# hkchengrex/Cutie

Measured on AMD Instinct MI355X. Metric: frames/sec (480p, 3 objects), higher is better.
Workload: dtype bf16

## Files before the change

### cutie_amd/_lib.py

```python
import ctypes
import os

_HERE = os.path.dirname(os.path.abspath(__file__))
LIB_PATH = os.environ.get('CUTIE_AMD_LIB') or os.path.join(_HERE, 'libcutie_hip.so')
ABI_VERSION = 11
OP_STRUCT_SIZE = 256

_lib = None


class HipLibraryError(RuntimeError):
    pass


def load():
    global _lib
    if _lib is not None:
        return _lib
    if not os.path.exists(LIB_PATH):
        raise HipLibraryError(
            f'{LIB_PATH} not found: build it with `python -c "import __graft_entry__ as g; g.build()"` '
            f'(or `make -C cutie_amd/csrc`).  cutie_amd has no CPU fallback.')
    lib = ctypes.CDLL(LIB_PATH)
    lib.cutie_exec.argtypes = [ctypes.c_void_p, ctypes.c_int, ctypes.c_void_p]
    lib.cutie_exec.restype = ctypes.c_int
    lib.cutie_exec_one.argtypes = [ctypes.c_void_p, ctypes.c_void_p]
    lib.cutie_exec_one.restype = ctypes.c_int
    lib.cutie_graph_capture.argtypes = [ctypes.c_void_p, ctypes.c_int, ctypes.c_void_p]
    lib.cutie_graph_capture.restype = ctypes.c_void_p
    lib.cutie_graph_launch.argtypes = [ctypes.c_void_p, ctypes.c_void_p]
    lib.cutie_graph_launch.restype = ctypes.c_int
    lib.cutie_graph_destroy.argtypes = [ctypes.c_void_p]
    lib.cutie_graph_destroy.restype = None
    lib.cutie_time_ops.argtypes = [ctypes.c_void_p, ctypes.c_int, ctypes.c_int, ctypes.c_void_p]
    lib.cutie_time_ops.restype = ctypes.c_float
    lib.cutie_hip_last_error.argtypes = []
    lib.cutie_hip_last_error.restype = ctypes.c_char_p
    lib.cutie_hip_abi_version.restype = ctypes.c_int
    lib.cutie_op_struct_size.restype = ctypes.c_int
    lib.cutie_hip_build_flags.restype = ctypes.c_int
    if lib.cutie_hip_abi_version() != ABI_VERSION or lib.cutie_op_struct_size() != OP_STRUCT_SIZE:
        raise HipLibraryError(f'{LIB_PATH} is stale (ABI {lib.cutie_hip_abi_version()}, '
                              f'op size {lib.cutie_op_struct_size()}); rebuild it.')
    _lib = lib
    return lib


EXPORTED_SYMBOLS = ['cutie_exec', 'cutie_exec_one', 'cutie_graph_capture', 'cutie_graph_launch',
                    'cutie_graph_destroy', 'cutie_time_ops', 'cutie_hip_last_error',
                    'cutie_hip_abi_version', 'cutie_op_struct_size', 'cutie_hip_build_flags']


def has_diag_kernels():
    return bool(load().cutie_hip_build_flags() & 1)


def has_png_decode():
    return bool(load().cutie_hip_build_flags() & 2)


class HipExecutor:
    is_mock = False

    def __init__(self):
        import torch
        self.lib = load()
        if not torch.cuda.is_available():
            raise HipLibraryError('no HIP device visible: cutie_amd runs on MI355X only (no CPU fallback).')
        self._torch = torch
        self._raw_stream = getattr(torch._C, '_cuda_getCurrentRawStream', None)
        self.graph_stats = [0, 0]
        self._warned = False

    def stream(self):
        raw = self._raw_stream
        if raw is not None:
            return raw(self._torch.cuda.current_device())
        return self._torch.cuda.current_stream().cuda_stream

    def run(self, arr):
        rc = self.lib.cutie_exec(arr.ctypes.data, len(arr), self.stream())
        if rc != 0:
            raise RuntimeError('cutie_exec failed: ' + self.lib.cutie_hip_last_error().decode())

    def run_on(self, arr, stream):
        rc = self.lib.cutie_exec(arr.ctypes.data, len(arr), stream.cuda_stream)
        if rc != 0:
            raise RuntimeError('cutie_exec failed: ' + self.lib.cutie_hip_last_error().decode())

    GRAPH_CACHE_ENTRIES = 24

    def run_cached(self, arr, cache, head=0):
        if head:
            self.run(arr[:head])
            arr = arr[head:]
        key = arr['p'].tobytes()
        ent = cache.get(key)
        if ent is None:
            if len(cache) >= self.GRAPH_CACHE_ENTRIES:
                old = cache.pop(next(iter(cache)))
                if old not in (0, -1):
                    self.lib.cutie_graph_destroy(old)
            cache[key] = 0
            self.graph_stats[0] += 1
            return self.run(arr)
        if ent == 0:
            ent = self.lib.cutie_graph_capture(arr.ctypes.data, len(arr), self.stream()) or -1
            cache[key] = ent
            if ent == -1 and not self._warned:
                self._warned = True
                import warnings
                warnings.warn('HIP graph capture of a launch plan failed (%s); such plans keep running launch by launch'
                              % self.lib.cutie_hip_last_error().decode())
        if ent == -1:
            self.graph_stats[0] += 1
            return self.run(arr)
        self.graph_stats[1] += 1
        if self.lib.cutie_graph_launch(ent, self.stream()) != 0:
            raise RuntimeError('cutie_graph_launch failed: ' + self.lib.cutie_hip_last_error().decode())

    def time_ops(self, arr, iters):
        ms = self.lib.cutie_time_ops(arr.ctypes.data, len(arr), iters, self.stream())
        if ms < 0:
            raise RuntimeError('cutie_time_ops failed: ' + self.lib.cutie_hip_last_error().decode())
        return ms


_executor = None


def get_executor():
    global _executor
    if _executor is None:
        _executor = HipExecutor()
    return _executor


def set_executor_for_testing(ex):
    global _executor
    _executor = ex
```

### cutie_amd/csrc/api.hip

```cpp
#include "common.h"
#include <stdarg.h>
#include <stdio.h>
#include <string.h>

static thread_local char g_err[512] = "";

void cutie_set_error(const char* fmt, ...) {
    va_list ap;
    va_start(ap, fmt);
    vsnprintf(g_err, sizeof(g_err), fmt, ap);
    va_end(ap);
}

static int dispatch(const cutie_op* op, hipStream_t s) {
    switch (op->kind) {
        case CUTIE_OP_CONV: return launch_conv(op, s);
        case CUTIE_OP_QUERY_INIT: return (op->flags & 1) ? launch_attention(op, s) : launch_elementwise(op, s);
        case CUTIE_OP_QFFN: return launch_qchain(op, s);
        case CUTIE_OP_STEM: return launch_stem(op, s);
        case CUTIE_OP_ATTN_Q2P: case CUTIE_OP_ATTN_SELF: case CUTIE_OP_ATTN_P2Q:
            return (op->flags & 12) ? launch_qchain(op, s) : launch_attention(op, s);
        case CUTIE_OP_AUX_MASK:
            return launch_attention(op, s);
        case CUTIE_OP_KEY_PREP: case CUTIE_OP_AFF_SCORE: case CUTIE_OP_AFF_SELECT: case CUTIE_OP_AFF_READOUT:
            return launch_affinity(op, s);
        case CUTIE_OP_RANK_SELECT: case CUTIE_OP_GATHER_ROWS: case CUTIE_OP_CONSOL_AFF: case CUTIE_OP_CONSOL_READ:
            return launch_bank(op, s);
        default:
            if (op->kind > 0 && op->kind < CUTIE_OP__COUNT) return launch_elementwise(op, s);
            cutie_set_error("cutie_exec: unknown op kind %d", op->kind);
            return -3;
    }
}

extern "C" {

int cutie_exec(const cutie_op* ops, int n, void* stream) {
    hipStream_t s = (hipStream_t)stream;
    for (int k = 0; k < n; ++k) {
        int rc = dispatch(&ops[k], s);
        if (rc != 0) {
            if (rc > 0) cutie_set_error("op %d (kind %d): HIP error %d (%s)", k, ops[k].kind, rc, hipGetErrorString((hipError_t)rc));
            else {
                char tmp[400];
                snprintf(tmp, sizeof(tmp), "%s", g_err);
                cutie_set_error("op %d (kind %d): %s", k, ops[k].kind, tmp);
            }
            return rc > 0 ? -1 : rc;
        }
    }
    return 0;
}

int cutie_exec_one(const cutie_op* op, void* stream) { return cutie_exec(op, 1, stream); }

struct GraphHandle { hipGraph_t graph; hipGraphExec_t exec; };

void* cutie_graph_capture(const cutie_op* ops, int n, void* stream) {
    (void)stream;
    static thread_local hipStream_t cap = nullptr;
    if (!cap && hipStreamCreateWithFlags(&cap, hipStreamNonBlocking) != hipSuccess) {
        cap = nullptr;
        (void)hipGetLastError();
        cutie_set_error("graph: cannot create the capture stream");
        return nullptr;
    }
    hipGraph_t graph = nullptr;
    if (hipStreamBeginCapture(cap, hipStreamCaptureModeThreadLocal) != hipSuccess) {
        (void)hipGetLastError();
        cutie_set_error("graph: begin capture failed");
        return nullptr;
    }
    int rc = cutie_exec(ops, n, (void*)cap);
    hipError_t e = hipStreamEndCapture(cap, &graph);
    if (rc != 0 || e != hipSuccess || !graph) {
        if (graph) hipGraphDestroy(graph);
        if (rc == 0) cutie_set_error("graph: end capture failed (%d)", (int)e);
        (void)hipGetLastError();
        return nullptr;
    }
    hipGraphExec_t exec = nullptr;
    if (hipGraphInstantiate(&exec, graph, nullptr, nullptr, 0) != hipSuccess) {
        hipGraphDestroy(graph);
        (void)hipGetLastError();
        cutie_set_error("graph: instantiate failed");
        return nullptr;
    }
    GraphHandle* h = new GraphHandle{graph, exec};
    return h;
}

int cutie_graph_launch(void* graph, void* stream) {
    GraphHandle* h = (GraphHandle*)graph;
    if (!h) { cutie_set_error("graph: null handle"); return -4; }
    hipError_t e = hipGraphLaunch(h->exec, (hipStream_t)stream);
    if (e != hipSuccess) { cutie_set_error("graph launch: %s", hipGetErrorString(e)); return -1; }
    return 0;
}

void cutie_graph_destroy(void* graph) {
    GraphHandle* h = (GraphHandle*)graph;
    if (!h) return;
    hipGraphExecDestroy(h->exec);
    hipGraphDestroy(h->graph);
    delete h;
}

float cutie_time_ops(const cutie_op* ops, int n, int iters, void* stream) {
    hipStream_t s = (hipStream_t)stream;
    hipEvent_t a, b;
    if (hipEventCreate(&a) != hipSuccess || hipEventCreate(&b) != hipSuccess) { cutie_set_error("time: event create failed"); return -1.f; }
    if (cutie_exec(ops, n, stream) != 0) return -1.f;
    hipEventRecord(a, s);
    for (int it = 0; it < iters; ++it)
        if (cutie_exec(ops, n, stream) != 0) return -1.f;
    hipEventRecord(b, s);
    hipEventSynchronize(b);
    float ms = 0.f;
    hipEventElapsedTime(&ms, a, b);
    hipEventDestroy(a);
    hipEventDestroy(b);
    return ms / (float)iters;
}

const char* cutie_hip_last_error(void) { return g_err; }
int cutie_hip_abi_version(void) { return 11; }
int cutie_op_struct_size(void) { return (int)sizeof(cutie_op); }
int cutie_hip_build_flags(void) {
    const int forms = 2;
#ifdef CUTIE_DIAG
    return forms | 1;
#else
    return forms;
#endif
}

}
```

### cutie_amd/csrc/conv_common.h

```cpp
#pragma once
#include "common.h"

struct ConvParams {
    const bf16_t* x1; const bf16_t* x2; const bf16_t* w; const float* bias; const bf16_t* res; void* y;
    int B, H, W, C1, C2, ldx1, ldx2, OH, OW, Cout, ldy, KH, KW, stride, pad, ldr, Kpad;
    int flags, M, Cin, OHW;
    float* part; int splitk, ldp, Kslice;
    long long* gap; unsigned long long* zero; int nzero;
    const unsigned char* pf; int pf_bytes;
    const unsigned char* pf2; int pf2_bytes;
    int res_grp_rows, res_grp_stride;
};
#define GAP_FIXED_SCALE 16777216.f
#define GAP_ELEM_SHIFT 4
__device__ __forceinline__ long long conv_gapfx(float v) {
    if (__builtin_expect(fabsf(v) < 2048.f, 1)) return (long long)__float2int_rn(v * 1048576.f);
    if (v != v) return 0;
    const float c = fminf(fmaxf(v, -1048576.f), 1048576.f);
    const float hi = truncf(c);
    return (long long)(int)hi * 1048576LL + (long long)__float2int_rn((c - hi) * 1048576.f);
}

typedef __attribute__((ext_vector_type(4))) unsigned int u32x4;
typedef const __attribute__((address_space(1))) u32x4* gptr16;
#define GLOAD16(ptr) (*(gptr16)(ptr))

template <int CPR>
__device__ __forceinline__ int swz(int row) {
    return CPR == 4 ? ((row >> 3) & 1) * 3 : (row & (CPR - 1));
}

__device__ __forceinline__ int conv_res_row(const ConvParams& p, int m) {
    if (!(p.flags & CUTIE_F_RES_BCAST)) return m;
    int r = m % p.OHW;
    if (p.res_grp_rows > 0) r += (m / p.res_grp_rows) * p.res_grp_stride;
    return r;
}

__device__ __forceinline__ void conv_finish(const ConvParams& p, float* v, int m, int ch0) {
    const int act = (p.flags >> CUTIE_ACT_SHIFT) & 7;
    const bool out_f32 = p.flags & CUTIE_F_OUT_F32;
    const bool vec_y = out_f32 ? ((p.ldy & 3) == 0) : ((p.ldy & 7) == 0);
    const bool vec_r = (p.ldr & 7) == 0;
    const bool full = ch0 + 7 < p.Cout;
    if (p.bias) {
        if (full && (reinterpret_cast<uintptr_t>(p.bias) & 15) == 0) {
            const float4 b0 = *reinterpret_cast<const float4*>(p.bias + ch0), b1 = *reinterpret_cast<const float4*>(p.bias + ch0 + 4);
            v[0] += b0.x; v[1] += b0.y; v[2] += b0.z; v[3] += b0.w; v[4] += b1.x; v[5] += b1.y; v[6] += b1.z; v[7] += b1.w;
        } else {
#pragma unroll
            for (int r = 0; r < 8; ++r) if (ch0 + r < p.Cout) v[r] += p.bias[ch0 + r];
        }
    }
    if (p.res) {
        const int mres = conv_res_row(p, m);
        const bf16_t* rp = p.res + (long)mres * p.ldr + ch0;
        if (full && vec_r) {
            const uint4 rr = *reinterpret_cast<const uint4*>(rp);
            v[0] += __uint_as_float(rr.x << 16); v[1] += __uint_as_float(rr.x & 0xffff0000u);
            v[2] += __uint_as_float(rr.y << 16); v[3] += __uint_as_float(rr.y & 0xffff0000u);
            v[4] += __uint_as_float(rr.z << 16); v[5] += __uint_as_float(rr.z & 0xffff0000u);
            v[6] += __uint_as_float(rr.w << 16); v[7] += __uint_as_float(rr.w & 0xffff0000u);
        } else {
#pragma unroll
            for (int r = 0; r < 8; ++r) if (ch0 + r < p.Cout) v[r] += bf2f(rp[r]);
        }
    }
#pragma unroll
    for (int r = 0; r < 8; ++r) {
        if (act == CUTIE_ACT_RELU) v[r] = fmaxf(v[r], 0.f);
        else if (act == CUTIE_ACT_SIGMOID) v[r] = sigmoidf_(v[r]);
        else if (act == CUTIE_ACT_SQ1) v[r] = v[r] * v[r] + 1.f;
    }
    if (out_f32) {
        float* yp = reinterpret_cast<float*>(p.y) + (long)m * p.ldy + ch0;
        if (full && vec_y) {
            *reinterpret_cast<float4*>(yp) = make_float4(v[0], v[1], v[2], v[3]);
            *reinterpret_cast<float4*>(yp + 4) = make_float4(v[4], v[5], v[6], v[7]);
        } else {
#pragma unroll
            for (int r = 0; r < 8; ++r) if (ch0 + r < p.Cout) yp[r] = v[r];
        }
    } else {
        bf16_t* yp = reinterpret_cast<bf16_t*>(p.y) + (long)m * p.ldy + ch0;
        if (full && vec_y) {
            *reinterpret_cast<uint4*>(yp) = make_uint4(pack_bf2(v[0], v[1]), pack_bf2(v[2], v[3]), pack_bf2(v[4], v[5]), pack_bf2(v[6], v[7]));
        } else {
#pragma unroll
            for (int r = 0; r < 8; ++r) if (ch0 + r < p.Cout) yp[r] = f2bf(v[r]);
        }
    }
}

template <int BM, int BN, int BK, int WK>
constexpr int conv_lds_bytes() {
    constexpr int pipe = WK * 2 * (BM + BN) * (BK / 8) * 16, epi = BM * (BN + 4) * 4;
    return pipe > epi ? pipe : epi;
}

__device__ __forceinline__ void conv_preload_args(const ConvParams& p) {
#ifndef CONV_NO_PRELOAD
    asm volatile("" :: "s"(p.x1), "s"(p.w), "s"(p.bias), "s"(p.res), "s"(p.y), "s"(p.zero),
                 "s"(p.B), "s"(p.H), "s"(p.W), "s"(p.C1), "s"(p.C2), "s"(p.ldx1), "s"(p.ldx2), "s"(p.OH), "s"(p.OW), "s"(p.Cout), "s"(p.ldy),
                 "s"(p.KH), "s"(p.KW), "s"(p.stride), "s"(p.pad), "s"(p.ldr), "s"(p.Kpad), "s"(p.flags), "s"(p.M), "s"(p.Cin), "s"(p.OHW),
                 "s"(p.nzero), "s"(gridDim.x), "s"(gridDim.y));
#endif
}

#ifdef CONV_TIMELINE
#define TL_MAX 96
#define TL_BYTES (16 * TL_MAX * 8)
#define TL_DECL(...) unsigned long long* const tlp_ = reinterpret_cast<unsigned long long*>(__VA_ARGS__) + wave * TL_MAX; int tln_ = 0;
#define TL_PUT_(ID, CAP) { if (tln_ < (CAP)) { const unsigned long long t_ = (__builtin_readcyclecounter() << 8) | (unsigned)(ID); if ((threadIdx.x & 63) == 0) tlp_[tln_] = t_; ++tln_; } }
#define TL(ID) TL_PUT_(ID, TL_MAX - 6)
#define TLE(ID) TL_PUT_(ID, TL_MAX)
#define TL_DUMP(LOGICAL, NB, NWAVES)                                                                                        \
    {                                                                                                                       \
        const int slot_ = (LOGICAL) == 0 ? 0 : (LOGICAL) == 1 ? 1 : (LOGICAL) == (NB) / 2 ? 2 : (LOGICAL) == (NB) - 1 ? 3 : -1; \
        if (slot_ >= 0 && p.part) {                                                                                         \
            __builtin_amdgcn_s_waitcnt(0);                                                                                  \
            unsigned long long* o_ = reinterpret_cast<unsigned long long*>(p.part) + ((long)slot_ * 16 + wave) * (TL_MAX + 2); \
            if ((threadIdx.x & 63) == 0) { o_[0] = 0x544c0000ull | (unsigned)tln_; o_[1] = ((unsigned long long)(LOGICAL) << 32) | (unsigned)(NWAVES); } \
            for (int q_ = threadIdx.x & 63; q_ < tln_; q_ += 64) o_[2 + q_] = tlp_[q_];                                     \
        }                                                                                                                   \
    }
#else
#define TL_BYTES 0
#define TL_DECL(...)
#define TL(ID)
#define TLE(ID)
#define TL_DUMP(LOGICAL, NB, NWAVES)
#endif

int launch_conv_dma(const ConvParams& p, int tile, hipStream_t s);
int launch_conv_pc(const ConvParams& p, int tile, hipStream_t s);
```

### cutie_amd/csrc/conv_igemm.hip

```cpp
#include "conv_common.h"

template <int BM, int BN, int WM, int WN, int BK, int S, int OCC, int WK>
__global__ __launch_bounds__(WM * WN * WK * 64) void conv_igemm_kernel(ConvParams p) {
    if (p.flags & CUTIE_F_PRIO) __builtin_amdgcn_s_setprio(1);
    constexpr int NTB = WM * WN * WK * 64;
    constexpr int NT = WM * WN * 64;
    constexpr int CPR = BK / 8;
    constexpr int RPT = NT / CPR;
    constexpr int NX = (BM * CPR) / NT;
    constexpr int NWC = (BN * CPR + NT - 1) / NT;
    constexpr int TM = BM / WM / 16;
    constexpr int TN = BN / WN / 16;
    constexpr int KSUB = BK / 32;
    constexpr int NWRAP = BK == 32 ? 4 : BK / 32;
    static_assert((NT == 256 || NT == 512) && NTB <= 1024 && NX >= 1 && TM >= 1 && TN >= 1 && S >= 2 && (BM * CPR) % NT == 0, "bad tile");
    constexpr int LDC = BN + 4;
    constexpr int GRP_CHUNKS = 2 * (BM + BN) * CPR;
    extern __shared__ __attribute__((aligned(16))) u32x4 smem_raw[];
    const int grp = threadIdx.x / NT;
    u32x4 (*smem)[(BM + BN) * CPR] = reinterpret_cast<u32x4 (*)[(BM + BN) * CPR]>(smem_raw + grp * GRP_CHUNKS);

    const int tid = threadIdx.x % NT, lane = tid & 63, wave = tid >> 6;
    int m0, n0;
    {
// ... 136 lines not shown
            const int ks = ks0 + u;
            if (ks < nk) K_ITER(ks, u, ks + S - 1 < nk, ks + 1 < nk)
        }
    }

    float* ctile = reinterpret_cast<float*>(smem_raw);
#pragma unroll
    for (int g = WK - 1; g >= 0; --g) {
        if (grp == g) {
#pragma unroll
            for (int b = 0; b < TM; ++b)
#pragma unroll
                for (int a = 0; a < TN; ++a) {
                    const int px = pm0 + b * 16 + l15, ch = cn0 + a * 16 + l4 * 4;
                    f32x4* dst = reinterpret_cast<f32x4*>(ctile + px * LDC + ch);
                    if (g == WK - 1) *dst = acc[a][b];
                    else { f32x4 t = *dst; t[0] += acc[a][b][0]; t[1] += acc[a][b][1]; t[2] += acc[a][b][2]; t[3] += acc[a][b][3]; *dst = t; }
                }
        }
        __syncthreads();
    }
    constexpr int CH8 = BN / 8;
    if (p.splitk == 1) {
        for (int q = threadIdx.x; q < BM * CH8; q += NTB) {
            const int px = q / CH8, c8 = q - px * CH8;
            const int m = m0 + px, ch0 = n0 + c8 * 8;
            if (m >= p.M || ch0 >= p.Cout) continue;
            const f32x4 lo = *reinterpret_cast<const f32x4*>(ctile + px * LDC + c8 * 8);
            const f32x4 hi = *reinterpret_cast<const f32x4*>(ctile + px * LDC + c8 * 8 + 4);
            float v[8] = {lo[0], lo[1], lo[2], lo[3], hi[0], hi[1], hi[2], hi[3]};
            conv_finish(p, v, m, ch0);
        }
        return;
    }
    float* part = p.part + (long)blockIdx.z * p.M * p.ldp;
    for (int q = threadIdx.x; q < BM * CH8; q += NTB) {
        const int px = q / CH8, c8 = q - px * CH8;
        const int m = m0 + px, ch0 = n0 + c8 * 8;
        if (m >= p.M || ch0 >= p.Cout) continue;
        float* dst = part + (long)m * p.ldp + ch0;
        *reinterpret_cast<f32x4*>(dst) = *reinterpret_cast<const f32x4*>(ctile + px * LDC + c8 * 8);
        *reinterpret_cast<f32x4*>(dst + 4) = *reinterpret_cast<const f32x4*>(ctile + px * LDC + c8 * 8 + 4);
    }
}

__global__ __launch_bounds__(256) void conv_splitk_reduce_kernel(ConvParams p) {
    const int c8n = p.ldp >> 3;
    const long q = (long)blockIdx.x * 256 + threadIdx.x;
    if (q >= (long)p.M * c8n) return;
    const int m = (int)(q / c8n), ch0 = (int)(q - (long)m * c8n) * 8;
    float v[8] = {0.f, 0.f, 0.f, 0.f, 0.f, 0.f, 0.f, 0.f};
    for (int z = 0; z < p.splitk; ++z) {
        const float* src = p.part + ((long)z * p.M + m) * p.ldp + ch0;
        const f32x4 lo = *reinterpret_cast<const f32x4*>(src);
        const f32x4 hi = *reinterpret_cast<const f32x4*>(src + 4);
        v[0] += lo[0]; v[1] += lo[1]; v[2] += lo[2]; v[3] += lo[3];
        v[4] += hi[0]; v[5] += hi[1]; v[6] += hi[2]; v[7] += hi[3];
    }
    conv_finish(p, v, m, ch0);
}

__global__ __launch_bounds__(256) void conv_cout1_kernel(ConvParams p) {
    if (p.flags & CUTIE_F_PRIO) __builtin_amdgcn_s_setprio(1);
    extern __shared__ __attribute__((aligned(16))) unsigned char wlds_raw[];
    u32x4* wlds = reinterpret_cast<u32x4*>(wlds_raw);
    const int LP = p.Cin >> 3;
    const int ntap = p.KH * p.KW;
    const int ppb = 256 / LP;
    const int sub = threadIdx.x / LP, cl = threadIdx.x % LP;
    const int m = blockIdx.x * ppb + sub;
    const bool is33 = p.KH == 3 && p.KW == 3;
    const bool relu_in = p.flags & CUTIE_F_RELU_IN;
    const float bias0 = p.bias ? p.bias[0] : 0.f;
    u32x4 xv[9];
    float ok[9];
    if (is33) {
        const int mc = min(m, p.M - 1);
        const int b = mc / p.OHW, rem = mc - b * p.OHW, oh = rem / p.OW, ow = rem - oh * p.OW;
#pragma unroll
        for (int t = 0; t < 9; ++t) {
            const int ih = oh * p.stride - p.pad + t / 3, iw = ow * p.stride - p.pad + t % 3;
            const bool v = (unsigned)ih < (unsigned)p.H && (unsigned)iw < (unsigned)p.W;
            const int ihc = min(max(ih, 0), p.H - 1), iwc = min(max(iw, 0), p.W - 1);
            xv[t] = *reinterpret_cast<const u32x4*>(p.x1 + (((long)b * p.H + ihc) * p.W + iwc) * p.ldx1 + cl * 8);
            ok[t] = v ? 1.f : 0.f;
        }
    }
    for (int t = threadIdx.x; t < ntap * LP; t += 256) wlds[t] = *reinterpret_cast<const u32x4*>(p.w + (long)t * 8);
    __syncthreads();
    float acc = 0.f;
    if (m < p.M) {
        const int b = m / p.OHW, rem = m - b * p.OHW, oh = rem / p.OW, ow = rem - oh * p.OW;
        if (is33) {
#pragma unroll
            for (int t = 0; t < 9; ++t) {
                u32x4 x = xv[t];
                if (relu_in) { x.x = relu_bf2(x.x); x.y = relu_bf2(x.y); x.z = relu_bf2(x.z); x.w = relu_bf2(x.w); }
                const u32x4 wv = wlds[t * LP + cl];
                float a = 0.f;
#pragma unroll
                for (int i = 0; i < 4; ++i) {
                    a += __uint_as_float(x[i] << 16) * __uint_as_float(wv[i] << 16);
                    a += __uint_as_float(x[i] & 0xffff0000u) * __uint_as_float(wv[i] & 0xffff0000u);
                }
                acc += a * ok[t];
            }
        } else
        for (int kh = 0; kh < p.KH; ++kh) {
            const int ih = oh * p.stride - p.pad + kh;
            if ((unsigned)ih >= (unsigned)p.H) continue;
            for (int kw = 0; kw < p.KW; ++kw) {
                const int iw = ow * p.stride - p.pad + kw;
                if ((unsigned)iw >= (unsigned)p.W) continue;
                u32x4 xv = *reinterpret_cast<const u32x4*>(p.x1 + (((long)b * p.H + ih) * p.W + iw) * p.ldx1 + cl * 8);
                if (relu_in) { xv.x = relu_bf2(xv.x); xv.y = relu_bf2(xv.y); xv.z = relu_bf2(xv.z); xv.w = relu_bf2(xv.w); }
                const u32x4 wv = wlds[(kh * p.KW + kw) * LP + cl];
#pragma unroll
                for (int i = 0; i < 4; ++i) {
                    acc += __uint_as_float(xv[i] << 16) * __uint_as_float(wv[i] << 16);
                    acc += __uint_as_float(xv[i] & 0xffff0000u) * __uint_as_float(wv[i] & 0xffff0000u);
                }
            }
        }
    }
    for (int o = LP >> 1; o > 0; o >>= 1) acc += __shfl_xor(acc, o, 64);
    if (cl == 0 && m < p.M) {
        float v = acc + bias0;
        const int act = (p.flags >> CUTIE_ACT_SHIFT) & 7;
        if (act == CUTIE_ACT_RELU) v = fmaxf(v, 0.f);
        else if (act == CUTIE_ACT_SIGMOID) v = sigmoidf_(v);
        else if (act == CUTIE_ACT_SQ1) v = v * v + 1.f;
        if (p.flags & CUTIE_F_OUT_F32) reinterpret_cast<float*>(p.y)[(long)m * p.ldy] = v;
        else reinterpret_cast<bf16_t*>(p.y)[(long)m * p.ldy] = f2bf(v);
    }
}

template <int TR>
__global__ __launch_bounds__(256) void conv_cout1_tile_kernel(ConvParams p) {
    if (p.flags & CUTIE_F_PRIO) __builtin_amdgcn_s_setprio(1);
    static_assert(TR % 4 == 0, "rows per wave");
    constexpr int TC = 16, PW = TC + 2, NPIX = (TR + 2) * PW, RW = TR / 4;
    __shared__ u32x4 tile[NPIX * 16];
    const int tid = threadIdx.x, lane = tid & 63, wave = tid >> 6, n = lane & 15, g = lane >> 4;
    const int tiles_x = (p.W + TC - 1) / TC, tiles_y = (p.H + TR - 1) / TR;
    const int b = blockIdx.x / (tiles_x * tiles_y), rem = blockIdx.x - b * tiles_x * tiles_y;
    const int ty = rem / tiles_x, tx = rem - ty * tiles_x;
    const int x0 = tx * TC, y0 = ty * TR;
    const bool relu_in = p.flags & CUTIE_F_RELU_IN;
    const float bias0 = p.bias ? p.bias[0] : 0.f;
    __shared__ u32x4 wl[36 * 4];
    const u32x4 wmine = tid < 144 ? *reinterpret_cast<const u32x4*>(p.w + (long)((tid >> 4) * 16 + (tid & 15)) * 8) : (u32x4){0u, 0u, 0u, 0u};
    constexpr int NCH = (NPIX * 16 + 255) / 256;
    u32x4 st[NCH];
#pragma unroll
    for (int i = 0; i < NCH; ++i) {
        const int q = tid + 256 * i, px = q >> 4, c = q & 15;
        const int iy = y0 + px / PW - 1, ix = x0 + px % PW - 1;
        const bool in = q < NPIX * 16 && (unsigned)iy < (unsigned)p.H && (unsigned)ix < (unsigned)p.W;
        const long o = in ? (((long)b * p.H + iy) * p.W + ix) * p.ldx1 + c * 8 : 0;
        const u32x4 v = *reinterpret_cast<const u32x4*>(p.x1 + o);
        st[i] = in ? v : (u32x4){0u, 0u, 0u, 0u};
    }
#pragma unroll
    for (int i = 0; i < NCH; ++i) {
        const int q = tid + 256 * i, px = q >> 4, c = q & 15;
        u32x4 v = st[i];
        if (relu_in) { v.x = relu_bf2(v.x); v.y = relu_bf2(v.y); v.z = relu_bf2(v.z); v.w = relu_bf2(v.w); }
        if (q < NPIX * 16) tile[px * 16 + (c ^ (px & 15))] = v;
    }
    if (tid < 144) wl[tid] = wmine;
    __syncthreads();
    f32x4 acc[RW];
#pragma unroll
    for (int r = 0; r < RW; ++r) acc[r] = (f32x4){0.f, 0.f, 0.f, 0.f};
    const u32x4 zero4 = {0u, 0u, 0u, 0u};
#pragma unroll
    for (int sidx = 0; sidx < 36; ++sidx) {
        const int tap = sidx >> 2, ky = tap / 3, kx = tap - 3 * ky, ch = (sidx & 3) * 4 + g;
        const u32x4 wv = wl[sidx * 4 + g];
        const bf16x8 wb = __builtin_bit_cast(bf16x8, n == 0 ? wv : zero4);
#pragma unroll
        for (int r = 0; r < RW; ++r) {
            const int px = (wave * RW + r + ky) * PW + n + kx;
            const bf16x8 a = __builtin_bit_cast(bf16x8, tile[px * 16 + (ch ^ (px & 15))]);
            acc[r] = __builtin_amdgcn_mfma_f32_16x16x32_bf16(a, wb, acc[r], 0, 0, 0);
        }
    }
    if (n == 0) {
        const int act = (p.flags >> CUTIE_ACT_SHIFT) & 7;
#pragma unroll
        for (int r = 0; r < RW; ++r) {
            const int oy = y0 + wave * RW + r;
#pragma unroll
            for (int q = 0; q < 4; ++q) {
                const int x = x0 + 4 * g + q;
                if (x < p.W && oy < p.H) {
                    float v = acc[r][q] + bias0;
                    if (act == CUTIE_ACT_RELU) v = fmaxf(v, 0.f);
                    else if (act == CUTIE_ACT_SIGMOID) v = sigmoidf_(v);
                    else if (act == CUTIE_ACT_SQ1) v = v * v + 1.f;
                    const long m = ((long)b * p.H + oy) * p.W + x;
                    if (p.flags & CUTIE_F_OUT_F32) reinterpret_cast<float*>(p.y)[m * p.ldy] = v;
                    else reinterpret_cast<bf16_t*>(p.y)[m * p.ldy] = f2bf(v);
                }
            }
        }
    }
}

template <int R>
__global__ __launch_bounds__(256) void conv_cout1_rows_kernel(ConvParams p) {
    if (p.flags & CUTIE_F_PRIO) __builtin_amdgcn_s_setprio(1);
    const int LP = p.Cin >> 3;
    const int ppb = 256 / LP;
    const int sub = threadIdx.x / LP, cl = threadIdx.x % LP;
    const int tiles_x = (p.W + ppb - 1) / ppb, tiles_y = (p.H + R - 1) / R;
    const int b = blockIdx.x / (tiles_x * tiles_y), rem = blockIdx.x - b * tiles_x * tiles_y;
    const int ty = rem / tiles_x, tx = rem - ty * tiles_x;
    const int x = tx * ppb + sub, y0 = ty * R;
    const bool relu_in = p.flags & CUTIE_F_RELU_IN;
    const float bias0 = p.bias ? p.bias[0] : 0.f;
    u32x4 wv[9];
#pragma unroll
    for (int t = 0; t < 9; ++t) wv[t] = *reinterpret_cast<const u32x4*>(p.w + (long)(t * LP + cl) * 8);
    u32x4 xv[R + 2][3];
    float okc[3];
#pragma unroll
    for (int kx = 0; kx < 3; ++kx) okc[kx] = ((unsigned)(x + kx - 1) < (unsigned)p.W) ? 1.f : 0.f;
#pragma unroll
    for (int r = 0; r < R + 2; ++r) {
        const int iy = min(max(y0 + r - 1, 0), p.H - 1);
#pragma unroll
        for (int kx = 0; kx < 3; ++kx) {
            const int ix = min(max(x + kx - 1, 0), p.W - 1);
            xv[r][kx] = *reinterpret_cast<const u32x4*>(p.x1 + (((long)b * p.H + iy) * p.W + ix) * p.ldx1 + cl * 8);
        }
    }
    if (relu_in) {
#pragma unroll
        for (int r = 0; r < R + 2; ++r)
#pragma unroll
            for (int kx = 0; kx < 3; ++kx) { u32x4& v = xv[r][kx]; v.x = relu_bf2(v.x); v.y = relu_bf2(v.y); v.z = relu_bf2(v.z); v.w = relu_bf2(v.w); }
    }
    const int act = (p.flags >> CUTIE_ACT_SHIFT) & 7;
#pragma unroll
    for (int j = 0; j < R; ++j) {
        const int oy = y0 + j;
        float acc = 0.f;
#pragma unroll
        for (int ky = 0; ky < 3; ++ky) {
            const float okr = ((unsigned)(oy + ky - 1) < (unsigned)p.H) ? 1.f : 0.f;
#pragma unroll
            for (int kx = 0; kx < 3; ++kx) {
                const u32x4 xx = xv[j + ky][kx], ww = wv[ky * 3 + kx];
                float a = 0.f;
#pragma unroll
                for (int i = 0; i < 4; ++i) {
                    a += __uint_as_float(xx[i] << 16) * __uint_as_float(ww[i] << 16);
                    a += __uint_as_float(xx[i] & 0xffff0000u) * __uint_as_float(ww[i] & 0xffff0000u);
                }
                acc += a * (okr * okc[kx]);
            }
        }
        for (int o = LP >> 1; o > 0; o >>= 1) acc += __shfl_xor(acc, o, 64);
        if (cl == 0 && x < p.W && oy < p.H) {
            float v = acc + bias0;
            if (act == CUTIE_ACT_RELU) v = fmaxf(v, 0.f);
            else if (act == CUTIE_ACT_SIGMOID) v = sigmoidf_(v);
            else if (act == CUTIE_ACT_SQ1) v = v * v + 1.f;
            const long m = ((long)b * p.H + oy) * p.W + x;
            if (p.flags & CUTIE_F_OUT_F32) reinterpret_cast<float*>(p.y)[m * p.ldy] = v;
            else reinterpret_cast<bf16_t*>(p.y)[m * p.ldy] = f2bf(v);
        }
    }
}

template <int BM, int BN, int WM, int WN, int BK, int S, int OCC, int WK = 1>
static int launch_cfg(ConvParams p, hipStream_t s) {
    if (p.Kpad % BK) { cutie_set_error("conv: Kpad %d not a multiple of BK %d", p.Kpad, BK); return -2; }
    if (BK > 32 && p.Cin < 32) { cutie_set_error("conv: BK %d needs Cin >= 32 (Cin=%d)", BK, p.Cin); return -2; }
    const int nk_all = p.Kpad / BK;
    if (p.splitk > nk_all) { cutie_set_error("conv: splitk %d > K tiles %d", p.splitk, nk_all); return -2; }
    if (nk_all % (p.splitk * WK)) { cutie_set_error("conv: splitk %d x %d K groups must divide the %d K tiles", p.splitk, WK, nk_all); return -2; }
    p.Kslice = p.Kpad / p.splitk;
    constexpr int lds = conv_lds_bytes<BM, BN, BK, WK>();
    static bool attr_set = false;
    if (!attr_set) {
        if (lds > 65536 && hipFuncSetAttribute(reinterpret_cast<const void*>(conv_igemm_kernel<BM, BN, WM, WN, BK, S, OCC, WK>),
                                               hipFuncAttributeMaxDynamicSharedMemorySize, lds) != hipSuccess) {
            cutie_set_error("conv: cannot raise the dynamic LDS limit to %d bytes", lds);
            return -2;
        }
        attr_set = true;
    }
    dim3 grid((p.M + BM - 1) / BM, (p.Cout + BN - 1) / BN, p.splitk);
    hipLaunchKernelGGL((conv_igemm_kernel<BM, BN, WM, WN, BK, S, OCC, WK>), grid, dim3(WM * WN * WK * 64), lds, s, p);
    if (p.splitk > 1) {
        const long nq = (long)p.M * (p.ldp >> 3);
        hipLaunchKernelGGL(conv_splitk_reduce_kernel, dim3((unsigned)((nq + 255) / 256)), dim3(256), 0, s, p);
    }
    return (int)hipGetLastError();
}

int launch_conv(const cutie_op* op, hipStream_t s) {
    ConvParams p;
    p.x1 = (const bf16_t*)op->p[0]; p.x2 = (const bf16_t*)op->p[1]; p.w = (const bf16_t*)op->p[2];
    p.bias = (const float*)op->p[3]; p.res = (const bf16_t*)op->p[4]; p.y = (void*)op->p[5];
    const int32_t* i = op->i;
    p.B = i[0]; p.H = i[1]; p.W = i[2]; p.C1 = i[3]; p.C2 = i[4]; p.ldx1 = i[5]; p.ldx2 = i[6];
    p.OH = i[7]; p.OW = i[8]; p.Cout = i[9]; p.ldy = i[10]; p.KH = i[11]; p.KW = i[12];
    p.stride = i[13]; p.pad = i[14]; p.ldr = i[15]; p.Kpad = i[16];
    p.flags = op->flags; p.OHW = p.OH * p.OW; p.M = p.B * p.OHW; p.Cin = p.C1 + p.C2;
    p.splitk = i[19] > 1 ? i[19] : 1; p.part = (float*)op->p[6];
    p.ldp = (p.Cout + 7) & ~7;
    p.gap = (long long*)op->p[7]; p.zero = (unsigned long long*)op->p[8]; p.nzero = i[21];
    p.pf = (const unsigned char*)op->p[9]; p.pf_bytes = op->p[9] ? i[22] : 0;
    p.pf2 = (const unsigned char*)op->p[10]; p.pf2_bytes = op->p[10] ? i[23] : 0;
    p.res_grp_rows = p.res_grp_stride = 0;
    if ((p.flags & CUTIE_F_RES_BCAST) && op->f[0] > 0.f) {
        const int kg = (int)op->f[0];
        if (kg <= 0 || p.B % kg || op->f[1] < (float)p.OHW || op->f[1] != (float)(int)op->f[1]) { cutie_set_error("conv: residual groups of %d objects do not divide B = %d (or stride %g < OH*OW)", kg, p.B, (double)op->f[1]); return -2; }
        p.res_grp_rows = kg * p.OHW; p.res_grp_stride = (int)op->f[1];
    }
    if ((p.gap || p.zero) && (i[17] < 60 || i[17] >= 200 || ((p.flags & CUTIE_F_OUT_F32) && p.gap) || (p.Cout & 7) || (p.ldy & 7) || (p.res && (p.ldr & 7)))) {
        cutie_set_error("conv: GAP accumulation / zero job need an LDS-DMA tile (60..199), bf16 output, Cout %% 8 == 0 (tile %d)", i[17]);
        return -2;
    }
    if (p.splitk > 1 && (!p.part || (long)p.splitk * p.M * p.ldp > (long)i[20] * 1024)) {
        cutie_set_error("conv: split-K %d needs the fp32 partial scratch (p6, capacity i20 KiB-floats)", p.splitk);
        return -2;
    }
    if ((p.C1 & 7) || (p.C2 & 7) || (p.ldx1 & 7) || (p.C2 && (p.ldx2 & 7)) || (p.Kpad & 31) ||
        p.Kpad < p.KH * p.KW * p.Cin || p.M <= 0 || p.Cout <= 0) {
        cutie_set_error("conv: bad geometry C1=%d C2=%d ldx1=%d ldx2=%d Kpad=%d M=%d Cout=%d",
                        p.C1, p.C2, p.ldx1, p.ldx2, p.Kpad, p.M, p.Cout);
        return -2;
    }
    if (i[17] == 19) {
        const int LP = p.Cin >> 3;
        if (p.Cout != 1 || p.C2 != 0 || p.res || LP > 64 || (LP & (LP - 1)) || LP < 1) {
            cutie_set_error("conv cout1: needs Cout=1, single source, no residual, Cin/8 a power of two <= 64 (Cin=%d)", p.Cin);
            return -2;
        }
        const int ppb = 256 / LP;
        if (!(p.flags & CUTIE_F_PLAIN) && p.KH == 3 && p.KW == 3 && p.stride == 1 && p.pad == 1 && p.OH == p.H && p.OW == p.W && LP >= 8 && LP <= 32 && p.H * p.W >= 4096) {
            if (LP == 16 && !(p.flags & CUTIE_F_TILE_OFF)) {
                constexpr int TR = 8;
                const int blocks = p.B * ((p.H + TR - 1) / TR) * ((p.W + 15) / 16);
                hipLaunchKernelGGL(conv_cout1_tile_kernel<TR>, dim3(blocks), dim3(256), 0, s, p);
                return (int)hipGetLastError();
            }
            constexpr int R = 4;
            const int blocks = p.B * ((p.H + R - 1) / R) * ((p.W + ppb - 1) / ppb);
            hipLaunchKernelGGL(conv_cout1_rows_kernel<R>, dim3(blocks), dim3(256), 0, s, p);
            return (int)hipGetLastError();
        }
        hipLaunchKernelGGL(conv_cout1_kernel, dim3((p.M + ppb - 1) / ppb), dim3(256), (size_t)p.KH * p.KW * LP * 16, s, p);
        return (int)hipGetLastError();
    }
    if (i[17] >= 60 && i[17] < 90) return launch_conv_dma(p, i[17], s);
    if (i[17] >= 100 && i[17] < 200) return launch_conv_pc(p, i[17], s);
    switch (i[17]) {
        case 0: return launch_cfg<128, 128, 2, 2, 32, 4, 2>(p, s);
        case 1: return launch_cfg<128, 64, 2, 2, 32, 4, 3>(p, s);
        case 2: return launch_cfg<64, 64, 2, 2, 32, 4, 4>(p, s);
        case 3: return launch_cfg<256, 16, 4, 1, 32, 4, 3>(p, s);
        case 4: return launch_cfg<64, 128, 2, 2, 32, 4, 3>(p, s);
        case 5: return launch_cfg<64, 64, 2, 2, 64, 4, 3>(p, s);
        case 6: return launch_cfg<64, 128, 2, 2, 64, 3, 2>(p, s);
        case 7: return launch_cfg<128, 128, 2, 2, 64, 2, 2>(p, s);
        case 8: return launch_cfg<64, 64, 2, 2, 128, 3, 2>(p, s);
        case 9: return launch_cfg<32, 64, 2, 2, 64, 4, 4>(p, s);
        case 10: return launch_cfg<128, 64, 2, 2, 64, 3, 2>(p, s);
        case 11: return launch_cfg<32, 64, 2, 2, 128, 3, 3>(p, s);
        case 12: return launch_cfg<32, 128, 2, 2, 64, 3, 2>(p, s);
        case 13: return launch_cfg<64, 64, 2, 4, 64, 4, 5>(p, s);
        case 14: return launch_cfg<128, 64, 4, 2, 64, 4, 4>(p, s);
        case 15: return launch_cfg<64, 128, 2, 4, 64, 4, 4>(p, s);
        case 16: return launch_cfg<128, 128, 2, 4, 64, 3, 3>(p, s);
        case 17: return launch_cfg<64, 64, 2, 4, 128, 3, 4>(p, s);
        case 18: return launch_cfg<128, 128, 2, 4, 32, 4, 4>(p, s);
        case 20: return launch_cfg<64, 64, 2, 2, 64, 4, 3, 2>(p, s);
        case 21: return launch_cfg<64, 64, 2, 2, 128, 3, 2, 2>(p, s);
        case 22: return launch_cfg<32, 64, 2, 2, 128, 3, 3, 2>(p, s);
        case 23: return launch_cfg<128, 64, 2, 2, 64, 3, 2, 2>(p, s);
        case 24: return launch_cfg<64, 128, 2, 2, 64, 3, 2, 2>(p, s);
        case 25: return launch_cfg<128, 128, 2, 2, 64, 2, 2, 2>(p, s);
        case 26: return launch_cfg<32, 64, 2, 2, 64, 4, 4, 2>(p, s);
        case 27: return launch_cfg<64, 64, 2, 2, 64, 3, 3, 4>(p, s);
        case 28: return launch_cfg<32, 64, 2, 2, 64, 4, 4, 4>(p, s);
        case 29: return launch_cfg<64, 128, 2, 2, 32, 4, 3, 2>(p, s);
        case 30: return launch_cfg<64, 64, 2, 2, 32, 4, 4, 2>(p, s);
        default: cutie_set_error("conv: bad tile id %d", i[17]); return -2;
    }
}
```

### cutie_amd/csrc/conv_pc.hip

```cpp
#include "conv_common.h"

typedef __amdgpu_buffer_rsrc_t rsrc_t;
#define PC_WORD3 0x00020000
#define PC_RECORDS 0x7fffffff
#define PC_OOB 0x80000000u
#define LDS_PTR(p) ((__attribute__((address_space(3))) void*)(p))
#define PC_WAIT_VM(N) __builtin_amdgcn_s_waitcnt(((N) & 15) | (((N) >> 4) << 14) | (7 << 4) | (15 << 8))
#define PC_WAIT_LGKM0() __builtin_amdgcn_s_waitcnt(15 | (3 << 14) | (7 << 4) | (0 << 8))
#define PC_BARRIER() { asm volatile("" ::: "memory"); __builtin_amdgcn_s_barrier(); asm volatile("" ::: "memory"); }
#ifdef PC_ABL_NO_LOOPBAR
#define PC_LOOP_BARRIER() { asm volatile("" ::: "memory"); }
#else
#define PC_LOOP_BARRIER() PC_BARRIER()
#endif
#ifdef PC_ABL_NO_WAIT
#define PC_LOOP_WAIT_VM(N) ((void)0)
#else
#define PC_LOOP_WAIT_VM(N) PC_WAIT_VM(N)
#endif
#ifdef PC_ABL_SAME_TILE
#define PC_SAME_TILE_GUARD(...)
#else
#define PC_SAME_TILE_GUARD(...) __VA_ARGS__
#endif
#ifdef PC_ABL_NO_DMA
#define PC_DMA(...) ((void)0)
#else
#define PC_DMA(...) __builtin_amdgcn_raw_ptr_buffer_load_lds(__VA_ARGS__)
#endif

__device__ __forceinline__ rsrc_t pc_rsrc(const void* base) {
    return __builtin_amdgcn_make_buffer_rsrc(const_cast<void*>(base), 0, PC_RECORDS, PC_WORD3);
}

typedef short pc_s16x2 __attribute__((ext_vector_type(2)));
__device__ __forceinline__ unsigned pc_relu2(unsigned w) {
    return __builtin_bit_cast(unsigned, __builtin_elementwise_max(__builtin_bit_cast(pc_s16x2, w), (pc_s16x2){0, 0}));
}

__device__ __forceinline__ int pc_wrow(int R, bool pair) {
    if (!pair) return R;
    const int ii = R & 15, alo = (R >> 4) & 1;
    return (R & ~31) | ((ii >> 2) << 3) | (alo << 2) | (ii & 3);
}

#define PC_HT(TH, TW) ((TH) * 256 + (TW))
template <int BM, int BN, int NS, int HT>
constexpr int pc_lds_bytes(int NPW) {
    if (HT == 0) return NS * (BM + BN) * 128;
    const int TH = HT >> 8, TW = HT & 255, npiece = ((TH + 2) * (TW + 2) + 7) / 8, nxp = (npiece + NPW - 1) / NPW;
    return 2 * nxp * NPW * 1024 + NS * BN * 128;
}

template <int NCH>
__device__ __forceinline__ void pc_finish(const ConvParams& p, float (&v)[NCH], int m, int ch0, bool vec_ok, bool have_res,
                                          const unsigned (&rpre)[NCH / 2], float (&stored)[NCH]) {
#ifdef PC_ABL_FIXED_EPI
    {
#pragma unroll
        for (int r = 0; r < NCH; ++r) v[r] = fmaxf(v[r], 0.f);
        bf16_t* yp = reinterpret_cast<bf16_t*>(p.y) + (long)m * p.ldy + ch0;
        unsigned o[NCH / 2];
#pragma unroll
        for (int r = 0; r < NCH / 2; ++r) o[r] = pack_bf2(v[2 * r], v[2 * r + 1]);
        if constexpr (NCH == 8) *reinterpret_cast<uint4*>(yp) = make_uint4(o[0], o[1], o[NCH / 2 - 2], o[NCH / 2 - 1]);
        else *reinterpret_cast<uint2*>(yp) = make_uint2(o[0], o[1]);
        return;
    }
#endif
    const int act = (p.flags >> CUTIE_ACT_SHIFT) & 7;
    const bool out_f32 = p.flags & CUTIE_F_OUT_F32;
    const bool full = ch0 + NCH <= p.Cout;
    if (p.res) {
        if (have_res) {
#pragma unroll
            for (int r = 0; r < NCH / 2; ++r) { v[2 * r] += __uint_as_float(rpre[r] << 16); v[2 * r + 1] += __uint_as_float(rpre[r] & 0xffff0000u); }
        } else {
            const int mres = conv_res_row(p, m);
            const bf16_t* rp = p.res + (long)mres * p.ldr + ch0;
            if (full && vec_ok) {
                unsigned rr[NCH / 2];
                if constexpr (NCH == 8) { const uint4 t = *reinterpret_cast<const uint4*>(rp); rr[0] = t.x; rr[1] = t.y; rr[NCH / 2 - 2] = t.z; rr[NCH / 2 - 1] = t.w; }
                else { const uint2 t = *reinterpret_cast<const uint2*>(rp); rr[0] = t.x; rr[1] = t.y; }
#pragma unroll
                for (int r = 0; r < NCH / 2; ++r) { v[2 * r] += __uint_as_float(rr[r] << 16); v[2 * r + 1] += __uint_as_float(rr[r] & 0xffff0000u); }
            } else {
#pragma unroll
                for (int r = 0; r < NCH; ++r) if (ch0 + r < p.Cout) v[r] += bf2f(rp[r]);
            }
        }
    }
#pragma unroll
    for (int r = 0; r < NCH; ++r) {
        if (act == CUTIE_ACT_RELU) v[r] = fmaxf(v[r], 0.f);
        else if (act == CUTIE_ACT_SIGMOID) v[r] = sigmoidf_(v[r]);
        else if (act == CUTIE_ACT_SQ1) v[r] = v[r] * v[r] + 1.f;
    }
    if (out_f32) {
        float* yp = reinterpret_cast<float*>(p.y) + (long)m * p.ldy + ch0;
        if (full && vec_ok) {
#pragma unroll
            for (int r = 0; r < NCH; r += 4) *reinterpret_cast<float4*>(yp + r) = make_float4(v[r], v[r + 1], v[r + 2], v[r + 3]);
        } else {
#pragma unroll
            for (int r = 0; r < NCH; ++r) if (ch0 + r < p.Cout) yp[r] = v[r];
        }
    } else {
        bf16_t* yp = reinterpret_cast<bf16_t*>(p.y) + (long)m * p.ldy + ch0;
        unsigned o[NCH / 2];
#pragma unroll
        for (int r = 0; r < NCH / 2; ++r) o[r] = pack_bf2(v[2 * r], v[2 * r + 1]);
        if (full && vec_ok) {
            if constexpr (NCH == 8) *reinterpret_cast<uint4*>(yp) = make_uint4(o[0], o[1], o[NCH / 2 - 2], o[NCH / 2 - 1]);
            else *reinterpret_cast<uint2*>(yp) = make_uint2(o[0], o[1]);
        } else {
#pragma unroll
            for (int r = 0; r < NCH; ++r) if (ch0 + r < p.Cout) yp[r] = (bf16_t)(r & 1 ? o[r >> 1] >> 16 : o[r >> 1] & 0xffffu);
        }
        {
#pragma unroll
            for (int r = 0; r < NCH / 2; ++r) { stored[2 * r] = __uint_as_float(o[r] << 16); stored[2 * r + 1] = __uint_as_float(o[r] & 0xffff0000u); }
        }
    }
}

__device__ __forceinline__ int pc_div(int m, int d, float rd) {
    int q = (int)((float)m * rd);
    int r = m - q * d;
    q += (r >= d) ? 1 : 0;
    q -= (r < 0) ? 1 : 0;
    return q;
}

__device__ __forceinline__ int pc_res_row(const ConvParams& p, int m) {
    if (!(p.flags & CUTIE_F_RES_BCAST)) return m;
    int r = m - pc_div(m, p.OHW, __builtin_amdgcn_rcpf((float)p.OHW)) * p.OHW;
    if (p.res_grp_rows > 0) r += pc_div(m, p.res_grp_rows, __builtin_amdgcn_rcpf((float)p.res_grp_rows)) * p.res_grp_stride;
    return r;
}

template <int NCH>
__device__ __forceinline__ long long pc_colsum16(const long long (&s)[NCH], int l15, int& c, bool& writer) {
    const bool h8 = l15 & 8, h4 = l15 & 4, h2 = l15 & 2;
    long long w;
    if constexpr (NCH == 8) {
        long long t[4], u[2];
#pragma unroll
        for (int r = 0; r < 4; ++r) t[r] = (h8 ? s[4 + r] : s[r]) + __shfl_xor(h8 ? s[r] : s[4 + r], 8, 64);
#pragma unroll
        for (int r = 0; r < 2; ++r) u[r] = (h4 ? t[2 + r] : t[r]) + __shfl_xor(h4 ? t[r] : t[2 + r], 4, 64);
        w = (h2 ? u[1] : u[0]) + __shfl_xor(h2 ? u[0] : u[1], 2, 64);
        w += __shfl_xor(w, 1, 64);
        c = (h8 ? 4 : 0) + (h4 ? 2 : 0) + (h2 ? 1 : 0);
        writer = (l15 & 1) == 0;
    } else {
        long long t[2];
#pragma unroll
        for (int r = 0; r < 2; ++r) t[r] = (h8 ? s[2 + r] : s[r]) + __shfl_xor(h8 ? s[r] : s[2 + r], 8, 64);
        w = (h4 ? t[1] : t[0]) + __shfl_xor(h4 ? t[0] : t[1], 4, 64);
        w += __shfl_xor(w, 2, 64);
        w += __shfl_xor(w, 1, 64);
        c = (h8 ? 2 : 0) + (h4 ? 1 : 0);
        writer = (l15 & 3) == 0;
    }
    return w;
}
__device__ __forceinline__ long long pc_gapfx(float v) { return conv_gapfx(v); }
__device__ __forceinline__ void pc_gap_add(const ConvParams& p, int obj, int ch, long long v) {
    if (ch < p.Cout) atomicAdd(reinterpret_cast<unsigned long long*>(p.gap + (long)obj * p.Cout + ch), (unsigned long long)(v << GAP_ELEM_SHIFT));
}

template <int NCH, int TM, int TNP, bool PAIR, bool RELU_OUT, bool F32, bool RES, bool PRE, bool GAPJ = false>
__device__ __forceinline__ void pc_epilogue_fast(const ConvParams& p, const f32x4 (&acc)[PAIR ? 2 * TNP : TNP][TM], const float (&bias)[TNP][NCH],
                                                 const int (&mrow)[TM], const bool (&mval)[TM], int chbase,
                                                 const unsigned (&rpre)[PRE ? TM : 1][PRE ? TNP : 1][NCH / 2], int gap_obj = 0, int l15 = 0) {
    unsigned rr[TM][TNP][NCH / 2];
    if (RES && !PRE) {
#pragma unroll
        for (int b = 0; b < TM; ++b) {
            const int mres = pc_res_row(p, mrow[b]);
#pragma unroll
            for (int a = 0; a < TNP; ++a) {
                const bf16_t* rp = p.res + (long)mres * p.ldr + chbase + a * (PAIR ? 32 : 16);
#pragma unroll
                for (int r = 0; r < NCH / 2; ++r) rr[b][a][r] = 0u;
                if (mval[b]) {
                    if constexpr (NCH == 8) { const uint4 t = *reinterpret_cast<const uint4*>(rp); rr[b][a][0] = t.x; rr[b][a][1] = t.y; rr[b][a][NCH / 2 - 2] = t.z; rr[b][a][NCH / 2 - 1] = t.w; }
                    else { const uint2 t = *reinterpret_cast<const uint2*>(rp); rr[b][a][0] = t.x; rr[b][a][1] = t.y; }
                }
            }
        }
    }
#pragma unroll
    for (int a = 0; a < TNP; ++a) {
        long long gs[NCH];
#pragma unroll
        for (int r = 0; r < NCH; ++r) gs[r] = 0;
#pragma unroll
        for (int b = 0; b < TM; ++b) {
            float v[NCH];
#pragma unroll
            for (int r = 0; r < 4; ++r) {
                v[r] = acc[PAIR ? 2 * a : a][b][r] + bias[a][r];
                if (PAIR) v[(NCH - 4) + r] = acc[PAIR ? 2 * a + 1 : a][b][r] + bias[a][(NCH - 4) + r];
            }
            if (RES) {
#pragma unroll
                for (int r = 0; r < NCH / 2; ++r) {
                    const unsigned w = PRE ? rpre[PRE ? b : 0][PRE ? a : 0][r] : rr[b][a][r];
                    v[2 * r] += __uint_as_float(w << 16); v[2 * r + 1] += __uint_as_float(w & 0xffff0000u);
                }
            }
            if (RELU_OUT) {
#pragma unroll
                for (int r = 0; r < NCH; ++r) v[r] = fmaxf(v[r], 0.f);
            }
            if (mval[b]) {
                const long off = (long)mrow[b] * p.ldy + chbase + a * (PAIR ? 32 : 16);
                if (F32) {
                    float* yp = reinterpret_cast<float*>(p.y) + off;
#pragma unroll
                    for (int r = 0; r < NCH; r += 4) *reinterpret_cast<float4*>(yp + r) = make_float4(v[r], v[r + 1], v[r + 2], v[r + 3]);
                } else {
                    bf16_t* yp = reinterpret_cast<bf16_t*>(p.y) + off;
                    unsigned o[NCH / 2];
#pragma unroll
                    for (int r = 0; r < NCH / 2; ++r) o[r] = pack_bf2(v[2 * r], v[2 * r + 1]);
                    if constexpr (NCH == 8) *reinterpret_cast<uint4*>(yp) = make_uint4(o[0], o[1], o[NCH / 2 - 2], o[NCH / 2 - 1]);
                    else *reinterpret_cast<uint2*>(yp) = make_uint2(o[0], o[1]);
                    if (GAPJ) {
#pragma unroll
                        for (int r = 0; r < NCH / 2; ++r) { gs[2 * r] += pc_gapfx(__uint_as_float(o[r] << 16)); gs[2 * r + 1] += pc_gapfx(__uint_as_float(o[r] & 0xffff0000u)); }
                    }
                }
            }
        }
        if (GAPJ) {
            int c; bool writer;
            const long long tot = pc_colsum16<NCH>(gs, l15, c, writer);
            if (writer) pc_gap_add(p, gap_obj, chbase + a * (PAIR ? 32 : 16) + c, tot);
        }
    }
}

template <int BM, int BN, int WM, int WN, int NPW, int NS, int HT, bool TAPS, bool RELU, bool TWO, int KP = 1>
__global__ __launch_bounds__((WM * WN + NPW) * 64) void conv_pc_kernel(ConvParams p) {
#if __HIP_DEVICE_COMPILE__
    if (p.flags & CUTIE_F_PRIO) __builtin_amdgcn_s_setprio(1);
    constexpr bool HALO = HT > 0;
    constexpr int TH = HALO ? (HT >> 8) : 1, TW = HALO ? (HT & 255) : 1;
    constexpr int NC = WM * WN, NTC = NC * 64;
    constexpr int TM = BM / WM / 16, TN = BN / WN / 16;
    constexpr bool PAIR = (TN % 2) == 0;
    constexpr int NCH = PAIR ? 8 : 4, TNP = PAIR ? TN / 2 : TN;
    constexpr int NXI = HALO ? 1 : BM / 8 / NPW;
    constexpr int NWI = BN / 8 / NPW;
    constexpr int LPT = HALO ? NWI : NXI + NWI;
    constexpr int PH = TH + 2, PW = TW + 2;
    constexpr int NPIECE = (PH * PW + 7) / 8, NXP = (NPIECE + NPW - 1) / NPW, XBUF = NXP * NPW * 1024;
    constexpr int WSTAGE = BN * 128, STAGE = HALO ? WSTAGE : (BM + BN) * 128;
    constexpr int WBASE = HALO ? 2 * XBUF : 0;
    constexpr bool PRE_RES = TM * TNP <= 4;
    static_assert(TM >= 1 && TN >= 1 && BM % (WM * 16) == 0 && BN % (WN * 16) == 0 && NWI >= 1 && NWI * 8 * NPW == BN && NS >= 2 && NS <= 8, "bad tile");
    static_assert(HALO || (NXI >= 1 && NXI * 8 * NPW == BM), "bad stream tile");
    static_assert(!HALO || (TH * TW <= BM && TH * TW > BM - 16 * WM && (NS == 3 || NS == 4) && NXP <= 11 - NS && NXP <= 8), "bad halo tile");
    static_assert(KP == 1 || (KP == 2 && (NS == 4 || NS == 6)), "pair steps: a ring of 2 or 3 pairs");
    constexpr int NP = NS / 2;
    extern __shared__ __attribute__((aligned(16))) u32x4 pc_smem[];
    char* const lds = reinterpret_cast<char*>(pc_smem);
    const int tid = threadIdx.x, lane = tid & 63, l15 = lane & 15, l4 = lane >> 4;
    const int wave = __builtin_amdgcn_readfirstlane(tid >> 6);
    TL_DECL(lds + pc_lds_bytes<BM, BN, NS, HT>(NPW))
    TL(0)
    conv_preload_args(p);
    TL(10)
    const int nb = gridDim.x * gridDim.y;
    int logical;
    {
        const int id = blockIdx.y * gridDim.x + blockIdx.x;
        const int xcd = id & 7, kq = id >> 3, q = nb >> 3, r = nb & 7;
        logical = (xcd < r ? xcd * (q + 1) : r * (q + 1) + (xcd - r) * q) + kq;
    }
    const int mt = logical / (int)gridDim.y;
    const int n0 = (logical - mt * (int)gridDim.y) * BN;
    int m0 = 0, bimg = 0, ty0 = 0, tx0 = 0;
    if (HALO) {
        const int tiles_x = (p.W + TW - 1) / TW, tiles_y = (p.H + TH - 1) / TH, per = tiles_x * tiles_y;
        bimg = mt / per;
        const int r = mt - bimg * per, ty = r / tiles_x;
        ty0 = ty * TH;
        tx0 = (r - ty * tiles_x) * TW;
    } else {
        m0 = mt * BM;
    }
    if (p.zero) {
        const int nthr = (NC + NPW) * 64;
        for (int z = (blockIdx.y * gridDim.x + blockIdx.x) * nthr + tid; z < p.nzero; z += gridDim.x * gridDim.y * nthr) p.zero[z] = 0ull;
    }
    const int nslice = p.Cin / 64;
#ifdef PC_ABL_NO_LOOP
    const int nk = 0;
#else
    const int nk = HALO ? nslice * 9 : p.KH * p.KW * nslice;
#endif

    if (wave >= NC) {
        const int pw = wave - NC;
        const int lr = lane >> 3;
        const unsigned kcb = (unsigned)(((lane & 7) ^ lr) * 16);
        constexpr unsigned PRE = 4096;
        unsigned woff[NWI];
#pragma unroll
        for (int i = 0; i < NWI; ++i)
            woff[i] = (unsigned)((n0 + pc_wrow((pw * NWI + i) * 8 + lr, PAIR)) * p.Kpad * 2) + kcb + (HALO ? 0u : PRE - (unsigned)i * 1024u);
        const rsrc_t rw = pc_rsrc(reinterpret_cast<const char*>(p.w) - (HALO ? 0 : PRE));
        const int wdst = WBASE + (HALO ? 0 : BM * 128) + pw * NWI * 1024;
        TL(11)
        if constexpr (!HALO) {
            const int cin2 = p.Cin * 2, c12 = p.C1 * 2;
            unsigned wsoff = 0;
            int ldw = 0;
#define PCS_WPIECE(I, LD)                                                                                      \
    if constexpr ((I) < NWI) PC_DMA(rw, LDS_PTR(lds + (LD) + wdst), 16, woff[(I) < NWI ? (I) : 0], wsoff, (I) * 1024, 0);
#define PCS_LOAD_W(LD) { PCS_WPIECE(0, LD) PCS_WPIECE(1, LD) PCS_WPIECE(2, LD) PCS_WPIECE(3, LD) PC_SAME_TILE_GUARD(wsoff += 128;) }
            TL(1)
#pragma unroll
            for (int s = 0; s < NS - 1; ++s)
                if (s < nk) { PCS_LOAD_W(ldw) ldw += STAGE; }
            unsigned xoff1[NXI], xoff2[NXI], vmask[NXI];
            {
                int m = m0 + pw * NXI * 8 + lr;
                const int mm = m < p.M ? m : p.M - 1;
                const bool linear = !TAPS && p.stride == 1;
                int b = 0, oh = 0, ow = mm;
                if (!linear) {
                    b = pc_div(mm, p.OHW, __builtin_amdgcn_rcpf((float)p.OHW));
                    const int rem = mm - b * p.OHW;
                    oh = pc_div(rem, p.OW, __builtin_amdgcn_rcpf((float)p.OW));
                    ow = rem - oh * p.OW;
                }
#pragma unroll
                for (int i = 0; i < NXI; ++i) {
                    const int ih0 = oh * p.stride, iw0 = ow * p.stride;
                    const unsigned pix = linear ? (unsigned)min(mm + 8 * i, p.M - 1) : (unsigned)((b * p.H + ih0) * p.W + iw0);
                    xoff1[i] = pix * (unsigned)(p.ldx1 * 2) + kcb + PRE - (unsigned)i * 1024u;
                    xoff2[i] = TWO ? pix * (unsigned)(p.ldx2 * 2) + kcb + PRE - (unsigned)i * 1024u : 0u;
                    unsigned mk = 0;
                    if (TAPS) {
                        unsigned cols = 0;
                        for (int k = 0; k < p.KW; ++k) cols |= ((unsigned)(iw0 - p.pad + k) < (unsigned)p.W) ? (1u << k) : 0u;
                        for (int k = 0; k < p.KH; ++k) mk |= ((unsigned)(ih0 - p.pad + k) < (unsigned)p.H) ? (cols << (k * p.KW)) : 0u;
                    }
                    vmask[i] = mk;
                    if (i + 1 < NXI && !linear) {
                        m += 8;
                        if (m < p.M) {
                            ow += 8;
                            while (ow >= p.OW) { ow -= p.OW; ++oh; }
                            while (oh >= p.OH) { oh -= p.OH; ++b; }
                        }
                    }
                }
            }
            const long shift = (long)p.pad * p.W + p.pad;
            const char* xb1 = reinterpret_cast<const char*>(p.x1 - shift * p.ldx1) - PRE;
            const char* xb2 = TWO ? reinterpret_cast<const char*>(p.x2 - shift * p.ldx2) - PRE : xb1;
            const rsrc_t rx1 = pc_rsrc(xb1), rx2 = pc_rsrc(xb2);
            const int xdst = pw * NXI * 1024;
            int tap = 0, kw = 0, cc = 0, pixA = 0, pixB = 0;
            const int stepA1 = p.ldx1 * 2, stepA2 = (p.W - p.KW + 1) * p.ldx1 * 2;
            const int stepB1 = p.ldx2 * 2, stepB2 = (p.W - p.KW + 1) * p.ldx2 * 2;
#define PCS_XPIECE(I, LD)                                                                                      \
    if constexpr ((I) < NXI) {                                                                                 \
        const unsigned v_ = in1_ ? xoff1[(I) < NXI ? (I) : 0] : xoff2[(I) < NXI ? (I) : 0];                   \
        PC_DMA(rx_, LDS_PTR(lds + (LD) + xdst), 16, (!TAPS || (vmask[(I) < NXI ? (I) : 0] & tapbit_)) ? v_ : PC_OOB, soff_, (I) * 1024, 0); \
    }
#define PCS_LOAD_X(LD)                                                                                         \
    {                                                                                                          \
        const unsigned tapbit_ = 1u << tap;                                                                    \
        const bool in1_ = !TWO || cc < c12;                                                                    \
        const unsigned soff_ = (unsigned)(in1_ ? pixA + cc : pixB + cc - c12);                                 \
        const rsrc_t rx_ = in1_ ? rx1 : rx2;                                                                   \
        PCS_XPIECE(0, LD) PCS_XPIECE(1, LD) PCS_XPIECE(2, LD) PCS_XPIECE(3, LD)                                \
        PC_SAME_TILE_GUARD(cc += 128;)                                                                         \
        if (TAPS || TWO) {                                                                                     \
            const bool wrap_ = cc >= cin2;                                                                     \
            cc = wrap_ ? 0 : cc;                                                                               \
            if (TAPS) {                                                                                        \
                tap += wrap_ ? 1 : 0;                                                                          \
                kw += wrap_ ? 1 : 0;                                                                           \
                const bool wrap2_ = kw == p.KW;                                                                \
                kw = wrap2_ ? 0 : kw;                                                                          \
                pixA += wrap_ ? (wrap2_ ? stepA2 : stepA1) : 0;                                                \
                if (TWO) pixB += wrap_ ? (wrap2_ ? stepB2 : stepB1) : 0;                                       \
            }                                                                                                  \
        }                                                                                                      \
    }
#define PCS_LOAD_TILE(LD) { PCS_LOAD_X(LD) PCS_LOAD_W(LD) }
            static_assert(NXI <= 4 && NWI <= 4, "pieces per producer wave");
            int ld = 0;
#pragma unroll
            for (int s = 0; s < NS - 1; ++s)
                if (s < nk) { PCS_LOAD_X(ld) ld += STAGE; }
            if constexpr (KP == 1) {
            if (NS == 3 && nk >= NS - 1) { PC_WAIT_VM((NS - 2) * NXI); } else { PC_WAIT_VM(0); }
            TL(2)
            PC_BARRIER()
            int kt = 0;
            for (; kt < nk - (NS - 1); ++kt) {
                TL(3)
                PCS_LOAD_TILE(ld)
                TL(4)
                PC_LOOP_WAIT_VM((NS - 2) * LPT);
                TL(5)
                PC_LOOP_BARRIER()
                ld = ld == (NS - 1) * STAGE ? 0 : ld + STAGE;
            }
            for (; kt < nk; ++kt) {
                PC_WAIT_VM(0);
                PC_LOOP_BARRIER()
            }
            } else {
            PC_WAIT_VM(0);
            TL(2)
            PC_BARRIER()
            int t = nk < NS - 1 ? nk : NS - 1;
            const int P = (nk + 1) >> 1;
            int u = 0;
            for (; 2 * (u + NP - 1) + 1 < nk; ++u) {
                TL(3)
                for (; t <= 2 * (u + NP - 1) + 1; ++t) { PCS_LOAD_TILE(ld) ld = ld == (NS - 1) * STAGE ? 0 : ld + STAGE; }
                TL(4)
                PC_LOOP_WAIT_VM((NP - 2) * 2 * LPT);
                TL(5)
                PC_LOOP_BARRIER()
            }
            for (; u < P; ++u) {
                for (; t < nk && t <= 2 * (u + NP - 1) + 1; ++t) { PCS_LOAD_TILE(ld) ld = ld == (NS - 1) * STAGE ? 0 : ld + STAGE; }
                PC_WAIT_VM(0);
                PC_LOOP_BARRIER()
            }
            }
#undef PCS_LOAD_TILE
#undef PCS_LOAD_X
#undef PCS_LOAD_W
#undef PCS_WPIECE
#undef PCS_XPIECE
        } else {
            unsigned xo1[NXP], xo2[NXP];
#pragma unroll
            for (int i = 0; i < NXP; ++i) {
                const int pp = (pw + NPW * i) * 8 + lr;
                const int py = pp / PW, px = pp - py * PW;
                const int gy = ty0 - 1 + py, gx = tx0 - 1 + px;
                const bool ok = pp < PH * PW && (unsigned)gy < (unsigned)p.H && (unsigned)gx < (unsigned)p.W;
                const unsigned pix = (unsigned)((bimg * p.H + gy) * p.W + gx);
                const unsigned kc = (unsigned)(((lane & 7) ^ (pp & 7)) * 16);
                xo1[i] = ok ? pix * (unsigned)(p.ldx1 * 2) + kc : PC_OOB;
                xo2[i] = TWO ? (ok ? pix * (unsigned)(p.ldx2 * 2) + kc : PC_OOB) : 0u;
            }
            const rsrc_t rx1 = pc_rsrc(p.x1), rx2 = TWO ? pc_rsrc(p.x2) : rx1;
            const int cin2 = p.Cin * 2;
#define PCH_XPIECE(I, SL)                                                                                      \
    {                                                                                                          \
        const bool f_ = !TWO || (SL) * 64 < p.C1;                                                              \
        const int so_ = (f_ ? (SL) * 64 : (SL) * 64 - p.C1) * 2;                                               \
        PC_DMA(f_ ? rx1 : rx2, LDS_PTR(lds + ((SL) & 1) * XBUF + (pw + NPW * (I)) * 1024), 16, f_ ? xo1[I] : xo2[I], so_, 0, 0); \
    }
            int wsl = 0, wtap = 0, wld = 0;
            unsigned wso = 0;
#define PCH_WTILE()                                                                                            \
    {                                                                                                          \
        _Pragma("unroll") for (int i = 0; i < NWI; ++i) PC_DMA(rw, LDS_PTR(lds + wld + wdst + i * 1024), 16, woff[i], wso, 0, 0); \
        wld = wld == (NS - 1) * WSTAGE ? 0 : wld + WSTAGE;                                                     \
        ++wtap; PC_SAME_TILE_GUARD(wso += (unsigned)cin2;)                                                     \
        if (wtap == 9) { wtap = 0; ++wsl; PC_SAME_TILE_GUARD(wso = (unsigned)(wsl * 128);) }                                       \
    }
            TL(1)
#pragma unroll
            for (int s = 0; s < NS - 1; ++s)
                if (s < nk) PCH_WTILE()
#pragma unroll
            for (int i = 0; i < NXP; ++i) PCH_XPIECE(i, 0)
            PC_WAIT_VM(0);
            TL(2)
            PC_BARRIER()
            if constexpr (KP == 1) {
            int sl = 0, tap = 0;
            int xprev = 0;
            int kt = 0;
            for (; kt < nk - (NS - 1); ++kt) {
                TL(3)
                const int xp = (sl + 1 < nslice && tap < NXP) ? 1 : 0;
                if (xp) {
                    switch (tap) {
                        case 0: if constexpr (NXP > 0) PCH_XPIECE(0, sl + 1) break;
                        case 1: if constexpr (NXP > 1) PCH_XPIECE(NXP > 1 ? 1 : 0, sl + 1) break;
                        case 2: if constexpr (NXP > 2) PCH_XPIECE(NXP > 2 ? 2 : 0, sl + 1) break;
                        case 3: if constexpr (NXP > 3) PCH_XPIECE(NXP > 3 ? 3 : 0, sl + 1) break;
                        case 4: if constexpr (NXP > 4) PCH_XPIECE(NXP > 4 ? 4 : 0, sl + 1) break;
                        case 5: if constexpr (NXP > 5) PCH_XPIECE(NXP > 5 ? 5 : 0, sl + 1) break;
                        case 6: if constexpr (NXP > 6) PCH_XPIECE(NXP > 6 ? 6 : 0, sl + 1) break;
                        default: if constexpr (NXP > 7) PCH_XPIECE(NXP > 7 ? 7 : 0, sl + 1) break;
                    }
                }
                PCH_WTILE()
                TL(4)
                const int xin = NS == 3 ? xp : xp + xprev;
                if (xin == 0) { PC_LOOP_WAIT_VM((NS - 2) * NWI); } else if (xin == 1) { PC_LOOP_WAIT_VM((NS - 2) * NWI + 1); } else { PC_LOOP_WAIT_VM((NS - 2) * NWI + 2); }
                TL(5)
                PC_LOOP_BARRIER()
                xprev = xp;
                ++tap;
                if (tap == 9) { tap = 0; ++sl; }
            }
            for (; kt < nk; ++kt) {
                PC_WAIT_VM(0);
                PC_LOOP_BARRIER()
            }
            } else {
            static_assert(NXP <= 8 && NP <= 3, "pair steps: two patch pieces per iteration over four iterations");
            int t = nk < NS - 1 ? nk : NS - 1;
            const int P = (nk + 1) >> 1;
            int ps = 0, pk = 0, pnext = 5;
            int u = 0;
            for (; 2 * (u + NP - 1) + 1 < nk; ++u) {
                TL(3)
                if (u == pnext) { ++ps; pk = 0; pnext += (ps & 1) ? 4 : 5; }
                if (ps + 1 < nslice && pk < 4) {
                    switch (pk) {
                        case 0: if constexpr (NXP > 0) PCH_XPIECE(0, ps + 1) if constexpr (NXP > 1) PCH_XPIECE(NXP > 1 ? 1 : 0, ps + 1) break;
                        case 1: if constexpr (NXP > 2) PCH_XPIECE(NXP > 2 ? 2 : 0, ps + 1) if constexpr (NXP > 3) PCH_XPIECE(NXP > 3 ? 3 : 0, ps + 1) break;
                        case 2: if constexpr (NXP > 4) PCH_XPIECE(NXP > 4 ? 4 : 0, ps + 1) if constexpr (NXP > 5) PCH_XPIECE(NXP > 5 ? 5 : 0, ps + 1) break;
                        default: if constexpr (NXP > 6) PCH_XPIECE(NXP > 6 ? 6 : 0, ps + 1) if constexpr (NXP > 7) PCH_XPIECE(NXP > 7 ? 7 : 0, ps + 1) break;
                    }
                    ++pk;
                }
                for (; t <= 2 * (u + NP - 1) + 1; ++t) PCH_WTILE()
                TL(4)
                PC_LOOP_WAIT_VM((NP - 2) * 2 * NWI);
                TL(5)
                PC_LOOP_BARRIER()
            }
            for (; u < P; ++u) {
                for (; t < nk && t <= 2 * (u + NP - 1) + 1; ++t) PCH_WTILE()
                PC_WAIT_VM(0);
// ... 365 lines not shown
```

### cutie_amd/model/plans.py

```python
import math
import os

import numpy as np
import torch

from .. import _lib
from .. import ops as O
from ..ops import Dyn
from .param_spec import resnet_layers

BF16, F32 = torch.bfloat16, torch.float32


class Act:
    __slots__ = ('t', 'B', 'H', 'W', 'C', 'ld')

    def __init__(self, t, B, H, W, C, ld=None):
        self.t, self.B, self.H, self.W, self.C, self.ld = t, B, H, W, C, (C if ld is None else ld)


def positional_encoding(h, w, dim_total, scale, temperature):
    dim = int(math.ceil(dim_total / 4) * 2)
    inv_freq = 1.0 / (temperature ** (torch.arange(0, dim, 2).float() / dim))
    py = torch.arange(h, dtype=torch.float32)
    px = torch.arange(w, dtype=torch.float32)
    py = py / (py[-1] + 1e-6) * scale
    px = px / (px[-1] + 1e-6) * scale
    sy, sx = py[:, None] * inv_freq[None], px[:, None] * inv_freq[None]
    ey = torch.stack((sy.sin(), sy.cos()), -1).flatten(-2)
    ex = torch.stack((sx.sin(), sx.cos()), -1).flatten(-2)
    emb = torch.zeros(h, w, dim * 2)
    emb[:, :, :dim] = ex[None]
    emb[:, :, dim:] = ey[:, None]
    return emb


TILE_CACHE_ENV = 'CUTIE_AMD_TILE_CACHE'
TUNE_REPS, TUNE_ITERS = (int(v) for v in os.environ.get('CUTIE_AMD_TUNE', '3x8').lower().split('x'))


GRAPHS = os.environ.get('CUTIE_AMD_GRAPHS', '0') not in ('', '0')
GRAPH_MIN_OPS = 8
QINIT_SKIP = os.environ.get('CUTIE_AMD_QINIT_SKIP', '1') not in ('', '0')
AUTOTUNE = os.environ.get('CUTIE_AMD_AUTOTUNE', '0') not in ('', '0')
PACKAGED_TILES = os.path.join(os.path.dirname(os.path.abspath(__file__)), '..', 'tiles_gfx950.json')


def load_tile_cache():
    import json
    path = os.environ.get(TILE_CACHE_ENV)
    if path == 'none':
        return {}
    cache = {}
    for f in (PACKAGED_TILES, path):
        if f and os.path.exists(f):
            try:
                cache.update({tuple(k): tuple(v) for k, v in json.load(open(f))['tiles']})
            except Exception:
                pass
    return cache


def save_tile_cache(cache):
    import json
    path = os.environ.get(TILE_CACHE_ENV)
    if not path or path == 'none':
        return
    tmp = path + '.tmp%d' % os.getpid()
    with open(tmp, 'w') as f:
        json.dump({'tiles': [[list(k), list(v)] for k, v in cache.items()]}, f)
    os.replace(tmp, path)


ARENA_POISON = os.environ.get('CUTIE_AMD_ARENA_POISON', '0') not in ('', '0')
ARENA_ALIGN = 256


class Arena:

    def __init__(self, device):
        self.device = device
        self.tensor = None
        self.size = 0
        self.plans = []

    def require(self, nbytes):
        if nbytes <= self.size:
            return
        self.size = -(-int(nbytes * 1.1) // (1 << 20)) * (1 << 20)
        if self.tensor is not None:
            self._old = [self.tensor]
        self.tensor = torch.zeros(self.size, dtype=torch.uint8, device=self.device)
        for p in self.plans:
            p.rebind_arena()

    def base(self):
        return self.tensor.data_ptr()


_USE_COUNT = getattr(torch._C, '_storage_Use_Count', None)


def _storage_users(t):
    return _USE_COUNT(t.untyped_storage()._cdata) - 2


class SlotPool:
    SLOTS = int(os.environ.get('CUTIE_AMD_POOL_SLOTS', '6'))

    IDLE_FRAMES = int(os.environ.get('CUTIE_AMD_POOL_IDLE', '512'))

    def __init__(self):
        self.groups = {}
        self.last_used = {}
        self.frame = 0
        self.offset = 0

    def tick(self):
        self.frame += 1
        if self.frame % 64 == 0 and self.IDLE_FRAMES > 0:
            for k in [k for k, f in self.last_used.items() if self.frame - f > self.IDLE_FRAMES]:
                self.groups.pop(k, None)
                del self.last_used[k]

    @staticmethod
    def _make_slot(specs, dev):
        names = tuple(specs)
        tensors = [torch.zeros(sh, dtype=dt, device=dev) for (sh, dt, z) in specs.values()]
        stores = [t.untyped_storage() for t in tensors]
        return names, tensors, stores, [st._cdata for st in stores]

    @staticmethod
    def _free(slot):
        for c in slot[3]:
            if _USE_COUNT(c) != 2:
                return False
        return True

    @staticmethod
    def _hand_out(slot):
        return {nm: t.detach() for nm, t in zip(slot[0], slot[1])}

    def get(self, key, specs, dev):
        if self.SLOTS <= 0 or _USE_COUNT is None:
            return {n: (torch.zeros if z else torch.empty)(sh, dtype=dt, device=dev) for n, (sh, dt, z) in specs.items()}
        slots = self.groups.get(key)
        if slots is None:
            slots = self.groups[key] = {}
        self.last_used[key] = self.frame
        i = (self.frame + self.offset) % self.SLOTS
        slot = slots.get(i)
        if slot is None:
            slot = slots[i] = self._make_slot(specs, dev)
        if self._free(slot):
            return self._hand_out(slot)
        return {n: (torch.zeros if z else torch.empty)(sh, dtype=dt, device=dev) for n, (sh, dt, z) in specs.items()}

    def get_ring(self, key, specs, dev, ring=3):
        if self.SLOTS <= 0 or _USE_COUNT is None:
            return {n: (torch.zeros if z else torch.empty)(sh, dtype=dt, device=dev) for n, (sh, dt, z) in specs.items()}
        slots = self.groups.setdefault(key, {'next': 0})
        self.last_used[key] = self.frame
        i = slots['next'] % ring
        slots['next'] = i + 1
        slot = slots.get(i)
        if slot is None:
            slot = slots[i] = self._make_slot(specs, dev)
        if self._free(slot):
            return self._hand_out(slot)
        return {n: (torch.zeros if z else torch.empty)(sh, dtype=dt, device=dev) for n, (sh, dt, z) in specs.items()}


def weights_go_cold(px16, K=None):
    return 1400 <= px16 < 4500 if K is None else 4800 <= px16 * (1 + K) < 18000


class Plan:
    def __init__(self, eng, touch=True, prio=True):
        self.eng = eng
        self.prio = prio
        self.dev = eng.device
        self.ol = O.OpList(scratch_owner=eng, touch_next_weights=touch, prio=prio)
        self.bufs = {}
        self.meta = {}
        self.tuned = False
        self.persistent = set()
        self.arena = None
        self._arena_slots = []
        self._arena_views = {}
        self._graphs = {}
        self.korder_ref = 0

    def buf(self, name, shape, dtype=BF16, persistent=False):
        assert name not in self.bufs, name
        t = torch.zeros(tuple(int(s) for s in shape), dtype=dtype, device=self.dev)
        self.bufs[name] = t
        if persistent:
            self.persistent.add(name)
        return t

    def pack_into(self, arena):
        arr = self.ol.finalize()
        ptrs = arr['p'].astype(np.int64)
        items = []
        for name, t in self.bufs.items():
            if name in self.persistent or t.numel() == 0:
                continue
            base, nbytes = t.data_ptr(), t.numel() * t.element_size()
            hit = (ptrs >= base) & (ptrs < base + nbytes)
            if not hit.any():
                continue
            rows = np.nonzero(hit.any(axis=1))[0]
            items.append(dict(name=name, base=base, nbytes=nbytes, first=int(rows[0]), last=int(rows[-1]), hit=hit, t=t))
        items.sort(key=lambda b: (b['first'], -b['nbytes']))
        placed = []
        total = 0
        for b in items:
            size = -(-b['nbytes'] // ARENA_ALIGN) * ARENA_ALIGN
            live = sorted((o, e) for (o, e, last) in placed if last >= b['first'])
            off = 0
            for o, e in live:
                if off + size <= o:
                    break
                off = max(off, e)
            b['off'] = off
            placed.append((off, off + size, b['last']))
            total = max(total, off + size)
        self.arena = arena
        self._arena_slots = []
        for b in items:
            idx, slot = np.nonzero(b['hit'])
            for i, sl in zip(idx, slot):
                self._arena_slots.append((int(i), int(sl), b['off'] + int(ptrs[i, sl] - b['base'])))
            self._arena_views[b['name']] = (b['off'], tuple(b['t'].shape), b['t'].dtype)
        self.ol.keep = [k for k in self.ol.keep if not any(k is b['t'] for b in items)]
        arena.plans.append(self)
        arena.require(total)
        self.rebind_arena()
        self.meta['arena_bytes'] = total
        self.meta['unpacked_bytes'] = sum(b['nbytes'] for b in items)

    def rebind_arena(self):
        if self.arena is None or self.arena.tensor is None:
            return
        base = self.arena.base()
        p = self.ol.arr['p']
        for (i, sl, off) in self._arena_slots:
            p[i, sl] = base + off
            self.ol.recs[i][4][sl] = base + off
        for name, (off, shape, dtype) in self._arena_views.items():
            n = int(np.prod(shape)) * torch.empty((), dtype=dtype).element_size()
            self.bufs[name] = self.arena.tensor[off:off + n].view(dtype).view(shape)

    graph_head = 0

    def run(self, **dyn):
        if not self.tuned:
            self.tuned = True
            self.autotune_convs(**dyn)
        if ARENA_POISON and self.arena is not None and self.arena.tensor is not None:
            self.arena.tensor.fill_(0xFF)
        ol = self.ol
        ex = _lib.get_executor()
        if GRAPHS and len(ol.recs) >= GRAPH_MIN_OPS and hasattr(ex, 'run_cached'):
            if ol.arr is None:
                ol.finalize()
            if dyn:
                ol.bind(**dyn)
            ex.run_cached(ol.arr, self._graphs, self.graph_head)
        else:
            ol.run(**dyn)

    def run_part(self, lo, hi, first=True, **dyn):
        if not self.tuned:
            self.tuned = True
            self.autotune_convs(**dyn)
        if first and ARENA_POISON and self.arena is not None and self.arena.tensor is not None:
            self.arena.tensor.fill_(0xFF)
        ol = self.ol
        if ol.arr is None:
            ol.finalize()
        if dyn:
            ol.bind(**dyn)
        _lib.get_executor().run(ol.arr[lo:hi])

    def autotune_convs(self, **dyn):
        from .. import _lib
        ex = _lib.get_executor()
        ex = getattr(ex, 'ex', ex)
        if ex.is_mock or not hasattr(ex, 'time_ops'):
            return
        ol = self.ol
        if ol.arr is None:
            ol.finalize()
        ol.bind(**dyn)
        arr = ol.arr
        cache = self.eng.tile_cache
        tuned_any = False
        for n in range(len(arr)):
            if arr['kind'][n] != O.CONV:
                continue
            i = arr['i'][n]
            M, cout, cin = int(i[0]) * int(i[7]) * int(i[8]), int(i[9]), int(i[3]) + int(i[4])
            key = (M, cout, cin, int(i[11]), int(i[13]), int(arr['flags'][n]) & 3, int(i[1]), int(i[2]))
            best = cache.get(key)
            twin = self.korder_ref and int(i[0]) % self.korder_ref == 0
            if twin:
                Bk = self.korder_ref
                key1 = (M // Bk,) + key[1:]
                ref = cache.get(key1) or (O.COUT1_TILE if (int(i[17]) == O.COUT1_TILE) else
                                          O.pick_tile(M // Bk, cout, cin, dict(kh=int(i[11]), c2=int(i[4]))), 1)
                want = O.korder_class(*ref)
                if isinstance(want, str) and cache.get(key + (want,)) is not None:
                    best = cache[key + (want,)]
                if best is None or O.korder_class(*best) != want:
                    best = (int(i[17]), 1) if O.korder_class(int(i[17]), int(i[19])) == want else tuple(ref)
                assert O.korder_class(*best) == want, (key, best, ref)
            if best is None and not getattr(self.eng, 'autotune', AUTOTUNE):
                continue
            if best is None:
                one = arr[n:n + 1].copy()
                best, best_t = (int(i[17]), 1), None
                cands = O.tile_candidates(M, cout, cin, int(i[16]),
                                          geom=dict(kh=int(i[11]), stride=int(i[13]), pad=int(i[14]), W=int(i[2]), c2=int(i[4])))
                if int(i[4]) or arr['p'][n, 4]:
                    cands = [t for t in cands if t != O.COUT1_TILE]
                for t in cands:
                    for sk in O.splitk_candidates(M, cout, int(i[16]), t):
                        one['i'][0, 17], one['i'][0, 19] = t, sk
                        ms = min(ex.time_ops(one, TUNE_ITERS) for _ in range(TUNE_REPS))
                        if best_t is None or ms < best_t:
                            best, best_t = (t, sk), ms
                cache[key] = best
                tuned_any = True
            apply = True
            if (best[0] in O.DMA_TILES or best[0] in O.PC_TILES) and not O.dma_tiles_enabled():
                apply = False
            if (arr['p'][n, 7] or arr['p'][n, 8]) and best[0] not in O.DMA_TILES and best[0] not in O.PC_TILES:
                apply = False
            if apply:
                arr['i'][n, 17], arr['i'][n, 19] = best
            if twin:
                assert O.korder_class(int(arr['i'][n, 17]), int(arr['i'][n, 19])) == want, (key, int(arr['i'][n, 17]), int(arr['i'][n, 19]), want)
        ol.wire_next_weights()
        self.tuned = True
        if tuned_any:
            save_tile_cache(cache)

    def conv(self, wname, x, *, name=None, out=None, stride=1, pad=None, x2=None, res=None, res_bcast=False,
             relu_in=False, act=O.ACT_NONE, out_f32=False, ldy=None, gap_acc=None, zero=None, persistent=False, res_group=None):
        w = self.eng.w[wname]
        if pad is None:
            pad = (w.kh - 1) // 2
        OH = (x.H + 2 * pad - w.kh) // stride + 1
        OW = (x.W + 2 * pad - w.kw) // stride + 1
        if out is None:
            t = self.buf(name or wname, (x.B, OH, OW, w.cout), F32 if out_f32 else BF16, persistent=persistent)
            out = Act(t, x.B, OH, OW, w.cout, w.cout if ldy is None else ldy)
        else:
            assert out.B == x.B and out.H == OH and out.W == OW and out.C == w.cout, (wname, out.B, out.H, out.W, out.C, OH, OW, w.cout)
        if res is not None:
            assert res.C == w.cout and res.H == OH and res.W == OW
        self.ol.conv(x.t, w, out.t, B=x.B, H=x.H, W=x.W, C1=x.C, ldx1=x.ld, OH=OH, OW=OW, ldy=out.ld, stride=stride,
                     pad=pad, x2=None if x2 is None else x2.t, C2=0 if x2 is None else x2.C,
                     ldx2=0 if x2 is None else x2.ld, res=None if res is None else res.t,
                     ldr=0 if res is None else res.ld, res_bcast=res_bcast, relu_in=relu_in, act=act, out_f32=out_f32,
                     gap_acc=gap_acc, zero=zero, prio=self.prio, res_group=res_group)
        return out

    def ca_block(self, prefix, x, name, out=None, head=None):
        if head is not None:
            head = (self.eng.w[head[0]], head[1])
        w = self.eng.w[prefix + '.conv2']
        gap = self.buf(name + '.gap', (x.B, x.C), F32)
        HW = x.H * x.W
        if O.conv_side_jobs_ok(cin=x.C, cout=w.cout, kh=w.kh):
            sums = self.buf(name + '.gapsum', (x.B, x.C), torch.int64)
            t1 = self.conv(prefix + '.conv1', x, name=name + '.t1', relu_in=True, act=O.ACT_RELU, zero=sums)
            t2 = self.conv(prefix + '.conv2', t1, name=name + '.t2', gap_acc=sums)
            if out is None:
                out = Act(self.buf(name + '.out', (x.B, x.H, x.W, x.C)), x.B, x.H, x.W, x.C)
            self.ol.eca_apply(t2.t, gap, self.eng.w[prefix + '.conv.weight'], x.t, out.t, B=x.B, HW=HW, C=x.C, fixed_sums=sums, head=head)
            return out
        t1 = self.conv(prefix + '.conv1', x, name=name + '.t1', relu_in=True, act=O.ACT_RELU)
        t2 = self.conv(prefix + '.conv2', t1, name=name + '.t2')
        self.ol.gap(t2.t, gap, B=x.B, HW=HW, C=x.C, partial_only=True)
        if out is None:
            out = Act(self.buf(name + '.out', (x.B, x.H, x.W, x.C)), x.B, x.H, x.W, x.C)
        self.ol.eca_apply(t2.t, gap, self.eng.w[prefix + '.conv.weight'], x.t, out.t, B=x.B, HW=HW, C=x.C, head=head)
        return out

    def fusion_block(self, prefix, x, g, name, out=None, xt=None, xt_group=None):
        if xt is None:
            xt = self.conv(prefix + '.distributor.x_transform', x, name=name + '.xt')
        g0 = self.conv(prefix + '.distributor.g_transform', g, name=name + '.g0', res=xt, res_bcast=True, res_group=xt_group)
        g1 = self.ca_block(prefix + '.block1', g0, name + '.b1')
        return self.ca_block(prefix + '.block2', g1, name + '.b2', out=out)

    def resnet(self, prefix, x, taps=None):
        bottleneck, layers = resnet_layers(self.eng.m, prefix)
        feats = {}
        for (lname, planes, nb, lstride) in layers:
            for bi in range(nb):
                p = f'{prefix}.{lname}.{bi}'
                s = lstride if bi == 0 else 1
                last = bi == nb - 1
                out = taps.get(lname) if (taps and last) else None
                if bottleneck:
                    t1 = self.conv(p + '.conv1', x, act=O.ACT_RELU)
                    t2 = self.conv(p + '.conv2', t1, stride=s, act=O.ACT_RELU)
                    r = self.conv(p + '.downsample.0', x, stride=s) if (p + '.downsample.0') in self.eng.w else x
                    x = self.conv(p + '.conv3', t2, res=r, act=O.ACT_RELU, out=out)
                else:
                    t1 = self.conv(p + '.conv1', x, stride=s, act=O.ACT_RELU)
                    r = self.conv(p + '.downsample.0', x, stride=s) if (p + '.downsample.0') in self.eng.w else x
                    x = self.conv(p + '.conv2', t1, res=r, act=O.ACT_RELU, out=out)
            feats[lname] = x
        return x, feats


def stem_ok(eng, name):
    w = eng.w.get(name)
    return w is not None and w.cout == 64 and w.kh == 7 and w.kw == 7 and w.cin_padded == 8 and w.bias is not None


def build_encode(eng, h0, w0, H, W, pad_left, pad_top, B=1, qrows=64):
    P = Plan(eng, touch=weights_go_cold(B * (H // 16) * (W // 16)), prio=False)
    m = eng.m
    img = (lambda b: Dyn('image')) if B == 1 else (lambda b: Dyn('image%d' % b))
    if stem_ok(eng, 'pixel_encoder.conv1'):
        pool = P.buf('pool', (B, H // 4, W // 4, 64))
        SM = O.OpList.STEM_MAX_IMAGES
        for b0 in range(0, B, SM):
            P.ol.stem(img(b0), None, eng.w['pixel_encoder.conv1'], pool[b0:], h0=h0, w0=w0, H=H, W=W, pad_left=pad_left, pad_top=pad_top, K=1,
                      mean=m['pixel_mean'], std=m['pixel_std'], relu=True, more_images=[img(b) for b in range(b0 + 1, min(B, b0 + SM))])
        x = Act(pool, B, H // 4, W // 4, 64)
    else:
        img8 = P.buf('img8', (B, H, W, 8))
        for b in range(B):
            P.ol.img_prep(img(b), None, img8[b], h0=h0, w0=w0, H=H, W=W, pad_left=pad_left, pad_top=pad_top, K=1,
                          mean=m['pixel_mean'], std=m['pixel_std'])
        x = P.conv('pixel_encoder.conv1', Act(img8, B, H, W, 8), stride=2, pad=3, act=O.ACT_RELU)
        pool = P.buf('pool', (B, x.H // 2, x.W // 2, 64))
        P.ol.maxpool(x.t, pool, B=B, H=x.H, W=x.W, C=64)
        x = Act(pool, B, x.H // 2, x.W // 2, 64)
    h4, w4, h8, w8, h, w = H // 4, W // 4, H // 8, W // 8, H // 16, W // 16
    ms = m['pixel_encoder']['ms_dims']
    taps = {'res2': Act(Dyn('f4'), B, h4, w4, ms[2]), 'layer2': Act(Dyn('f8'), B, h8, w8, ms[1]),
            'layer3': Act(Dyn('f16'), B, h, w, ms[0])}
    f16, _ = P.resnet('pixel_encoder', x, taps)
    pix = P.conv('pix_feat_proj', f16, out=Act(Dyn('pix_feat'), B, h, w, m['pixel_dim']))
    build_key_ops(P, f16, h, w, qrows)
    W_ = eng.w
    for wname, src, dname in (('mask_decoder.decoder_feat_proc.transforms.0', taps['layer2'], 'f8p'),
                              ('mask_decoder.decoder_feat_proc.transforms.1', taps['res2'], 'f4p'),
                              ('pixel_fuser.fuser.distributor.x_transform', pix, 'fuse_xt')):
        P.conv(wname, src, out=Act(Dyn(dname), B, src.H, src.W, W_[wname].cout))
    P.meta.update(h=h, w=w, B=B)
    if B > 1:
        P.korder_ref = B
    return P


def build_key_ops(P, f16, h, w, qrows=64):
    m = P.eng.m
    CK = m['key_dim']
    B = f16.B
    kx = P.conv('key_proj.pix_feat_proj', f16, name='keyx')
    P.conv('key_proj.key_proj', kx, out=Act(Dyn('key'), B, h, w, CK), out_f32=True)
    P.conv('key_proj.d_proj', kx, out=Act(Dyn('shr'), B, h, w, 1), out_f32=True, act=O.ACT_SQ1)
    P.conv('key_proj.e_proj', kx, out=Act(Dyn('sel'), B, h, w, CK), out_f32=True, act=O.ACT_SIGMOID)
    hw, HWp = h * w, -(-h * w // qrows) * qrows
    for b in range(B):
        P.ol.key_prep(Dyn('key', b * hw * CK * 4), Dyn('sel', b * hw * CK * 4), Dyn('Bhi', b * HWp * 128 * 2), Dyn('Blo', b * HWp * 128 * 2),
                      Dyn('cq', b * HWp * 4), n=hw, query=True)


def build_transform_key(eng, h, w):
    P = Plan(eng)
    build_key_ops(P, Act(Dyn('f16'), 1, h, w, eng.m['pixel_encoder']['ms_dims'][0]), h, w)
    return P


def build_pixel_fusion(eng, K, h, w, pre=False, pre_md=False, clips=1, wstride=1, stacked=False):
    G, Kc = clips, K
    K = G * Kc
    assert G == 1 or pre, 'clips in lock step take x_transform(pix_feat) from the encoder plan'
    P = Plan(eng, touch=weights_go_cold(h * w, K))
    m = eng.m
    if pre_md:
        pair = eng.mask_down_bufs(K, h, w, G)[0]
        P.ol.keep.append(pair)
    else:
        pair = P.buf('pair', (K, h, w, 64), persistent=True)
        m16 = P.buf('m16', (K, h, w), F32)
        for c in range(G):
            P.ol.mask_down(Dyn('last_mask' if G == 1 else 'last_mask%d' % c), pair[c * Kc:], m16[c * Kc:], K=Kc, H=16 * h, W=16 * w, pair_channels=64)
    if G > 1 and not stacked:
        px = P.buf('pixel_all', (K, h, w, m['value_dim']))
        nb = Kc * h * w * m['value_dim'] * 2
        P.ol.bank_write([(Dyn('pixel%d' % c), px[c * Kc:], nb) for c in range(G)])
        pixel = Act(px, K, h, w, m['value_dim'])
    else:
        pixel = Act(Dyn('pixel'), K, h, w, m['value_dim'])
    p16 = P.conv('pixel_fuser.sensory_compress', Act(Dyn('sensory_bf16'), K, h, w, m['sensory_dim']),
                 x2=Act(pair, K, h, w, 64), res=pixel, name='p16')
    xt = Act(Dyn('fuse_xt'), G, h, w, eng.w['pixel_fuser.fuser.distributor.x_transform'].cout) if pre else None
    P.fusion_block('pixel_fuser.fuser', Act(Dyn('pix_feat'), 1, h, w, m['pixel_dim']), p16, 'fuse',
                   out=Act(Dyn('fused'), K, h, w, m['embed_dim']), xt=xt, xt_group=(Kc, wstride * h * w) if G > 1 else None)
    if G > 1:
        P.korder_ref = G
    return P


def build_readout_query(eng, K, h, w, last_aux=True, fresh=True, clips=1):
    G, Kc = clips, K
    K = G * Kc
    P = Plan(eng, touch=weights_go_cold(h * w, K))
    if G > 1:
        P.korder_ref = G
    m, ol, W = eng.m, P.ol, eng.w
    ot = m['object_transformer']
    C, Q, heads, nb = m['embed_dim'], ot['num_queries'], ot['num_heads'], ot['num_blocks']
    HW, M = h * w, K * Q
    t = 'object_transformer'
    f = lambda name, shape: P.buf(name, shape, F32)
    query, query_emb = eng.query_bufs(K)
    use_chain = C == 256 and Q == 16 and heads == 8 and HW <= 24576 and ot['ff_dim'] % 64 == 0
    assert G == 1 or use_chain, 'clips in lock step need the chain form of the query side'
    qacc = P.buf('qacc', (3 * nb, M, C), torch.int64) if use_chain else None
    zero_on_conv = None
    if C == 256 and Q == 16:
        if fresh or not use_chain:
            ol.query_init2(Dyn('obj_mem'), query, query_emb, rows=M, w_init=W[t + '.summary_to_query_init'], res_init=eng.rep_embedding('query_init', K),
                           w_emb=W[t + '.summary_to_query_emb'], res_emb=eng.rep_embedding('query_emb', K), zero=qacc)
        elif O.conv_side_jobs_ok(cin=C, cout=C, kh=1):
            zero_on_conv = qacc
        else:
            ol.memset32(qacc, 2 * qacc.numel(), 0)
    else:
        vals = f('vals', (M, C))
        ol.query_init(Dyn('obj_mem'), vals, rows=M, C=C)
        ol.linear(vals, W[t + '.summary_to_query_init'], query, M=M, res=eng.rep_embedding('query_init', K))
        ol.linear(vals, W[t + '.summary_to_query_emb'], query_emb, M=M, res=eng.rep_embedding('query_emb', K))
    pix_in = Act(Dyn('pixel'), K, h, w, C)
    pixel = P.conv(t + '.pixel_init_proj', pix_in, name='pixel_init', zero=zero_on_conv)
    aux = P.buf('aux_logits', (nb + 1, K, HW), F32, persistent=True)
    fused_mask = HW <= 24576
    fg = None if fused_mask else P.buf('fg', (K, HW), torch.uint8)
    nfg = None if fused_mask else P.buf('nfg', (K,), torch.int32)
    P.conv(t + '.mask_pred.0.1', pixel, relu_in=True, out_f32=True, out=Act(aux[0], K, h, w, 1))
    if not fused_mask:
        ol.aux_mask(aux[0], fg, nfg, K=K, HW=HW)
    x = query
    prev_acc = q_pre = xn_next = None
    for b in range(nb):
        q = f'{t}.blocks.{b}'
        n = f'b{b}.'
        kvq = P.conv(q + '.pixel_proj_x', pixel, x2=pix_in, name=n + 'kvq', res=Act(eng.pe_rb(h, w, b), 1, h, w, 3 * C), res_bcast=True)
        ln = lambda name: (W[q + name + '.weight'], W[q + name + '.bias'])
        xn = xn_next if xn_next is not None else f(n + 'xn', (M, C))
        xn_next = None
        fuse_proj = fused_mask and C == 256
        chain = fuse_proj and use_chain
        if chain:
            Wo1, Wo2 = W[q + '.read_from_pixel.out'], W[q + '.self_attn.out']
            W1, W2 = W[q + '.ffn.linear1'], W[q + '.ffn.linear2']
            a1, a2, a3 = qacc[3 * b], qacc[3 * b + 1], qacc[3 * b + 2]
            if q_pre is not None:
                ol.attn_q2p(None, kvq.t, None, None, None, K=K, Q=Q, HW=HW, C=C, heads=heads, ldkv=3 * C, voff=C, logits=aux[b],
                            q_pre=q_pre, out_proj=(Wo1, a1), clip_objects=Kc)
            else:
                ol.attn_q2p(None, kvq.t, None, None, None, K=K, Q=Q, HW=HW, C=C, heads=heads, ldkv=3 * C, voff=C, logits=aux[b],
                            proj=dict(x=x, W=W[q + '.read_from_pixel.q'], emb=query_emb, ln=ln('.read_from_pixel.norm'), ln_out=xn),
                            acc_in=prev_acc, out_proj=(Wo1, a1), clip_objects=Kc)
            y = f(n + 'y', (M, C))
            ol.attn_self(None, None, None, K=K, Q=Q, C=C, heads=heads,
                         proj=dict(x=xn, W=W[q + '.self_attn.qkv'], emb=query_emb, ln=ln('.self_attn.norm'), ln_out=y),
                         acc_in=(a1, Wo1.bias), out_proj=(Wo2, a2))
            x2 = f(n + 'x2', (M, C))
            ol.qffn(y, x2, a3, rows=M, ln=ln('.ffn.norm'), W1=W1, W2=W2, acc_in=(a2, Wo2.bias), hid_slice=64)
            x = x2
            prev_acc = (a3, W2.bias)
            next_q = None
            if b + 1 < nb:
                qn = f'{t}.blocks.{b + 1}'
                q_pre, xn_next = f(f'b{b + 1}.q', (M, C)), f(f'b{b + 1}.xn', (M, C))
                next_q = dict(ln=(W[qn + '.read_from_pixel.norm.weight'], W[qn + '.read_from_pixel.norm.bias']), W=W[qn + '.read_from_pixel.q'],
                              q_out=q_pre, xn_out=xn_next)
            else:
                q_pre = None
            pa = P.buf(n + 'pa', (K, h, w, C))
            ol.attn_p2q(kvq.t.view(-1)[2 * C:], None, None, pa, K=K, Q=Q, HW=HW, C=C, heads=heads, ldq=3 * C,
                        proj=dict(x=x, W=W[q + '.read_from_query.kv'], emb=query_emb), acc_in=prev_acc, next_q=next_q)
        else:
            att = f(n + 'att', (M, C))
            if fuse_proj:
                ol.attn_q2p(None, kvq.t, None, None, att, K=K, Q=Q, HW=HW, C=C, heads=heads, ldkv=3 * C, voff=C, logits=aux[b],
                            proj=dict(x=x, W=W[q + '.read_from_pixel.q'], emb=query_emb, ln=ln('.read_from_pixel.norm'), ln_out=xn))
            else:
                qp = f(n + 'qp', (M, C))
                ol.linear(x, W[q + '.read_from_pixel.q'], qp, M=M, x_add=query_emb, add_rows=M, ln=ln('.read_from_pixel.norm'), ln_out=xn)
                ol.attn_q2p(qp, kvq.t, fg, nfg, att, K=K, Q=Q, HW=HW, C=C, heads=heads, ldkv=3 * C, voff=C, logits=aux[b] if fused_mask else None)
            x1 = f(n + 'x1', (M, C))
            ol.linear(att, W[q + '.read_from_pixel.out'], x1, M=M, res=xn)
            y = f(n + 'y', (M, C))
            sa = f(n + 'sa', (M, C))
            if fuse_proj:
                ol.attn_self(None, None, sa, K=K, Q=Q, C=C, heads=heads,
                             proj=dict(x=x1, W=W[q + '.self_attn.qkv'], emb=query_emb, ln=ln('.self_attn.norm'), ln_out=y))
            else:
                qkv = f(n + 'qkv', (M, 3 * C))
                ol.linear(x1, W[q + '.self_attn.qkv'], qkv, M=M, x_add=query_emb, add_rows=M, add_cols=2 * C, ln=ln('.self_attn.norm'), ln_out=y)
                ol.attn_self(qkv, qkv.view(-1)[2 * C:], sa, K=K, Q=Q, C=C, heads=heads, ldqk=3 * C, ldv=3 * C)
            x2 = f(n + 'x2', (M, C))
            ol.linear(sa, W[q + '.self_attn.out'], x2, M=M, res=y)
            hid = f(n + 'hid', (M, ot['ff_dim']))
            ol.linear(x2, W[q + '.ffn.linear1'], hid, M=M, relu=True, ln=ln('.ffn.norm'))
            x3 = f(n + 'x3', (M, C))
            ol.linear(hid, W[q + '.ffn.linear2'], x3, M=M, res=x2)
            x = x3
            pa = P.buf(n + 'pa', (K, h, w, C))
            if fuse_proj:
                ol.attn_p2q(kvq.t.view(-1)[2 * C:], None, None, pa, K=K, Q=Q, HW=HW, C=C, heads=heads, ldq=3 * C,
                            proj=dict(x=x, W=W[q + '.read_from_query.kv'], emb=query_emb))
            else:
                kv2 = f(n + 'kv2', (M, 2 * C))
                ol.linear(x, W[q + '.read_from_query.kv'], kv2, M=M, x_add=query_emb, add_rows=M, add_cols=C)
                ol.attn_p2q(kvq.t.view(-1)[2 * C:], kv2, kv2.view(-1)[C:], pa, K=K, Q=Q, HW=HW, C=C, heads=heads, ldq=3 * C, ldkv=2 * C)
        pf = P.conv(q + '.read_from_query.out', Act(pa, K, h, w, C), name=n + 'pf', res=pixel)
        last = b == nb - 1
        want_aux = not last or last_aux
        fuse_head = want_aux and C == 256
        pixel = P.ca_block(q + '.pixel_ffn.conv', pf, n + 'ffn', out=Act(Dyn('out'), K, h, w, C) if last else None,
                           head=(f'{t}.mask_pred.{b + 1}.1', aux[b + 1]) if fuse_head else None)
        if want_aux and not fuse_head:
            P.conv(f'{t}.mask_pred.{b + 1}.1', pixel, relu_in=True, out_f32=True, out=Act(aux[b + 1], K, h, w, 1))
        if not last and not fused_mask:
            ol.aux_mask(aux[b + 1], fg, nfg, K=K, HW=HW)
    return P


def build_segment(eng, K, h, w, update_sensory, pre=False, md=False, clips=1, wstride=1):
    G, Kc = clips, K
    K = G * Kc
    assert G == 1 or (pre and Kc + 1 <= 8), 'clips in lock step: image-only decoder convs from the encoder plan, <= 7 objects per clip'
    P = Plan(eng, touch=weights_go_cold(h * w, K))
    if G > 1:
        P.korder_ref = G
    m, ol = eng.m, P.ol
    up = m['mask_decoder']['up_dims']
    ms = m['pixel_encoder']['ms_dims']
    CS = m['sensory_dim']
    h8, w8, h4, w4 = 2 * h, 2 * w, 4 * h, 4 * w
    if pre:
        f8p, f4p = Act(Dyn('f8p'), G, h8, w8, up[0]), Act(Dyn('f4p'), G, h4, w4, up[1])
    else:
        f8p = P.conv('mask_decoder.decoder_feat_proc.transforms.0', Act(Dyn('f8'), 1, h8, w8, ms[1]), name='f8p')
        f4p = P.conv('mask_decoder.decoder_feat_proc.transforms.1', Act(Dyn('f4'), 1, h4, w4, ms[2]), name='f4p')
    p16 = Act(Dyn('p16'), K, h, w, up[0])
    u8 = P.buf('u8', (K, h8, w8, up[0]))
    ol.upsample2x_add(p16.t, f8p.t, u8, B=K, h=h, w=w, C=up[0], skip_group=(Kc, wstride * h8 * w8) if G > 1 else None)
    u8 = Act(u8, K, h8, w8, up[0])
    t1 = P.conv('mask_decoder.up_16_8.out_conv.conv1', u8, relu_in=True, act=O.ACT_RELU)
    ds = P.conv('mask_decoder.up_16_8.out_conv.downsample', u8)
    p8 = P.conv('mask_decoder.up_16_8.out_conv.conv2', t1, res=ds, name='p8')
    u4 = P.buf('u4', (K, h4, w4, up[1]))
    ol.upsample2x_add(p8.t, f4p.t, u4, B=K, h=h8, w=w8, C=up[1], skip_group=(Kc, wstride * h4 * w4) if G > 1 else None)
    u4 = Act(u4, K, h4, w4, up[1])
    t2 = P.conv('mask_decoder.up_8_4.out_conv.conv1', u4, relu_in=True, act=O.ACT_RELU)
    p4 = P.conv('mask_decoder.up_8_4.out_conv.conv2', t2, res=u4, name='p4')
    logits = P.buf('logits', (K, h4, w4), F32)
    P.conv('mask_decoder.pred', p4, relu_in=True, out_f32=True, out=Act(logits, K, h4, w4, 1))
    P.meta['logits_done'] = len(ol.recs)
    if update_sensory:
        CT = up[1] + up[2] + 64
        gcat = P.buf('gcat', (K, h, w, CT), persistent=True)
        ol.area_down3([dict(x=p8.t, y=gcat, B=K, H=h8, W=w8, C=up[1], ldx=up[1], ldy=CT, r=2),
                       dict(x=p4.t, y=gcat.view(-1)[up[1]:], B=K, H=h4, W=w4, C=up[2], ldx=up[2], ldy=CT, r=4),
                       dict(x=logits, y=gcat.view(-1)[up[1] + up[2]:], B=K, H=h4, W=w4, C=1, ldx=1, ldy=CT, r=4, f32_in=True, Cz=8)])
        g3 = P.conv('mask_decoder.sensory_update.g_all', p16, x2=Act(gcat, K, h, w, CT), name='g3')
        vals = P.conv('mask_decoder.sensory_update.transform', g3, x2=Act(Dyn('sensory_bf16'), K, h, w, CS),
                      out_f32=True, name='gru_vals')
        ol.gru(vals.t, Dyn('sensory_f32'), Dyn('sensory_bf16'), n=K * h * w, C=CS)
    if Kc + 1 <= 16:
        ol.up4_softmax(logits, Dyn('prob'), Dyn('logits_up'), P=Kc + 1, h=h4, w=w4, from_logits=True, clips=G,
                       mask_down=(eng.mask_down_bufs(K, h, w, G)[1], eng.mask_down_bufs(K, h, w, G)[0], 64) if md else None)
    else:
        agg = P.buf('agg', (K + 1, h4, w4), F32)
        ol.seg_agg(logits, agg, K=K, hw=h4 * w4)
        ol.up4_softmax(agg, Dyn('prob'), Dyn('logits_up'), P=K + 1, h=h4, w=w4)
    return P


def build_encode_mask(eng, K, h0, w0, H, W, pad_left, pad_top, deep_update=True, pre_md=False, clips=1, wstride=1):
    G, Kc = clips, K
    K = G * Kc
    P = Plan(eng, touch=weights_go_cold((H // 16) * (W // 16), K))
    if G > 1:
        P.korder_ref = G
    m, ol = eng.m, P.ol
    h, w = H // 16, W // 16
    CV, CS, CE, Q = m['value_dim'], m['sensory_dim'], m['embed_dim'], m['object_summarizer']['num_summaries']
    masks_of = (lambda c: Dyn('masks')) if G == 1 else (lambda c: Dyn('masks', 4 * (c * (Kc + 1) + 1) * H * W))
    assert G == 1 or stem_ok(eng, 'mask_encoder.conv1')
    if stem_ok(eng, 'mask_encoder.conv1'):
        pool = P.buf('pool', (K, H // 4, W // 4, 64))
        iname = lambda c: Dyn('image' if G == 1 else 'image%d' % c)
        SM = O.OpList.STEM_MAX_IMAGES
        for c0 in range(0, G, SM):
            ol.stem(iname(c0), masks_of(c0), eng.w['mask_encoder.conv1'], pool[c0 * Kc:], h0=h0, w0=w0, H=H, W=W, pad_left=pad_left, pad_top=pad_top,
                    K=Kc, mean=m['pixel_mean'], std=m['pixel_std'], relu=True, more_images=[iname(c) for c in range(c0 + 1, min(G, c0 + SM))],
                    mask_stride=(Kc + 1) * H * W)
    else:
# ... 43 lines not shown
```

### cutie_amd/ops.py

```python
import os

import numpy as np
import torch

from . import _lib

NI, NF, NP = 24, 6, 16
OP_DTYPE = np.dtype([('kind', '<i4'), ('flags', '<i4'), ('i', '<i4', (NI,)), ('f', '<f4', (NF,)), ('p', '<u8', (NP,))])
assert OP_DTYPE.itemsize == _lib.OP_STRUCT_SIZE

(CONV, MAXPOOL, IMG_PREP, UPSAMPLE2X_ADD, AREA_DOWN, MASK_DOWN, GAP, ECA_APPLY, GRU, SEG_AGG, UP4_SOFTMAX,
 MASK_MERGE, AGG_SOFTMAX, LINEAR, LAYERNORM, QUERY_INIT, AUX_MASK, ATTN_Q2P, ATTN_SELF, ATTN_P2Q, SUMMARIZE,
 ADD_PE, KEY_PREP, AFF_SCORE, AFF_SELECT, AFF_READOUT, MEMSET32, COPY2D, AXPY, USAGE_TICK, RANK_SELECT,
 GATHER_ROWS, CONSOL_AFF, CONSOL_READ, CAST, PROB_TO_ID, RESIZE, FLIP_W, AREA_DOWN3, QFFN, STEM, BANK_WRITE) = range(1, 43)

KIND_NAMES = {}
for _n in ('CONV MAXPOOL IMG_PREP UPSAMPLE2X_ADD AREA_DOWN MASK_DOWN GAP ECA_APPLY GRU SEG_AGG UP4_SOFTMAX MASK_MERGE '
           'AGG_SOFTMAX LINEAR LAYERNORM QUERY_INIT AUX_MASK ATTN_Q2P ATTN_SELF ATTN_P2Q SUMMARIZE ADD_PE KEY_PREP '
           'AFF_SCORE AFF_SELECT AFF_READOUT MEMSET32 COPY2D AXPY USAGE_TICK RANK_SELECT GATHER_ROWS CONSOL_AFF '
           'CONSOL_READ CAST PROB_TO_ID RESIZE FLIP_W AREA_DOWN3 QFFN STEM').split():
    KIND_NAMES[globals()[_n]] = _n

F_RELU_IN, F_OUT_F32, F_RES_BCAST = 1, 2, 4
F_PRIO, F_AFF_PRIO = 256, 64
F_TILE_OFF = 128 if os.environ.get('CUTIE_AMD_COUT1_TILE', '1') in ('', '0') else 0
ACT_NONE, ACT_RELU, ACT_SIGMOID, ACT_SQ1 = 0, 1, 2, 3
ACT_SHIFT = 4
AREA_RT = 8 if os.environ.get('CUTIE_AMD_AREA_R', '1') in ('', '0') else 0
GRU_SCALAR = 1 if os.environ.get('CUTIE_AMD_GRU4', '1') in ('', '0') else 0
KEYPREP_LOOP = 2 if os.environ.get('CUTIE_AMD_KEYPREP_LOOP', '0') not in ('', '0') else 0
UP4_LANES = 16 if os.environ.get('CUTIE_AMD_UP4_SHARED', '1') in ('', '0') else 0
SELECT_COARSE = 2 if os.environ.get('CUTIE_AMD_SELECT_FINE', '1') in ('', '0') else 0
UP4_RTK = 8 if os.environ.get('CUTIE_AMD_UP4_KC', '1') in ('', '0') else 0

TILES = {0: (128, 128, 32), 1: (128, 64, 32), 2: (64, 64, 32), 3: (256, 16, 32), 4: (64, 128, 32),
         5: (64, 64, 64), 6: (64, 128, 64), 7: (128, 128, 64), 8: (64, 64, 128), 9: (32, 64, 64),
         10: (128, 64, 64), 11: (32, 64, 128), 12: (32, 128, 64),
         13: (64, 64, 64), 14: (128, 64, 64), 15: (64, 128, 64), 16: (128, 128, 64), 17: (64, 64, 128), 18: (128, 128, 32),
         20: (64, 64, 64), 21: (64, 64, 128), 22: (32, 64, 128), 23: (128, 64, 64), 24: (64, 128, 64), 25: (128, 128, 64),
         26: (32, 64, 64), 27: (64, 64, 64), 28: (32, 64, 64), 29: (64, 128, 32), 30: (64, 64, 32)}
TILE_WK = {20: 2, 21: 2, 22: 2, 23: 2, 24: 2, 25: 2, 26: 2, 27: 4, 28: 4, 29: 2, 30: 2}

DMA_TILES = {60: (128, 128, 64), 61: (128, 128, 64), 62: (128, 128, 64), 63: (128, 64, 64), 64: (64, 128, 64), 65: (64, 64, 64),
             66: (64, 64, 64), 67: (32, 64, 64), 68: (256, 128, 64), 69: (32, 128, 64), 70: (128, 128, 64), 71: (128, 64, 64),
             72: (64, 64, 64), 73: (64, 64, 64), 74: (64, 64, 64), 75: (32, 64, 64), 76: (128, 64, 64), 77: (64, 128, 64), 78: (32, 128, 64),
             80: (64, 64, 128), 81: (64, 64, 128), 82: (32, 64, 128), 83: (32, 64, 128), 84: (64, 128, 128), 85: (128, 64, 128),
             86: (96, 64, 64), 87: (96, 64, 64), 88: (64, 64, 64), 89: (64, 64, 64)}


PC_TILES = {100: (64, 64, 64), 101: (64, 64, 64), 102: (32, 64, 64), 103: (128, 64, 64), 104: (64, 128, 64), 105: (128, 128, 64),
            106: (128, 128, 64), 107: (64, 64, 64), 108: (128, 128, 64), 109: (32, 64, 64), 110: (96, 64, 64), 111: (96, 128, 64),
            120: (64, 64, 64), 121: (64, 64, 64), 122: (128, 64, 64), 123: (128, 128, 64), 124: (64, 128, 64), 125: (32, 64, 64),
            126: (128, 128, 64), 127: (64, 128, 64), 129: (96, 64, 64), 130: (32, 64, 64), 131: (64, 128, 64),
            132: (64, 64, 64), 133: (96, 128, 64), 134: (320, 64, 64),
            140: (64, 64, 64), 141: (96, 64, 64), 142: (96, 64, 64), 143: (32, 64, 64), 144: (128, 64, 64),
            145: (96, 64, 64), 146: (128, 64, 64), 147: (32, 64, 64)}
PC_HALO = {120: (8, 8), 121: (4, 16), 122: (8, 16), 123: (8, 16), 124: (8, 8), 125: (4, 8), 126: (8, 16), 127: (4, 16),
           129: (10, 9), 130: (5, 6), 131: (6, 9), 132: (6, 9), 133: (10, 9), 134: (20, 16),
           145: (10, 9), 146: (8, 16), 147: (5, 6)}

ALL_TILES = {**TILES, **DMA_TILES, **PC_TILES}


def korder_class(tile, splitk=1):
    if tile in PC_HALO:
        return 'halo'
    if tile in TILE_WK or splitk != 1:
        return ('split', tile, splitk)
    if tile in (3, COUT1_TILE):
        return ('small', tile)
    return 'stream' if (tile in DMA_TILES or tile in PC_TILES) else 'igemm'


def pc_tile_ok(tile, *, cin, kh, stride=1, pad=None, c2=0):
    if cin % 64 or (c2 and (c2 % 64 or (cin - c2) % 64)) or kh > 5:
        return False
    if tile in PC_HALO:
        return kh == 3 and stride == 1 and (pad is None or pad == 1)
    return True


def pc_blocks(tile, B, OH, OW, cout):
    bm, bn, _ = PC_TILES[tile]
    if tile in PC_HALO:
        th, tw = PC_HALO[tile]
        return B * -(-OH // th) * -(-OW // tw) * -(-cout // bn)
    return -(-(B * OH * OW) // bm) * -(-cout // bn)


def dma_tiles_enabled():
    return os.environ.get('CUTIE_AMD_DMA_TILES', '1') not in ('', '0')


def dma_tile_ok(tile, *, cin, kh, c2=0):
    bk = DMA_TILES[tile][2]
    return cin % bk == 0 and (c2 == 0 or (c2 % bk == 0 and (cin - c2) % bk == 0)) and kh * kh <= 32


def conv_side_jobs_ok(*, cin, cout, kh, c2=0):
    return dma_tiles_enabled() and dma_tile_ok(60, cin=cin, kh=kh, c2=c2) and cout % 8 == 0 and cout > 16


NUM_CU = 256
WEIGHT_PREFETCH = int(os.environ.get('CUTIE_AMD_WPF', str(8 << 20)))
WEIGHT_PREFETCH_BLOCK = int(os.environ.get('CUTIE_AMD_WPF_BLOCK', str(48 << 10)))


COUT1_TILE = 19


def cout1_ok(cout, cin, c2=0, res=False):
    lp = cin // 8
    return cout == 1 and c2 == 0 and not res and cin % 8 == 0 and 1 <= lp <= 64 and (lp & (lp - 1)) == 0


def tile_candidates(M, cout, cin, kpad=None, geom=None):
    if cout <= 16:
        return [3] + ([COUT1_TILE] if cout1_ok(cout, cin) else [])
    out = []
    for t, (bm, bn, bk) in TILES.items():
        if t == 3 or (bk > 32 and cin < 32):
            continue
        wk = TILE_WK.get(t, 1)
        if wk > 1 and (kpad is None or (kpad // bk) % wk or kpad // bk < 2 * wk):
            continue
        if bn == 128 and cout <= 64:
            continue
        if bm * 2 > max(M, 64) * 2 and bm > 64:
            continue
        out.append(t)
    if dma_tiles_enabled() and geom is not None and dma_tile_ok(60, cin=cin, kh=geom['kh'], c2=geom.get('c2', 0)):
        for t, (bm, bn, bk) in DMA_TILES.items():
            if not (bn == 128 and cout <= 64) and not (bm > 64 and bm > max(M, 64)) and not (bm == 256 and M < 16384) \
                    and dma_tile_ok(t, cin=cin, kh=geom['kh'], c2=geom.get('c2', 0)):
                out.append(t)
    if dma_tiles_enabled() and geom is not None:
        for t, (bm, bn, bk) in PC_TILES.items():
            if pc_tile_ok(t, cin=cin, kh=geom['kh'], stride=geom.get('stride', 1), pad=geom.get('pad'), c2=geom.get('c2', 0)) \
                    and not (bn == 128 and cout <= 64) and not (bm > 64 and bm > max(M, 64)) and not (bm == 256 and M < 16384):
                out.append(t)
    return out


SPLITK_PART_FLOATS = 16 << 20
_splitk_scratch = {}


def splitk_scratch(device, owner=None):
    dev = torch.device(device)
    store = _splitk_scratch if owner is None else owner.__dict__.setdefault('_splitk_part', {})
    key = str(dev)
    if key not in store:
        n = SPLITK_PART_FLOATS if dev.type == 'cuda' else 1024
        store[key] = torch.zeros(n, dtype=torch.float32, device=device)
    return store[key]


def splitk_candidates(M, cout, kpad, tile):
    if tile == COUT1_TILE or tile == 3 or tile in DMA_TILES or tile in PC_TILES:
        return [1]
    bm, bn, bk = TILES[tile]
    blocks = -(-M // bm) * -(-cout // bn)
    nk = kpad // bk // TILE_WK.get(tile, 1)
    ldp = (cout + 7) & ~7
    out = [1]
    for sk in (2, 3, 4, 6, 8, 9, 12, 16, 18):
        if blocks >= NUM_CU or blocks * sk > 6 * NUM_CU or nk // sk < 2:
            break
        if sk * M * ldp > SPLITK_PART_FLOATS:
            break
        if nk % sk == 0:
            out.append(sk)
    return out


def pick_tile(M, cout, cin=64, geom=None):
    if cout <= 16:
        return 3
    if geom is not None and dma_tiles_enabled() and dma_tile_ok(60, cin=cin, kh=geom['kh'], c2=geom.get('c2', 0)):
        cands = [t for t in (108, 103, 110, 101, 102) if pc_tile_ok(t, cin=cin, kh=geom['kh'], c2=geom.get('c2', 0))]
    else:
        cands = [6, 5, 9] if cin >= 32 else [4, 2]
    if cout <= 64:
        cands = [c for c in cands if ALL_TILES[c][1] <= 64] or [2]
    best, best_blocks = None, -1
    for t in cands:
        bm, bn, _ = ALL_TILES[t]
        blocks = -(-M // bm) * -(-cout // bn)
        if blocks >= NUM_CU:
            return t
        if blocks > best_blocks:
            best, best_blocks = t, blocks
    return best


def aa_taps(n_in, n_out):
    f32 = np.float32
    i = np.arange(n_out)
    if n_in == n_out:
        return i, np.ones(n_out, dtype=np.int64), np.ones((n_out, 1), dtype=f32)
    scale = f32(n_in) / f32(n_out)
    support = scale if scale >= 1 else f32(1.0)
    invscale = f32(1.0 / np.float64(scale)) if scale >= 1 else f32(1.0)
    max_taps = int(np.ceil(support)) * 2 + 1
    center = (np.float64(scale) * (i + 0.5)).astype(f32)
    first = np.maximum(((center - support).astype(np.float64) + 0.5).astype(np.int64), 0)
    count = np.minimum(((center + support).astype(np.float64) + 0.5).astype(np.int64), n_in) - first
    count = np.clip(count, 0, max_taps)
    j = np.arange(max_taps)
    pos = (first[:, None] + j[None, :]).astype(f32)
    arg = (((pos - center[:, None]).astype(np.float64) + 0.5) * np.float64(invscale)).astype(f32)
    arg = np.abs(arg)
    w = np.where(arg < 1, f32(1.0) - arg, f32(0.0)).astype(f32)
    w[j[None, :] >= count[:, None]] = 0
    total = np.zeros(n_out, dtype=f32)
    for k in range(max_taps):
        total = (total + w[:, k]).astype(f32)
    nz = total != 0
    w[nz] = (w[nz] / total[nz, None]).astype(f32)
    return first, count, w


def resize_aa_table(H, W, OH, OW):
    parts = [aa_taps(W, OW), aa_taps(H, OH)]
    K = max(int(w.shape[1]) for _, _, w in parts)
    tab = np.zeros((OW + OH, K + 2), dtype=np.int32)
    r = 0
    for first, count, w in parts:
        n = len(first)
        tab[r:r + n, 0], tab[r:r + n, 1] = first, count
        tab[r:r + n, 2:2 + w.shape[1]] = w.view(np.int32)
        r += n
    return tab


class Dyn:
    __slots__ = ('name', 'offset')

    def __init__(self, name, offset=0):
        self.name, self.offset = name, offset


def _ptr(t):
    if t is None:
        return 0
    if isinstance(t, int):
        return t
    return t.data_ptr()


JPEG_SYNC_ROUNDS = 4


class OpList:
    PRIO_KINDS = frozenset((UPSAMPLE2X_ADD, AREA_DOWN3, ECA_APPLY, GRU, UP4_SOFTMAX, ATTN_Q2P, ATTN_SELF, ATTN_P2Q, QFFN))

    def __init__(self, scratch_owner=None, touch_next_weights=True, prio=True):
        self.prio = prio
        self.scratch_owner = scratch_owner
        self.touch_next_weights = touch_next_weights
        self.recs = []
        self.keep = []
        self.wbytes = {}
        self.dyn = {}
        self.arr = None
        self._words = None

    def add(self, kind, flags=0, ints=(), floats=(), ptrs=()):
        idx = len(self.recs)
        if kind in self.PRIO_KINDS and self.prio:
            flags |= F_PRIO
        pl = []
        for slot, t in enumerate(ptrs):
            if isinstance(t, Dyn):
                self.dyn.setdefault(t.name, []).append((idx, slot, t.offset))
                pl.append(0)
            else:
                if isinstance(t, torch.Tensor):
                    self.keep.append(t)
                pl.append(_ptr(t))
        self.recs.append((kind, flags, [int(v) for v in ints], [float(v) for v in floats], pl))
        self.arr = self._words = None
        return idx

    def finalize(self):
        arr = np.zeros(len(self.recs), dtype=OP_DTYPE)
        for n, (kind, flags, ints, floats, ptrs) in enumerate(self.recs):
            arr['kind'][n] = kind
            arr['flags'][n] = flags
            arr['i'][n, :len(ints)] = ints
            arr['f'][n, :len(floats)] = floats
            arr['p'][n, :len(ptrs)] = ptrs
        self.arr = arr
        self._words = None
        self.wire_next_weights()
        return arr

    def wire_next_weights(self):
        arr = self.arr
        convs = [n for n in range(len(arr)) if arr['kind'][n] == CONV]
        for n in convs:
            arr['p'][n, 9:11] = 0
            arr['i'][n, 22:24] = 0
        if not (WEIGHT_PREFETCH and self.touch_next_weights):
            return
        nxt, nxt2 = None, None
        for n in reversed(convs):
            i = arr['i'][n]
            pc = int(i[17]) in PC_TILES
            if nxt is not None and pc:
                budget = WEIGHT_PREFETCH_BLOCK * -(-pc_blocks(int(i[17]), int(i[0]), int(i[7]), int(i[8]), int(i[9])) // 8)
                n1 = min(nxt[1], WEIGHT_PREFETCH, budget)
                arr['p'][n, 9], arr['i'][n, 22] = nxt[0], n1
                n2 = min(nxt2[1], WEIGHT_PREFETCH, budget - n1) if (nxt2 is not None and not nxt[2]) else 0
                if n2 > 0:
                    arr['p'][n, 10], arr['i'][n, 23] = nxt2[0], n2
            nxt, nxt2 = (int(arr['p'][n, 2]), self.wbytes[n], pc), nxt

    def patch_ints(self, op, start, values):
        values = [int(v) for v in values]
        ints = self.recs[op][2]
        end = start + len(values)
        if len(ints) < end:
            ints.extend([0] * (end - len(ints)))
        ints[start:end] = values
        if self.arr is not None:
            self.arr['i'][op, start:end] = values

    def bind(self, **tensors):
        if self.arr is None:
            self.finalize()
        words = self._words
        if words is None:
            assert OP_DTYPE.itemsize == 256 and OP_DTYPE.fields['p'][1] == 128
            words = self._words = ({name: tuple((idx * 32 + 16 + slot, off) for (idx, slot, off) in sl) for name, sl in self.dyn.items()},
                                   memoryview(self.arr).cast('B').cast('Q'))
        table, mv = words
        for name, t in tensors.items():
            sl = table.get(name)
            if sl is None:
                continue
            base = 0 if t is None else (t if type(t) is int else t.data_ptr())
            if base:
                for w, off in sl:
                    mv[w] = base + off
            else:
                for w, off in sl:
                    mv[w] = 0

    def run(self, _stream=None, **tensors):
        if self.arr is None:
            self.finalize()
        if tensors:
            self.bind(**tensors)
        ex = _lib.get_executor()
        if _stream is None:
            ex.run(self.arr)
        elif hasattr(ex, 'run_on'):
            ex.run_on(self.arr, _stream)
        else:
            with torch.cuda.stream(_stream):
                ex.run(self.arr)

    def __len__(self):
        return len(self.recs)

    def conv(self, x1, w, y, *, B, H, W, C1, ldx1, OH, OW, ldy, stride=1, pad=0, x2=None, C2=0, ldx2=0,
             res=None, ldr=0, res_bcast=False, relu_in=False, act=ACT_NONE, out_f32=False, tile=None, splitk=1,
             gap_acc=None, zero=None, prio=False, res_group=None):
        flags = (F_RELU_IN if relu_in else 0) | (F_OUT_F32 if out_f32 else 0) | (F_RES_BCAST if res_bcast else 0) | (act << ACT_SHIFT) | F_TILE_OFF | \
            (F_PRIO if prio else 0)
        assert C1 + C2 == w.cin_padded, (C1, C2, w.cin_padded)
        M = B * OH * OW
        side = gap_acc is not None or zero is not None
        if tile is None:
            tile = COUT1_TILE if (cout1_ok(w.cout, C1 + C2, C2, res is not None) and not side) else pick_tile(M, w.cout, C1 + C2, dict(kh=w.kh, c2=C2))
        if side:
            assert (tile in DMA_TILES or tile in PC_TILES) and not out_f32 and w.cout % 8 == 0 and ldy % 8 == 0, 'GAP accumulation needs an LDS-DMA conv (see conv_side_jobs_ok)'
        part = splitk_scratch(w.weight.device, self.scratch_owner)
        self.wbytes[len(self.recs)] = w.weight.numel() * w.weight.element_size()
        return self.add(CONV, flags,
                        [B, H, W, C1, C2, ldx1, ldx2, OH, OW, w.cout, ldy, w.kh, w.kw, stride, pad, ldr, w.kpad, tile, w.cin_real,
                         splitk, part.numel() // 1024, 0 if zero is None else zero.numel()],
                        self._res_group(res_group, res_bcast, B, OH * OW), [x1, x2, w.weight, w.bias, res, y, part, gap_acc, zero])

    @staticmethod
    def _res_group(res_group, res_bcast, B, OHW):
        if res_group is None:
            return []
        kg, stride = int(res_group[0]), int(res_group[1])
        assert res_bcast and kg > 0 and B % kg == 0 and stride >= OHW and stride < (1 << 24), (res_group, B, OHW)
        return [float(kg), float(stride)]

    def maxpool(self, x, y, *, B, H, W, C, relu=False):
        OH, OW = (H + 2 - 3) // 2 + 1, (W + 2 - 3) // 2 + 1
        return self.add(MAXPOOL, 1 if relu else 0, [B, H, W, C, OH, OW], [], [x, y])

    STEM_MAX_IMAGES = 12

    def stem(self, image, masks, w, y, *, h0, w0, H, W, pad_left, pad_top, K, mean, std, relu=True, more_images=(), mask_stride=0):
        assert w.cout == 64 and w.kh == 7 and w.cin_padded == 8 and H % 16 == 0 and W % 16 == 0
        more = list(more_images)
        assert len(more) < self.STEM_MAX_IMAGES
        ints = [h0, w0, H, W, pad_left, pad_top, K, w.kpad] + ([1 + len(more), int(mask_stride)] if more else [])
        return self.add(STEM, 1 if relu else 0, ints, list(mean) + list(std), [image, masks, w.weight, w.bias, y] + more)

    def img_prep(self, image, masks, y, *, h0, w0, H, W, pad_left, pad_top, K, mean, std):
        return self.add(IMG_PREP, 0, [h0, w0, H, W, pad_left, pad_top, K], list(mean) + list(std), [image, masks, y])

    def upsample2x_add(self, g, skip, y, *, B, h, w, C, skip_group=None):
        ints = [B, h, w, C]
        if skip_group is not None:
            kg, stride = int(skip_group[0]), int(skip_group[1])
            assert kg > 0 and B % kg == 0 and stride >= 4 * h * w
            ints += [kg, stride]
        return self.add(UPSAMPLE2X_ADD, 0, ints, [], [g, skip, y])

    def area_down(self, x, y, *, B, H, W, C, ldx, ldy, r, f32_in=False, Cz=None):
        return self.add(AREA_DOWN, 1 if f32_in else 0, [B, H, W, C, ldx, ldy, r, C if Cz is None else Cz], [], [x, y])

    def area_down3(self, segs):
        assert len(segs) == 3
        ints, ptrs, flags = [], [], 0
        for q, g in enumerate(segs):
            ints += [g['B'], g['H'], g['W'], g['C'], g['ldx'], g['ldy'], g['r'], g['C'] if g.get('Cz') is None else g['Cz']]
            ptrs += [g['x'], g['y']]
            flags |= (1 << q) if g.get('f32_in') else 0
        return self.add(AREA_DOWN3, flags | AREA_RT, ints, [], ptrs)

    def mask_down(self, masks, pair, m16, *, K, H, W, r=16, pair_channels=8):
        assert pair_channels % 8 == 0
        return self.add(MASK_DOWN, 0, [K, H, W, r, pair_channels], [], [masks, pair, m16])

    def gap(self, x, y, *, B, HW, C, scratch=None, partial_only=False):
        if scratch is None:
            scratch = torch.zeros((B, -(-HW // 64), C), dtype=torch.float32, device=y.device)
        self._last_gap_scratch = scratch
        return self.add(GAP, 1 if partial_only else 0, [B, HW, C], [], [x, y, scratch])

    def eca_apply(self, x, gap, wk, r, y, *, B, HW, C, part=None, fixed_sums=None, head=None):
        tail = []
        if head is not None:
            w, out = head
            assert C == 256 and w.cout == 1 and w.kh == 1 and w.cin_padded == 256
            tail = [w.weight, w.bias, out]
        if fixed_sums is not None:
            return self.add(ECA_APPLY, 1, [B, HW, C], [], [x, gap, wk, r, y, fixed_sums] + tail)
        if part is None:
            part = self._last_gap_scratch
        return self.add(ECA_APPLY, 0, [B, HW, C], [], [x, gap, wk, r, y, part] + tail)

    def gru(self, values, h, hb, *, n, C):
        return self.add(GRU, GRU_SCALAR, [n, C], [], [values, h, hb])

    def seg_agg(self, logits, agg, *, K, hw):
        return self.add(SEG_AGG, 0, [K, hw], [], [logits, agg])

    def up4_softmax(self, agg, prob, logits_up, *, P, h, w, from_logits=False, mask_down=None, clips=1):
        if mask_down is not None:
            assert from_logits and P <= 8 and h % 4 == 0 and w % 4 == 0
            m16, pair, pitch = mask_down
            return self.add(UP4_SOFTMAX, 1 | 4 | UP4_RTK | UP4_LANES, [P, h, w, pitch, clips], [], [agg, prob, logits_up, m16, pair])
        assert clips == 1 or (from_logits and P <= 8)
        return self.add(UP4_SOFTMAX, (1 | UP4_RTK) if from_logits else 0, [P, h, w, 0, clips], [], [agg, prob, logits_up])

    def mask_merge(self, inmask, pred, src, planes, *, h0, w0, H, W, pad_left, pad_top, Knew, Kold, nfloat, float_mode):
        return self.add(MASK_MERGE, 1 if float_mode else 0, [h0, w0, H, W, pad_left, pad_top, Knew, Kold, nfloat], [],
                        [inmask, pred, src, planes])

    def agg_softmax(self, planes, prob, *, K, HW):
        return self.add(AGG_SOFTMAX, 0, [K, HW], [], [planes, prob])

    def linear(self, x, w, y, *, M, ldx=None, ldy=None, x_add=None, add_rows=0, res=None, relu=False, add_cols=0,
               ln=None, ln_out=None, eps=1e-5):
        flags = (1 if relu else 0) | (2 if ln is not None else 0)
        return self.add(LINEAR, flags,
                        [M, w.n, w.kd, w.kd if ldx is None else ldx, w.n if ldy is None else ldy, add_rows, add_cols], [eps],
                        [x, x_add, w.weight, w.bias, res, y, ln[0] if ln else None, ln[1] if ln else None, ln_out])

    def layernorm(self, x, g, b, y, *, M, C):
        return self.add(LAYERNORM, 0, [M, C], [], [x, g, b, y])

    def query_init(self, obj_mem, y, *, rows, C):
        return self.add(QUERY_INIT, 0, [rows, C], [], [obj_mem, y])

    def query_init2(self, obj_mem, query, query_emb, *, rows, w_init, res_init, w_emb, res_emb, zero=None):
        assert w_init.kd == 256 and w_init.n == 256 and w_emb.kd == 256 and w_emb.n == 256 and rows % 16 == 0
        nz = 0
        if zero is not None:
            nb = zero.numel() * zero.element_size()
            assert nb % 16 == 0 and zero.is_contiguous()
            nz = nb // 16
        return self.add(QUERY_INIT, 1, [rows, 256, nz], [], [obj_mem, query, query_emb, w_init.weight, w_init.bias, res_init,
                                                             w_emb.weight, w_emb.bias, res_emb, zero])

    def aux_mask(self, logits, fg, nfg, *, K, HW):
        self.memset32(nfg, K, 0)
        return self.add(AUX_MASK, 0, [K, HW], [], [logits, fg, nfg])

    @staticmethod
    def _proj(proj):
        ln = proj.get('ln') or (None, None)
        assert proj['W'].kd == 256
        return proj.get('ldx', 256), proj.get('ln_out'), [proj['W'].weight, proj['W'].bias, proj.get('emb'), ln[0], ln[1]]

    QACC_SCALE = 4294967296.0

    @staticmethod
    def _proj_extras(flags, ints, ptrs, acc_in, out_proj):
        ints = list(ints) + [0] * (9 - len(ints))
        ptrs = list(ptrs) + [None] * (14 - len(ptrs))
        if acc_in is not None:
            assert acc_in[0].dtype == torch.int64
            flags |= 4
            ptrs[10], ptrs[11] = acc_in[0], acc_in[1]
        if out_proj is not None:
            assert out_proj[0].kd == 256 and out_proj[0].n == 256 and out_proj[1].dtype == torch.int64
            flags |= 8
            ptrs[12], ptrs[13] = out_proj[0].weight, out_proj[1]
        return flags, ints, ptrs

    def attn_q2p(self, q, kv, fg, nfg, y, *, K, Q, HW, C, heads, ldkv, voff, logits=None, proj=None, acc_in=None, out_proj=None, q_pre=None, hstride=None,
                 clip_objects=None):
        hs = 0 if hstride in (None, C // heads) else hstride
        kg = 0 if clip_objects in (None, K) else int(clip_objects)
        assert kg == 0 or (out_proj is not None and K % kg == 0), 'clips in lock step need the chain form'
        if q_pre is not None:
            assert proj is None and acc_in is None and out_proj is not None and logits is not None
            flags, ints, ptrs = self._proj_extras(3 | 16, [K, Q, HW, C, heads, ldkv, voff, 256], [q_pre, kv, logits, None, None], None, out_proj)
            ints[8] = hs
            return self.add(ATTN_Q2P, flags, ints + [kg], [], ptrs)
        if proj is not None:
            assert logits is not None
            ldx, ln_out, tail = self._proj(proj)
            assert out_proj is not None or acc_in is None, 'the chain form of ATTN_Q2P needs out_proj'
            flags, ints, ptrs = self._proj_extras(3, [K, Q, HW, C, heads, ldkv, voff, ldx], [proj['x'], kv, logits, ln_out, y] + tail, acc_in, out_proj)
            assert hs == 0 or out_proj is not None, 'a head stride needs the chain form'
            ints[8] = hs
            return self.add(ATTN_Q2P, flags, ints + [kg], [], ptrs)
        assert acc_in is None and out_proj is None
        if logits is not None:
            return self.add(ATTN_Q2P, 1, [K, Q, HW, C, heads, ldkv, voff], [], [q, kv, logits, None, y])
        return self.add(ATTN_Q2P, 0, [K, Q, HW, C, heads, ldkv, voff], [], [q, kv, fg, nfg, y])

    def attn_self(self, qk, v, y, *, K, Q, C, heads, ldqk=0, ldv=0, proj=None, acc_in=None, out_proj=None):
        if proj is not None:
            ldx, ln_out, tail = self._proj(proj)
            assert out_proj is not None or acc_in is None, 'the chain form of ATTN_SELF needs out_proj'
            flags, ints, ptrs = self._proj_extras(2, [K, Q, C, heads, 0, 0, ldx], [proj['x'], None, y, ln_out, None] + tail, acc_in, out_proj)
            return self.add(ATTN_SELF, flags, ints, [], ptrs)
        assert acc_in is None and out_proj is None
        return self.add(ATTN_SELF, 0, [K, Q, C, heads, ldqk, ldv], [], [qk, v, y])

    def attn_p2q(self, q, kq, vq, y, *, K, Q, HW, C, heads, ldq, ldkv=0, proj=None, acc_in=None, next_q=None, out=None):
        if proj is not None:
            ldx, _, tail = self._proj(proj)
            flags, ints, ptrs = self._proj_extras(2, [K, Q, HW, C, heads, ldq, ldkv, ldx], [q, proj['x'], None, y, None] + tail[:3], acc_in, None)
            if out is not None:
                assert acc_in is not None and out['Wo'].dtype == torch.uint8 and out['Wo'].numel() == 256 * 256 * 2 + 256 * 4
                flags |= 32
                ptrs[2], ptrs[4] = out['Wo'], out['res']
            if next_q is not None:
                assert acc_in is not None and next_q['W'].kd == 256 and next_q['W'].n == 256
                flags |= 16
                ptrs = ptrs + [None] * (16 - len(ptrs))
                ptrs[8], ptrs[9] = next_q['ln']
                ptrs[12], ptrs[13], ptrs[14], ptrs[15] = next_q['W'].weight, next_q['W'].bias, next_q['q_out'], next_q['xn_out']
            return self.add(ATTN_P2Q, flags, ints, [], ptrs)
        assert acc_in is None
        return self.add(ATTN_P2Q, 0, [K, Q, HW, C, heads, ldq, ldkv], [], [q, kq, vq, y])

    def qffn(self, x, x_out, acc_out, *, rows, ln, W1, W2, acc_in=None, hid_slice=64):
        FF = W1.n
        assert W1.kd == 256 and W2.kd == FF and W2.n == 256 and FF % hid_slice == 0 and hid_slice in (64, 128) and rows % 16 == 0
        assert acc_out.dtype == torch.int64
        ints = [rows, FF, hid_slice]
        ptrs = [x, x_out, ln[0], ln[1], W1.weight, W1.bias, W2.weight, acc_out] + [None] * 6
        if acc_in is not None:
            assert acc_in[0].dtype == torch.int64
            ptrs[10], ptrs[11] = acc_in[0], acc_in[1]
        return self.add(QFFN, 0, ints, [], ptrs)

    def summarize(self, feat, wl, m16, y, *, K, HW, C, Q, scratch=None, feat_f32=False, ldf=None, ldw=None):
        if scratch is None:
            scratch = torch.zeros((K, -(-HW // 128), Q, C + 1), dtype=torch.float32, device=m16.device)
        return self.add(SUMMARIZE, 1 if feat_f32 else 0, [K, HW, C, Q, C if ldf is None else ldf, Q if ldw is None else ldw], [], [feat, wl, m16, y, scratch])

    def add_pe(self, x, pe, y, *, B, n):
        return self.add(ADD_PE, 0, [B, n], [], [x, pe, y])

    def key_prep(self, key, aux, hi, lo, sc, *, n, query):
        return self.add(KEY_PREP, (1 | KEYPREP_LOOP) if query else 0, [n], [], [key, aux, hi, lo, sc])

    AFF_CSTRIDE = 32

    def aff_score(self, Ahi, Alo, scale, Bhi, Blo, c, out, cand_val, cand_idx, count, *, HW, HWp, ranges, cap, mode, gmax_precedes_tau=False, nq=None, dma=None,
                  frames=1, extra_lds_kb=0, prio=False, banks=None):
        ranges = [(s, n) for (s, n) in ranges if n > 0]
        assert 1 <= len(ranges) <= 3
        G = sum(-(-n // 16) for _, n in ranges)
        ints = [HW, HWp, len(ranges)]
        for r in range(3):
            ints += list(ranges[r]) if r < len(ranges) else [0, 0]
        ints += [G, cap, mode, 2 if nq is None else nq, 0, int(extra_lds_kb), int(bool(dma))]
        if frames > 1:
            ints[1] = frames * HWp
            ints += [HWp]
        ptrs = [Ahi, Alo, scale, Bhi, Blo, c, out, cand_val, cand_idx, count]
        flags = (1 if (gmax_precedes_tau and mode == 1) else 0) | (F_AFF_PRIO if prio else 0)
        if banks is not None:
            assert frames > 1 and frames % banks[1] == 0 and ints[12] == 2 and HWp % 128 == 0
            ints += [banks[1]]
            ptrs += [None, banks[0]]
            flags |= 4
        return self.add(AFF_SCORE, flags, ints, [], ptrs)

    def aff_select(self, gmax, tau, *, HW, HWp, G, top_k, clear_count=None, ticks=(), zero=None, frames=1, prio=False):
        if zero is not None:
            assert not ticks
            return self.add(AFF_SELECT, 1 | SELECT_COARSE | (F_AFF_PRIO if prio else 0), [HW, HWp, G, top_k, zero[1], 0, frames], [], [gmax, tau, clear_count, zero[0], None])
        ticks = list(ticks) + [(None, 0)] * (2 - len(ticks))
        assert len(ticks) == 2
        return self.add(AFF_SELECT, SELECT_COARSE | (F_AFF_PRIO if prio else 0), [HW, HWp, G, top_k, ticks[0][1], ticks[1][1], frames], [], [gmax, tau, clear_count, ticks[0][0], ticks[1][0]])

    def aff_readout(self, cand_val, cand_idx, count, vptrs, usage, y, overflow, *, HW, cap, top_k, K, CV, frames=1, HWp=0, usage_stride=0, prio=False, banks=1, usage_fx=False):
        assert banks == 1 or frames % banks == 0
        return self.add(AFF_READOUT, (F_AFF_PRIO if prio else 0) | (1 if usage_fx else 0), [HW, cap, top_k, K, CV, frames, HWp, usage_stride, banks], [], [cand_val, cand_idx, count, vptrs, usage, y, overflow])

    def memset32(self, dst, n, value=0):
        return self.add(MEMSET32, 0, [n, value], [], [dst])

    def bank_write(self, copies=(), fills=()):
        copies, fills = list(copies), list(fills)
        idx = None
        while copies or fills:
            c, copies = copies[:6], copies[6:]
            fl, fills = fills[:2], fills[2:]
            ints, ptrs = [0] * 10, [0] * 14
            for s, (src, dst, nbytes) in enumerate(c):
                assert nbytes % 4 == 0 and nbytes > 0
                ints[s], ptrs[2 * s], ptrs[2 * s + 1] = nbytes // 4, src, dst
            for t, (dst, words, pattern) in enumerate(fl):
                ints[6 + t], ints[8 + t], ptrs[12 + t] = words, pattern, dst
            idx = self.add(BANK_WRITE, 0, ints, [], ptrs)
        return idx

    def copy2d(self, src, dst, *, rows, rowbytes, src_stride, dst_stride):
        assert rowbytes % 4 == 0 and src_stride % 4 == 0 and dst_stride % 4 == 0
        return self.add(COPY2D, 0, [rows, rowbytes, src_stride, dst_stride], [], [src, dst])

    def axpy(self, x, y, *, n, a=1.0):
        return self.add(AXPY, 0, [n], [a], [x, y])

    def usage_tick(self, life, n, life2=None, n2=0, use=None, delta=None, n_use=0, delta_fx=False, clear_delta=False):
        assert delta_fx or not clear_delta
        return self.add(USAGE_TICK, (1 if delta_fx else 0) | (2 if clear_delta else 0), [n, n2, n_use], [], [life, life2, use, delta])

    RS_SPLIT = 16

    def rank_select(self, use, life, order, *, n, k, scratch=None, gathers=(), zero=None):
        if scratch is None:
            scratch = torch.empty((self.RS_SPLIT * n,), dtype=torch.int32, device=use.device)
            self.keep.append(scratch)
        gathers = list(gathers) + [(None, None, 0)] * (2 - len(gathers))
        assert len(gathers) == 2 and all(g[2] % 16 == 0 for g in gathers)
        z = zero if zero is not None else (None, 0)
        return self.add(RANK_SELECT, 0, [n, k, gathers[0][2] // 4, gathers[1][2] // 4, z[1]], [],
                        [use, life, order, scratch, gathers[0][0], gathers[0][1], gathers[1][0], gathers[1][1], z[0]])

    def gather_rows(self, src, order, dst, *, k, rowbytes, src_stride, dst_stride):
        return self.add(GATHER_ROWS, 0, [k, rowbytes, src_stride, dst_stride], [], [src, order, dst])

    @staticmethod
    def consol_lds(n):
# ... 303 lines not shown
```

### include/cutie_hip.h

```cpp
#ifndef CUTIE_HIP_H
#define CUTIE_HIP_H

#include <stdint.h>

#ifdef __cplusplus
extern "C" {
#endif

#define CUTIE_OP_NI 24
#define CUTIE_OP_NF 6
#define CUTIE_OP_NP 16
#define CUTIE_MERGE_MAX_SOURCES 8
#define CUTIE_JF_MAX_RADIUS 40

typedef struct cutie_op {
    int32_t kind;
    int32_t flags;
    int32_t i[CUTIE_OP_NI];
    float f[CUTIE_OP_NF];
    uint64_t p[CUTIE_OP_NP];
} cutie_op;

#define CUTIE_F_RELU_IN   1
#define CUTIE_F_OUT_F32   2
#define CUTIE_F_RES_BCAST 4
#define CUTIE_F_PLAIN     8
#define CUTIE_F_TILE_OFF  128
#define CUTIE_F_PRIO      256
#define CUTIE_ACT_SHIFT   4
#define CUTIE_ACT_NONE    0
#define CUTIE_ACT_RELU    1
#define CUTIE_ACT_SIGMOID 2
#define CUTIE_ACT_SQ1     3

enum {
    CUTIE_OP_CONV = 1,
    CUTIE_OP_MAXPOOL = 2,
    CUTIE_OP_IMG_PREP = 3,
    CUTIE_OP_UPSAMPLE2X_ADD = 4,
    CUTIE_OP_AREA_DOWN = 5,
    CUTIE_OP_MASK_DOWN = 6,
    CUTIE_OP_GAP = 7,
    CUTIE_OP_ECA_APPLY = 8,
    CUTIE_OP_GRU = 9,
    CUTIE_OP_SEG_AGG = 10,
    CUTIE_OP_UP4_SOFTMAX = 11,
    CUTIE_OP_MASK_MERGE = 12,
    CUTIE_OP_AGG_SOFTMAX = 13,
    CUTIE_OP_LINEAR = 14,
    CUTIE_OP_LAYERNORM = 15,
    CUTIE_OP_QUERY_INIT = 16,
    CUTIE_OP_AUX_MASK = 17,
    CUTIE_OP_ATTN_Q2P = 18,
    CUTIE_OP_ATTN_SELF = 19,
    CUTIE_OP_ATTN_P2Q = 20,
    CUTIE_OP_SUMMARIZE = 21,
    CUTIE_OP_ADD_PE = 22,
    CUTIE_OP_KEY_PREP = 23,
    CUTIE_OP_AFF_SCORE = 24,
    CUTIE_OP_AFF_SELECT = 25,
    CUTIE_OP_AFF_READOUT = 26,
    CUTIE_OP_MEMSET32 = 27,
    CUTIE_OP_COPY2D = 28,
    CUTIE_OP_AXPY = 29,
    CUTIE_OP_USAGE_TICK = 30,
    CUTIE_OP_RANK_SELECT = 31,
    CUTIE_OP_GATHER_ROWS = 32,
    CUTIE_OP_CONSOL_AFF = 33,
    CUTIE_OP_CONSOL_READ = 34,
    CUTIE_OP_CAST = 35,
    CUTIE_OP_PROB_TO_ID = 36,
    CUTIE_OP_RESIZE = 37,
    CUTIE_OP_FLIP_W = 38,
    CUTIE_OP_AREA_DOWN3 = 39,
    CUTIE_OP_QFFN = 40,
    CUTIE_OP_STEM = 41,
    CUTIE_OP_BANK_WRITE = 42,
    CUTIE_OP__COUNT
};

int cutie_exec(const cutie_op* ops, int n, void* stream);
int cutie_exec_one(const cutie_op* op, void* stream);
void* cutie_graph_capture(const cutie_op* ops, int n, void* stream);
int cutie_graph_launch(void* graph, void* stream);
void cutie_graph_destroy(void* graph);
float cutie_time_ops(const cutie_op* ops, int n, int iters, void* stream);
const char* cutie_hip_last_error(void);
int cutie_hip_abi_version(void);
int cutie_op_struct_size(void);
int cutie_hip_build_flags(void);

#ifdef __cplusplus
}
#endif
#endif
```

Measured before the change: 1166.

## Fuse ResNet bottleneck conv2 and conv3 into one back-to-back conv kernel

Adds a back-to-back conv kernel that computes the 3x3 conv2 tile and keeps its output in LDS as the input for the 1x1 conv3 GEMM, with producer waves streaming conv2 inputs and conv3 weights through LDS DMA rings. The executor fuses a conv flagged FUSE_NEXT with the op that follows it. The planner moves the downsample conv ahead of conv2 so that conv2 and conv3 sit next to each other, and extends buffer lifetimes to match. This removes the global write and re-read of the intermediate activation and one kernel launch per bottleneck. The cost is a larger LDS footprint and lower occupancy, plus possible register pressure and a fallback path when fusion is not accepted.

```diff
diff --git a/cutie_amd/_lib.py b/cutie_amd/_lib.py
--- a/cutie_amd/_lib.py
+++ b/cutie_amd/_lib.py
@@ -57,6 +57,10 @@
 
 def has_png_decode():
     return bool(load().cutie_hip_build_flags() & 2)
+
+
+def has_conv_b2b():
+    return bool(load().cutie_hip_build_flags() & 16)
 
 
 class HipExecutor:
diff --git a/cutie_amd/csrc/api.hip b/cutie_amd/csrc/api.hip
--- a/cutie_amd/csrc/api.hip
+++ b/cutie_amd/csrc/api.hip
@@ -1,4 +1,4 @@
-#include "common.h"
+#include "conv_common.h"
 #include <stdarg.h>
 #include <stdio.h>
 #include <string.h>
@@ -38,7 +38,14 @@
 int cutie_exec(const cutie_op* ops, int n, void* stream) {
     hipStream_t s = (hipStream_t)stream;
     for (int k = 0; k < n; ++k) {
-        int rc = dispatch(&ops[k], s);
+        int rc, fused = 0;
+        if (ops[k].kind == CUTIE_OP_CONV && (ops[k].flags & CUTIE_F_FUSE_NEXT) && k + 1 < n) {
+            rc = launch_conv_b2b(&ops[k], &ops[k + 1], s, &fused);
+            if (rc == 0 && fused) { ++k; continue; }
+            if (rc == 0) rc = dispatch(&ops[k], s);
+        } else {
+            rc = dispatch(&ops[k], s);
+        }
         if (rc != 0) {
             if (rc > 0) cutie_set_error("op %d (kind %d): HIP error %d (%s)", k, ops[k].kind, rc, hipGetErrorString((hipError_t)rc));
             else {
@@ -127,7 +134,7 @@
 int cutie_hip_abi_version(void) { return 11; }
 int cutie_op_struct_size(void) { return (int)sizeof(cutie_op); }
 int cutie_hip_build_flags(void) {
-    const int forms = 2;
+    const int forms = 2 | 16;
 #ifdef CUTIE_DIAG
     return forms | 1;
 #else
diff --git a/cutie_amd/csrc/conv_b2b.hip b/cutie_amd/csrc/conv_b2b.hip
--- /dev/null
+++ b/cutie_amd/csrc/conv_b2b.hip
@@ -0,0 +1,377 @@
+#include "conv_pc_common.h"
+
+template <int BM, int CMID, int BN2, int NS, int NS2, bool W2SEP>
+constexpr int b2b_w2_base() {
+    return W2SEP ? NS * (BM + CMID) * 128 : BM * CMID * 2;
+}
+template <int BM, int CMID, int BN2, int NS, int NS2, bool W2SEP>
+constexpr int b2b_lds_bytes() {
+    constexpr int ring = NS * (BM + CMID) * 128, w2end = b2b_w2_base<BM, CMID, BN2, NS, NS2, W2SEP>() + NS2 * BN2 * 128;
+    return ring > w2end ? ring : w2end;
+}
+
+template <int BM, int CMID, int NPW, int WM1, int WN1, int WM2, int WN2, int BN2, int NS, int NS2, bool W2SEP>
+__global__ __launch_bounds__((WM1 * WN1 + NPW) * 64) void conv_b2b_kernel(ConvParams p, ConvParams q) {
+#if __HIP_DEVICE_COMPILE__
+    if (p.flags & CUTIE_F_PRIO) __builtin_amdgcn_s_setprio(1);
+    constexpr int NC = WM1 * WN1;
+    constexpr int TM1 = BM / WM1 / 16, TN1 = CMID / WN1 / 16, TM2 = BM / WM2 / 16, TN2 = BN2 / WN2 / 16;
+    constexpr int TNP1 = TN1 / 2, TNP2 = TN2 / 2;
+    constexpr int NXI = BM / 8 / NPW, NWI = CMID / 8 / NPW, LPT = NXI + NWI, NWI2 = BN2 / 8 / NPW;
+    constexpr int STAGE = (BM + CMID) * 128, RING = NS * STAGE;
+    constexpr int KS2 = CMID / 64, A2SLICE = BM * 128, W2STAGE = BN2 * 128;
+    constexpr int W2BASE = b2b_w2_base<BM, CMID, BN2, NS, NS2, W2SEP>();
+    constexpr bool W2_EARLY = W2SEP;
+    static_assert(WM2 * WN2 == NC && TM1 >= 1 && TM2 >= 1 && TN1 >= 2 && TN2 >= 2 && TN1 % 2 == 0 && TN2 % 2 == 0, "bad wave grid");
+    static_assert(BM % (WM1 * 16) == 0 && BM % (WM2 * 16) == 0 && CMID % (WN1 * 32) == 0 && BN2 % (WN2 * 32) == 0, "bad tile");
+    static_assert(NXI >= 1 && NXI <= 4 && NWI >= 1 && NWI <= 4 && NWI2 >= 1 && NXI * 8 * NPW == BM && NS >= 3 && NS2 >= 3, "pieces per producer wave");
+    static_assert(W2BASE >= BM * CMID * 2, "the stage-2 weight ring must not meet the hand-over tile");
+    extern __shared__ __attribute__((aligned(16))) u32x4 b2b_smem[];
+    char* const lds = reinterpret_cast<char*>(b2b_smem);
+    const int tid = threadIdx.x, lane = tid & 63, l15 = lane & 15, l4 = lane >> 4;
+    const int wave = __builtin_amdgcn_readfirstlane(tid >> 6);
+    conv_preload_args(p);
+    const int nb = gridDim.x;
+    int logical;
+    {
+        const int id = blockIdx.x;
+        const int xcd = id & 7, kq = id >> 3, qq = nb >> 3, r = nb & 7;
+        logical = (xcd < r ? xcd * (qq + 1) : r * (qq + 1) + (xcd - r) * qq) + kq;
+    }
+    const int m0 = logical * BM;
+    const int nk1 = p.KH * p.KW * (p.Cin / 64);
+    const int nk2 = (q.Cout / BN2) * KS2;
+
+    if (wave >= NC) {
+        const int pw = wave - NC;
+        const int lr = lane >> 3;
+        const unsigned kcb = (unsigned)(((lane & 7) ^ lr) * 16);
+        constexpr unsigned PRE = 4096;
+        unsigned woff[NWI];
+#pragma unroll
+        for (int i = 0; i < NWI; ++i)
+            woff[i] = (unsigned)(pc_wrow((pw * NWI + i) * 8 + lr, true) * p.Kpad * 2) + kcb + PRE - (unsigned)i * 1024u;
+        const rsrc_t rw = pc_rsrc(reinterpret_cast<const char*>(p.w) - PRE);
+        const int wdst = BM * 128 + pw * NWI * 1024;
+        const int cin2 = p.Cin * 2;
+        unsigned wsoff = 0;
+        int ldw = 0;
+#define B2B_WPIECE(I, LD)                                                                                      \
+    if constexpr ((I) < NWI) PC_DMA(rw, LDS_PTR(lds + (LD) + wdst), 16, woff[(I) < NWI ? (I) : 0], wsoff, (I) * 1024, 0);
+#define B2B_LOAD_W(LD) { B2B_WPIECE(0, LD) B2B_WPIECE(1, LD) B2B_WPIECE(2, LD) B2B_WPIECE(3, LD) wsoff += 128; }
+#pragma unroll
+        for (int s = 0; s < NS - 1; ++s) { B2B_LOAD_W(ldw) ldw += STAGE; }
+        unsigned xoff1[NXI], vmask[NXI];
+        {
+            int m = m0 + pw * NXI * 8 + lr;
+            const int mm = m < p.M ? m : p.M - 1;
+            int b = pc_div(mm, p.OHW, __builtin_amdgcn_rcpf((float)p.OHW));
+            const int rem = mm - b * p.OHW;
+            int oh = pc_div(rem, p.OW, __builtin_amdgcn_rcpf((float)p.OW));
+            int ow = rem - oh * p.OW;
+#pragma unroll
+            for (int i = 0; i < NXI; ++i) {
+                const int ih0 = oh * p.stride, iw0 = ow * p.stride;
+                const unsigned pix = (unsigned)((b * p.H + ih0) * p.W + iw0);
+                xoff1[i] = pix * (unsigned)(p.ldx1 * 2) + kcb + PRE - (unsigned)i * 1024u;
+                unsigned mk = 0, cols = 0;
+                for (int k = 0; k < p.KW; ++k) cols |= ((unsigned)(iw0 - p.pad + k) < (unsigned)p.W) ? (1u << k) : 0u;
+                for (int k = 0; k < p.KH; ++k) mk |= ((unsigned)(ih0 - p.pad + k) < (unsigned)p.H) ? (cols << (k * p.KW)) : 0u;
+                vmask[i] = mk;
+                if (i + 1 < NXI) {
+                    m += 8;
+                    if (m < p.M) {
+                        ow += 8;
+                        while (ow >= p.OW) { ow -= p.OW; ++oh; }
+                        while (oh >= p.OH) { oh -= p.OH; ++b; }
+                    }
+                }
+            }
+        }
+        const long shift = (long)p.pad * p.W + p.pad;
+        const rsrc_t rx1 = pc_rsrc(reinterpret_cast<const char*>(p.x1 - shift * p.ldx1) - PRE);
+        const int xdst = pw * NXI * 1024;
+        int tap = 0, kw = 0, cc = 0, pixA = 0;
+        const int stepA1 = p.ldx1 * 2, stepA2 = (p.W - p.KW + 1) * p.ldx1 * 2;
+#define B2B_XPIECE(I, LD)                                                                                      \
+    if constexpr ((I) < NXI)                                                                                   \
+        PC_DMA(rx1, LDS_PTR(lds + (LD) + xdst), 16, (vmask[(I) < NXI ? (I) : 0] & tapbit_) ? xoff1[(I) < NXI ? (I) : 0] : PC_OOB, soff_, (I) * 1024, 0);
+#define B2B_LOAD_X(LD)                                                                                         \
+    {                                                                                                          \
+        const unsigned tapbit_ = 1u << tap;                                                                    \
+        const unsigned soff_ = (unsigned)(pixA + cc);                                                          \
+        B2B_XPIECE(0, LD) B2B_XPIECE(1, LD) B2B_XPIECE(2, LD) B2B_XPIECE(3, LD)                                \
+        cc += 128;                                                                                             \
+        const bool wrap_ = cc >= cin2;                                                                         \
+        cc = wrap_ ? 0 : cc;                                                                                   \
+        tap += wrap_ ? 1 : 0;                                                                                  \
+        kw += wrap_ ? 1 : 0;                                                                                   \
+        const bool wrap2_ = kw == p.KW;                                                                        \
+        kw = wrap2_ ? 0 : kw;                                                                                  \
+        pixA += wrap_ ? (wrap2_ ? stepA2 : stepA1) : 0;                                                        \
+    }
+        int ld = 0;
+#pragma unroll
+        for (int s = 0; s < NS - 1; ++s) { B2B_LOAD_X(ld) ld += STAGE; }
+        if (NS == 3) { PC_WAIT_VM((NS - 2) * NXI); } else { PC_WAIT_VM(0); }
+        PC_BARRIER()
+        int kt = 0;
+        for (; kt < nk1 - (NS - 1); ++kt) {
+            B2B_LOAD_X(ld) B2B_LOAD_W(ld)
+            PC_WAIT_VM((NS - 2) * LPT);
+            PC_BARRIER()
+            ld = ld == (NS - 1) * STAGE ? 0 : ld + STAGE;
+        }
+#undef B2B_LOAD_X
+#undef B2B_XPIECE
+#undef B2B_LOAD_W
+#undef B2B_WPIECE
+        unsigned woff2[NWI2];
+#pragma unroll
+        for (int i = 0; i < NWI2; ++i) woff2[i] = (unsigned)(pc_wrow((pw * NWI2 + i) * 8 + lr, true) * q.Kpad * 2) + kcb;
+        const rsrc_t rw2 = pc_rsrc(q.w);
+        const unsigned chunk2 = (unsigned)(BN2 * q.Kpad * 2);
+        unsigned w2so = 0, w2chunk = 0;
+        int w2ks = 0, w2ld = 0;
+#define B2B_W2TILE()                                                                                           \
+    {                                                                                                          \
+        _Pragma("unroll") for (int i = 0; i < NWI2; ++i)                                                       \
+            PC_DMA(rw2, LDS_PTR(lds + W2BASE + w2ld + (pw * NWI2 + i) * 1024), 16, woff2[i], w2chunk + w2so, 0, 0); \
+        w2ld = w2ld == (NS2 - 1) * W2STAGE ? 0 : w2ld + W2STAGE;                                               \
+        ++w2ks; w2so += 128;                                                                                   \
+        if (w2ks == KS2) { w2ks = 0; w2so = 0; w2chunk += chunk2; }                                            \
+    }
+        if (W2_EARLY) {
+#pragma unroll
+            for (int s = 0; s < NS2 - 1; ++s) B2B_W2TILE()
+        }
+        for (; kt < nk1; ++kt) {
+            PC_WAIT_VM(0);
+            PC_BARRIER()
+        }
+        if (!W2_EARLY) {
+#pragma unroll
+            for (int s = 0; s < NS2 - 1; ++s) B2B_W2TILE()
+        }
+        PC_WAIT_VM((NS2 - 2) * NWI2);
+        PC_BARRIER()
+        for (int t = 0; t < nk2; ++t) {
+            if (t + NS2 - 1 < nk2) {
+                B2B_W2TILE()
+                PC_WAIT_VM((NS2 - 2) * NWI2);
+            } else {
+                PC_WAIT_VM(0);
+            }
+            PC_BARRIER()
+        }
+#undef B2B_W2TILE
+        if (q.pf_bytes > 0) {
+            const int id = blockIdx.x;
+            const int nbx = (nb + 7) >> 3, kq = id >> 3;
+            u32x4 t = {0u, 0u, 0u, 0u};
+#pragma unroll
+            for (int r = 0; r < 2; ++r) {
+                const unsigned char* base = r ? q.pf2 : q.pf;
+                const int bytes = r ? q.pf2_bytes : q.pf_bytes;
+                const int chunk = (((bytes + nbx - 1) / nbx) + 1023) & ~1023;
+                const int b0 = kq * chunk, b1 = min(b0 + chunk, bytes & ~15);
+                for (int o = b0 + (pw * 64 + lane) * 16; o < b1; o += NPW * 1024)
+                    asm volatile("global_load_dwordx4 %0, %1, off" : "+v"(t) : "v"(base + o) : "memory");
+            }
+            asm volatile("s_waitcnt vmcnt(0)" : "+v"(t) :: "memory");
+        }
+        return;
+    }
+
+    typedef const __attribute__((address_space(1))) float* pc_gf32;
+    const int c0 = l4 << 4, c1 = (4 + l4) << 4;
+    const int swl = (l15 & 7) << 4;
+#define B2B_MFMA(AF, BF, ACC) ACC = __builtin_amdgcn_mfma_f32_16x16x32_bf16(AF, BF, ACC, 0, 0, 0)
+    {
+        const int pm0 = (wave / WN1) * (BM / WM1), cn0 = (wave % WN1) * (CMID / WN1);
+        float bias[TNP1][8];
+        const pc_gf32 bias_g = (pc_gf32)p.bias;
+#pragma unroll
+        for (int a = 0; a < TNP1; ++a)
+#pragma unroll
+            for (int r = 0; r < 8; ++r) bias[a][r] = bias_g[cn0 + a * 32 + l4 * 8 + r];
+        const int rdw0 = BM * 128 + (cn0 + l15) * 128, rdx0 = (pm0 + l15) * 128;
+        f32x4 acc[TN1][TM1];
+#pragma unroll
+        for (int a = 0; a < TN1; ++a)
+#pragma unroll
+            for (int b = 0; b < TM1; ++b) acc[a][b] = (f32x4){0.f, 0.f, 0.f, 0.f};
+        int rd = 0;
+        PC_BARRIER()
+        for (int kt = 0; kt < nk1; ++kt) {
+            u32x4 x0[TM1], x1[TM1];
+            bf16x8 w0[TN1], w1[TN1];
+            const char* const wst = lds + rd + rdw0;
+#pragma unroll
+            for (int a = 0; a < TN1; ++a) {
+                w0[a] = __builtin_bit_cast(bf16x8, *reinterpret_cast<const u32x4*>(wst + a * 2048 + (c0 ^ swl)));
+                w1[a] = __builtin_bit_cast(bf16x8, *reinterpret_cast<const u32x4*>(wst + a * 2048 + (c1 ^ swl)));
+            }
+            const char* const xs = lds + rd + rdx0;
+#pragma unroll
+            for (int b = 0; b < TM1; ++b) {
+                x0[b] = *reinterpret_cast<const u32x4*>(xs + b * 2048 + (c0 ^ swl));
+                x1[b] = *reinterpret_cast<const u32x4*>(xs + b * 2048 + (c1 ^ swl));
+            }
+#pragma unroll
+            for (int a = 0; a < TN1; ++a)
+#pragma unroll
+                for (int b = 0; b < TM1; ++b) B2B_MFMA(w0[a], __builtin_bit_cast(bf16x8, x0[b]), acc[a][b]);
+#pragma unroll
+            for (int a = 0; a < TN1; ++a)
+#pragma unroll
+                for (int b = 0; b < TM1; ++b) B2B_MFMA(w1[a], __builtin_bit_cast(bf16x8, x1[b]), acc[a][b]);
+            PC_WAIT_LGKM0();
+            PC_BARRIER()
+            rd = rd == (NS - 1) * STAGE ? 0 : rd + STAGE;
+        }
+        const bool relu1 = ((p.flags >> CUTIE_ACT_SHIFT) & 7) == CUTIE_ACT_RELU;
+#pragma unroll
+        for (int a = 0; a < TNP1; ++a)
+#pragma unroll
+            for (int b = 0; b < TM1; ++b) {
+                float v[8];
+#pragma unroll
+                for (int r = 0; r < 4; ++r) {
+                    v[r] = acc[2 * a][b][r] + bias[a][r];
+                    v[4 + r] = acc[2 * a + 1][b][r] + bias[a][4 + r];
+                }
+                if (relu1) {
+#pragma unroll
+                    for (int r = 0; r < 8; ++r) v[r] = fmaxf(v[r], 0.f);
+                }
+                const int row = pm0 + b * 16 + l15, ch = cn0 + a * 32 + l4 * 8;
+                u32x4 o = {pack_bf2(v[0], v[1]), pack_bf2(v[2], v[3]), pack_bf2(v[4], v[5]), pack_bf2(v[6], v[7])};
+                *reinterpret_cast<u32x4*>(lds + (ch >> 6) * A2SLICE + row * 128 + ((((ch & 63) >> 3) ^ (row & 7)) << 4)) = o;
+            }
+        PC_WAIT_LGKM0();
+        PC_BARRIER()
+    }
+    {
+        const int pm0 = (wave / WN2) * (BM / WM2), cn0 = (wave % WN2) * (BN2 / WN2);
+        int mrow[TM2];
+        bool mval[TM2];
+#pragma unroll
+        for (int b = 0; b < TM2; ++b) {
+            mrow[b] = m0 + pm0 + b * 16 + l15;
+            mval[b] = mrow[b] < p.M;
+        }
+        const pc_gf32 bias_g = (pc_gf32)q.bias;
+        const int rdw0 = W2BASE + (cn0 + l15) * 128, rdx0 = (pm0 + l15) * 128;
+        const unsigned rpre[1][1][4] = {{{0u, 0u, 0u, 0u}}};
+        f32x4 acc[TN2][TM2];
+        float bias[TNP2][8];
+        int rd = 0, ks = 0, n0 = 0;
+        for (int t = 0; t < nk2; ++t) {
+            if (ks == 0) {
+#pragma unroll
+                for (int a = 0; a < TN2; ++a)
+#pragma unroll
+                    for (int b = 0; b < TM2; ++b) acc[a][b] = (f32x4){0.f, 0.f, 0.f, 0.f};
+#pragma unroll
+                for (int a = 0; a < TNP2; ++a)
+#pragma unroll
+                    for (int r = 0; r < 8; ++r) bias[a][r] = bias_g[n0 + cn0 + a * 32 + l4 * 8 + r];
+            }
+            u32x4 x0[TM2], x1[TM2];
+            bf16x8 w0[TN2], w1[TN2];
+            const char* const wst = lds + rd + rdw0;
+#pragma unroll
+            for (int a = 0; a < TN2; ++a) {
+                w0[a] = __builtin_bit_cast(bf16x8, *reinterpret_cast<const u32x4*>(wst + a * 2048 + (c0 ^ swl)));
+                w1[a] = __builtin_bit_cast(bf16x8, *reinterpret_cast<const u32x4*>(wst + a * 2048 + (c1 ^ swl)));
+            }
+            const char* const xs = lds + ks * A2SLICE + rdx0;
+#pragma unroll
+            for (int b = 0; b < TM2; ++b) {
+                x0[b] = *reinterpret_cast<const u32x4*>(xs + b * 2048 + (c0 ^ swl));
+                x1[b] = *reinterpret_cast<const u32x4*>(xs + b * 2048 + (c1 ^ swl));
+            }
+#pragma unroll
+            for (int a = 0; a < TN2; ++a)
+#pragma unroll
+                for (int b = 0; b < TM2; ++b) B2B_MFMA(w0[a], __builtin_bit_cast(bf16x8, x0[b]), acc[a][b]);
+#pragma unroll
+            for (int a = 0; a < TN2; ++a)
+#pragma unroll
+                for (int b = 0; b < TM2; ++b) B2B_MFMA(w1[a], __builtin_bit_cast(bf16x8, x1[b]), acc[a][b]);
+            PC_WAIT_LGKM0();
+            PC_BARRIER()
+            rd = rd == (NS2 - 1) * W2STAGE ? 0 : rd + W2STAGE;
+            if (++ks == KS2) {
+                pc_epilogue_fast<8, TM2, TNP2, true, true, false, true, false>(q, acc, bias, mrow, mval, n0 + cn0 + l4 * 8, rpre);
+                ks = 0;
+                n0 += BN2;
+            }
+        }
+    }
+#undef B2B_MFMA
+#endif
+}
+
+template <int BM, int CMID, int NPW, int WM1, int WN1, int WM2, int WN2, int BN2, int NS, int NS2, bool W2SEP>
+static int launch_b2b(const ConvParams& p, const ConvParams& q, hipStream_t s) {
+    constexpr int lds = b2b_lds_bytes<BM, CMID, BN2, NS, NS2, W2SEP>();
+    static_assert(lds <= 160 * 1024, "LDS");
+    static bool attr_set = false;
+    if (!attr_set) {
+        if (hipFuncSetAttribute(reinterpret_cast<const void*>(conv_b2b_kernel<BM, CMID, NPW, WM1, WN1, WM2, WN2, BN2, NS, NS2, W2SEP>),
+                                hipFuncAttributeMaxDynamicSharedMemorySize, lds) != hipSuccess) {
+            cutie_set_error("conv b2b: cannot raise the dynamic LDS limit to %d bytes", lds);
+            return -2;
+        }
+        attr_set = true;
+    }
+    hipLaunchKernelGGL((conv_b2b_kernel<BM, CMID, NPW, WM1, WN1, WM2, WN2, BN2, NS, NS2, W2SEP>), dim3((unsigned)((p.M + BM - 1) / BM)),
+                       dim3((WM1 * WN1 + NPW) * 64), lds, s, p, q);
+    return (int)hipGetLastError();
+}
+
+static int b2b_min_rows(int cmid) {
+    switch (cmid) {
+        case 64: return 25920;
+        case 128: return 77760;
+        default: return 1 << 30;
+    }
+}
+
+static bool b2b_stream_tile(int t) { return (t >= 60 && t < 90) || (t >= 100 && t < 120) || (t >= 140 && t <= 144); }
+
+int launch_conv_b2b(const cutie_op* a, const cutie_op* b, hipStream_t s, int* fused) {
+    *fused = 0;
+    if (b->kind != CUTIE_OP_CONV || !a->p[5] || b->p[0] != a->p[5]) return 0;
+    const int32_t *ia = a->i, *ib = b->i;
+    const int act_a = (a->flags >> CUTIE_ACT_SHIFT) & 7, act_b = (b->flags >> CUTIE_ACT_SHIFT) & 7;
+    const int plain = CUTIE_F_RELU_IN | CUTIE_F_OUT_F32 | CUTIE_F_RES_BCAST | CUTIE_F_PLAIN;
+    const int cmid = ia[9];
+    if ((a->flags & plain) || (b->flags & plain) || act_a > CUTIE_ACT_RELU || act_b != CUTIE_ACT_RELU) return 0;
+    if (cmid != 64 && cmid != 128 && cmid != 256) return 0;
+    if (!b2b_stream_tile(ia[17]) || !b2b_stream_tile(ib[17])) return 0;
+    if (ia[4] || a->p[1] || a->p[4] || !a->p[3] || ia[19] > 1 || a->p[7] || a->p[8] || ia[3] % 64 || ia[11] > 5 || ia[12] > 5) return 0;
+    if (ib[11] != 1 || ib[12] != 1 || ib[13] != 1 || ib[14] != 0 || ib[4] || b->p[1] || !b->p[4] || !b->p[3] || ib[19] > 1 || b->p[7] || b->p[8]) return 0;
+    if (ib[3] != cmid || ib[5] != ia[10] || ib[0] != ia[0] || ib[1] != ia[7] || ib[2] != ia[8] || (ib[10] & 7) || (ib[15] & 7) || (ib[9] & 127) || ib[9] < 256) return 0;
+    if (ia[11] * ia[12] * (ia[3] / 64) < 2) return 0;
+    const long M = (long)ia[0] * ia[7] * ia[8];
+    if (!(a->flags & CUTIE_F_FUSE_ANY) && M < b2b_min_rows(cmid)) return 0;
+    ConvParams p, q;
+    if (const int rc = conv_params_from_op(a, p)) return rc;
+    if (const int rc = conv_params_from_op(b, q)) return rc;
+    const long x_bytes = (long)p.B * p.H * p.W * p.ldx1 * 2, w1_bytes = (long)cmid * p.Kpad * 2, w2_bytes = (long)q.Cout * q.Kpad * 2;
+    if (p.Kpad < p.KH * p.KW * p.Cin || q.Kpad < cmid || x_bytes >= PC_RECORDS - 8192 || w1_bytes >= PC_RECORDS - 8192 || w2_bytes >= PC_RECORDS - 8192) return 0;
+    int rc;
+    if (cmid == 64 && M >= 65536)
+        rc = launch_b2b<128, 64, 4, 2, 2, 2, 2, 64, 3, 3, false>(p, q, s);
+    else if (cmid == 64)
+        rc = launch_b2b<128, 64, 8, 4, 2, 2, 4, 128, 3, 3, true>(p, q, s);
+    else if (cmid == 128)
+        rc = launch_b2b<128, 128, 8, 2, 4, 2, 4, 128, 3, 3, true>(p, q, s);
+    else
+        rc = launch_b2b<64, 256, 8, 2, 4, 2, 4, 128, 3, 3, false>(p, q, s);
+    if (rc == 0) *fused = 1;
+    return rc;
+}
diff --git a/cutie_amd/csrc/conv_common.h b/cutie_amd/csrc/conv_common.h
--- a/cutie_amd/csrc/conv_common.h
+++ b/cutie_amd/csrc/conv_common.h
@@ -134,3 +134,5 @@
 
 int launch_conv_dma(const ConvParams& p, int tile, hipStream_t s);
 int launch_conv_pc(const ConvParams& p, int tile, hipStream_t s);
+int conv_params_from_op(const cutie_op* op, ConvParams& p);
+int launch_conv_b2b(const cutie_op* a, const cutie_op* b, hipStream_t s, int* fused);
diff --git a/cutie_amd/csrc/conv_igemm.hip b/cutie_amd/csrc/conv_igemm.hip
--- a/cutie_amd/csrc/conv_igemm.hip
+++ b/cutie_amd/csrc/conv_igemm.hip
@@ -462,8 +462,7 @@
     return (int)hipGetLastError();
 }
 
-int launch_conv(const cutie_op* op, hipStream_t s) {
-    ConvParams p;
+int conv_params_from_op(const cutie_op* op, ConvParams& p) {
     p.x1 = (const bf16_t*)op->p[0]; p.x2 = (const bf16_t*)op->p[1]; p.w = (const bf16_t*)op->p[2];
     p.bias = (const float*)op->p[3]; p.res = (const bf16_t*)op->p[4]; p.y = (void*)op->p[5];
     const int32_t* i = op->i;
@@ -496,6 +495,13 @@
                         p.C1, p.C2, p.ldx1, p.ldx2, p.Kpad, p.M, p.Cout);
         return -2;
     }
+    return 0;
+}
+
+int launch_conv(const cutie_op* op, hipStream_t s) {
+    ConvParams p;
+    if (const int rc = conv_params_from_op(op, p)) return rc;
+    const int32_t* i = op->i;
     if (i[17] == 19) {
         const int LP = p.Cin >> 3;
         if (p.Cout != 1 || p.C2 != 0 || p.res || LP > 64 || (LP & (LP - 1)) || LP < 1) {
diff --git a/cutie_amd/csrc/conv_pc.hip b/cutie_amd/csrc/conv_pc.hip
--- a/cutie_amd/csrc/conv_pc.hip
+++ b/cutie_amd/csrc/conv_pc.hip
@@ -1,247 +1,4 @@
-#include "conv_common.h"
-
-typedef __amdgpu_buffer_rsrc_t rsrc_t;
-#define PC_WORD3 0x00020000
-#define PC_RECORDS 0x7fffffff
-#define PC_OOB 0x80000000u
-#define LDS_PTR(p) ((__attribute__((address_space(3))) void*)(p))
-#define PC_WAIT_VM(N) __builtin_amdgcn_s_waitcnt(((N) & 15) | (((N) >> 4) << 14) | (7 << 4) | (15 << 8))
-#define PC_WAIT_LGKM0() __builtin_amdgcn_s_waitcnt(15 | (3 << 14) | (7 << 4) | (0 << 8))
-#define PC_BARRIER() { asm volatile("" ::: "memory"); __builtin_amdgcn_s_barrier(); asm volatile("" ::: "memory"); }
-#ifdef PC_ABL_NO_LOOPBAR
-#define PC_LOOP_BARRIER() { asm volatile("" ::: "memory"); }
-#else
-#define PC_LOOP_BARRIER() PC_BARRIER()
-#endif
-#ifdef PC_ABL_NO_WAIT
-#define PC_LOOP_WAIT_VM(N) ((void)0)
-#else
-#define PC_LOOP_WAIT_VM(N) PC_WAIT_VM(N)
-#endif
-#ifdef PC_ABL_SAME_TILE
-#define PC_SAME_TILE_GUARD(...)
-#else
-#define PC_SAME_TILE_GUARD(...) __VA_ARGS__
-#endif
-#ifdef PC_ABL_NO_DMA
-#define PC_DMA(...) ((void)0)
-#else
-#define PC_DMA(...) __builtin_amdgcn_raw_ptr_buffer_load_lds(__VA_ARGS__)
-#endif
-
-__device__ __forceinline__ rsrc_t pc_rsrc(const void* base) {
-    return __builtin_amdgcn_make_buffer_rsrc(const_cast<void*>(base), 0, PC_RECORDS, PC_WORD3);
-}
-
-typedef short pc_s16x2 __attribute__((ext_vector_type(2)));
-__device__ __forceinline__ unsigned pc_relu2(unsigned w) {
-    return __builtin_bit_cast(unsigned, __builtin_elementwise_max(__builtin_bit_cast(pc_s16x2, w), (pc_s16x2){0, 0}));
-}
-
-__device__ __forceinline__ int pc_wrow(int R, bool pair) {
-    if (!pair) return R;
-    const int ii = R & 15, alo = (R >> 4) & 1;
-    return (R & ~31) | ((ii >> 2) << 3) | (alo << 2) | (ii & 3);
-}
-
-#define PC_HT(TH, TW) ((TH) * 256 + (TW))
-template <int BM, int BN, int NS, int HT>
-constexpr int pc_lds_bytes(int NPW) {
-    if (HT == 0) return NS * (BM + BN) * 128;
-    const int TH = HT >> 8, TW = HT & 255, npiece = ((TH + 2) * (TW + 2) + 7) / 8, nxp = (npiece + NPW - 1) / NPW;
-    return 2 * nxp * NPW * 1024 + NS * BN * 128;
-}
-
-template <int NCH>
-__device__ __forceinline__ void pc_finish(const ConvParams& p, float (&v)[NCH], int m, int ch0, bool vec_ok, bool have_res,
-                                          const unsigned (&rpre)[NCH / 2], float (&stored)[NCH]) {
-#ifdef PC_ABL_FIXED_EPI
-    {
-#pragma unroll
-        for (int r = 0; r < NCH; ++r) v[r] = fmaxf(v[r], 0.f);
-        bf16_t* yp = reinterpret_cast<bf16_t*>(p.y) + (long)m * p.ldy + ch0;
-        unsigned o[NCH / 2];
-#pragma unroll
-        for (int r = 0; r < NCH / 2; ++r) o[r] = pack_bf2(v[2 * r], v[2 * r + 1]);
-        if constexpr (NCH == 8) *reinterpret_cast<uint4*>(yp) = make_uint4(o[0], o[1], o[NCH / 2 - 2], o[NCH / 2 - 1]);
-        else *reinterpret_cast<uint2*>(yp) = make_uint2(o[0], o[1]);
-        return;
-    }
-#endif
-    const int act = (p.flags >> CUTIE_ACT_SHIFT) & 7;
-    const bool out_f32 = p.flags & CUTIE_F_OUT_F32;
-    const bool full = ch0 + NCH <= p.Cout;
-    if (p.res) {
-        if (have_res) {
-#pragma unroll
-            for (int r = 0; r < NCH / 2; ++r) { v[2 * r] += __uint_as_float(rpre[r] << 16); v[2 * r + 1] += __uint_as_float(rpre[r] & 0xffff0000u); }
-        } else {
-            const int mres = conv_res_row(p, m);
-            const bf16_t* rp = p.res + (long)mres * p.ldr + ch0;
-            if (full && vec_ok) {
-                unsigned rr[NCH / 2];
-                if constexpr (NCH == 8) { const uint4 t = *reinterpret_cast<const uint4*>(rp); rr[0] = t.x; rr[1] = t.y; rr[NCH / 2 - 2] = t.z; rr[NCH / 2 - 1] = t.w; }
-                else { const uint2 t = *reinterpret_cast<const uint2*>(rp); rr[0] = t.x; rr[1] = t.y; }
-#pragma unroll
-                for (int r = 0; r < NCH / 2; ++r) { v[2 * r] += __uint_as_float(rr[r] << 16); v[2 * r + 1] += __uint_as_float(rr[r] & 0xffff0000u); }
-            } else {
-#pragma unroll
-                for (int r = 0; r < NCH; ++r) if (ch0 + r < p.Cout) v[r] += bf2f(rp[r]);
-            }
-        }
-    }
-#pragma unroll
-    for (int r = 0; r < NCH; ++r) {
-        if (act == CUTIE_ACT_RELU) v[r] = fmaxf(v[r], 0.f);
-        else if (act == CUTIE_ACT_SIGMOID) v[r] = sigmoidf_(v[r]);
-        else if (act == CUTIE_ACT_SQ1) v[r] = v[r] * v[r] + 1.f;
-    }
-    if (out_f32) {
-        float* yp = reinterpret_cast<float*>(p.y) + (long)m * p.ldy + ch0;
-        if (full && vec_ok) {
-#pragma unroll
-            for (int r = 0; r < NCH; r += 4) *reinterpret_cast<float4*>(yp + r) = make_float4(v[r], v[r + 1], v[r + 2], v[r + 3]);
-        } else {
-#pragma unroll
-            for (int r = 0; r < NCH; ++r) if (ch0 + r < p.Cout) yp[r] = v[r];
-        }
-    } else {
-        bf16_t* yp = reinterpret_cast<bf16_t*>(p.y) + (long)m * p.ldy + ch0;
-        unsigned o[NCH / 2];
-#pragma unroll
-        for (int r = 0; r < NCH / 2; ++r) o[r] = pack_bf2(v[2 * r], v[2 * r + 1]);
-        if (full && vec_ok) {
-            if constexpr (NCH == 8) *reinterpret_cast<uint4*>(yp) = make_uint4(o[0], o[1], o[NCH / 2 - 2], o[NCH / 2 - 1]);
-            else *reinterpret_cast<uint2*>(yp) = make_uint2(o[0], o[1]);
-        } else {
-#pragma unroll
-            for (int r = 0; r < NCH; ++r) if (ch0 + r < p.Cout) yp[r] = (bf16_t)(r & 1 ? o[r >> 1] >> 16 : o[r >> 1] & 0xffffu);
-        }
-        {
-#pragma unroll
-            for (int r = 0; r < NCH / 2; ++r) { stored[2 * r] = __uint_as_float(o[r] << 16); stored[2 * r + 1] = __uint_as_float(o[r] & 0xffff0000u); }
-        }
-    }
-}
-
-__device__ __forceinline__ int pc_div(int m, int d, float rd) {
-    int q = (int)((float)m * rd);
-    int r = m - q * d;
-    q += (r >= d) ? 1 : 0;
-    q -= (r < 0) ? 1 : 0;
-    return q;
-}
-
-__device__ __forceinline__ int pc_res_row(const ConvParams& p, int m) {
-    if (!(p.flags & CUTIE_F_RES_BCAST)) return m;
-    int r = m - pc_div(m, p.OHW, __builtin_amdgcn_rcpf((float)p.OHW)) * p.OHW;
-    if (p.res_grp_rows > 0) r += pc_div(m, p.res_grp_rows, __builtin_amdgcn_rcpf((float)p.res_grp_rows)) * p.res_grp_stride;
-    return r;
-}
-
-template <int NCH>
-__device__ __forceinline__ long long pc_colsum16(const long long (&s)[NCH], int l15, int& c, bool& writer) {
-    const bool h8 = l15 & 8, h4 = l15 & 4, h2 = l15 & 2;
-    long long w;
-    if constexpr (NCH == 8) {
-        long long t[4], u[2];
-#pragma unroll
-        for (int r = 0; r < 4; ++r) t[r] = (h8 ? s[4 + r] : s[r]) + __shfl_xor(h8 ? s[r] : s[4 + r], 8, 64);
-#pragma unroll
-        for (int r = 0; r < 2; ++r) u[r] = (h4 ? t[2 + r] : t[r]) + __shfl_xor(h4 ? t[r] : t[2 + r], 4, 64);
-        w = (h2 ? u[1] : u[0]) + __shfl_xor(h2 ? u[0] : u[1], 2, 64);
-        w += __shfl_xor(w, 1, 64);
-        c = (h8 ? 4 : 0) + (h4 ? 2 : 0) + (h2 ? 1 : 0);
-        writer = (l15 & 1) == 0;
-    } else {
-        long long t[2];
-#pragma unroll
-        for (int r = 0; r < 2; ++r) t[r] = (h8 ? s[2 + r] : s[r]) + __shfl_xor(h8 ? s[r] : s[2 + r], 8, 64);
-        w = (h4 ? t[1] : t[0]) + __shfl_xor(h4 ? t[0] : t[1], 4, 64);
-        w += __shfl_xor(w, 2, 64);
-        w += __shfl_xor(w, 1, 64);
-        c = (h8 ? 2 : 0) + (h4 ? 1 : 0);
-        writer = (l15 & 3) == 0;
-    }
-    return w;
-}
-__device__ __forceinline__ long long pc_gapfx(float v) { return conv_gapfx(v); }
-__device__ __forceinline__ void pc_gap_add(const ConvParams& p, int obj, int ch, long long v) {
-    if (ch < p.Cout) atomicAdd(reinterpret_cast<unsigned long long*>(p.gap + (long)obj * p.Cout + ch), (unsigned long long)(v << GAP_ELEM_SHIFT));
-}
-
-template <int NCH, int TM, int TNP, bool PAIR, bool RELU_OUT, bool F32, bool RES, bool PRE, bool GAPJ = false>
-__device__ __forceinline__ void pc_epilogue_fast(const ConvParams& p, const f32x4 (&acc)[PAIR ? 2 * TNP : TNP][TM], const float (&bias)[TNP][NCH],
-                                                 const int (&mrow)[TM], const bool (&mval)[TM], int chbase,
-                                                 const unsigned (&rpre)[PRE ? TM : 1][PRE ? TNP : 1][NCH / 2], int gap_obj = 0, int l15 = 0) {
-    unsigned rr[TM][TNP][NCH / 2];
-    if (RES && !PRE) {
-#pragma unroll
-        for (int b = 0; b < TM; ++b) {
-            const int mres = pc_res_row(p, mrow[b]);
-#pragma unroll
-            for (int a = 0; a < TNP; ++a) {
-                const bf16_t* rp = p.res + (long)mres * p.ldr + chbase + a * (PAIR ? 32 : 16);
-#pragma unroll
-                for (int r = 0; r < NCH / 2; ++r) rr[b][a][r] = 0u;
-                if (mval[b]) {
-                    if constexpr (NCH == 8) { const uint4 t = *reinterpret_cast<const uint4*>(rp); rr[b][a][0] = t.x; rr[b][a][1] = t.y; rr[b][a][NCH / 2 - 2] = t.z; rr[b][a][NCH / 2 - 1] = t.w; }
-                    else { const uint2 t = *reinterpret_cast<const uint2*>(rp); rr[b][a][0] = t.x; rr[b][a][1] = t.y; }
-                }
-            }
-        }
-    }
-#pragma unroll
-    for (int a = 0; a < TNP; ++a) {
-        long long gs[NCH];
-#pragma unroll
-        for (int r = 0; r < NCH; ++r) gs[r] = 0;
-#pragma unroll
-        for (int b = 0; b < TM; ++b) {
-            float v[NCH];
-#pragma unroll
-            for (int r = 0; r < 4; ++r) {
-                v[r] = acc[PAIR ? 2 * a : a][b][r] + bias[a][r];
-                if (PAIR) v[(NCH - 4) + r] = acc[PAIR ? 2 * a + 1 : a][b][r] + bias[a][(NCH - 4) + r];
-            }
-            if (RES) {
-#pragma unroll
-                for (int r = 0; r < NCH / 2; ++r) {
-                    const unsigned w = PRE ? rpre[PRE ? b : 0][PRE ? a : 0][r] : rr[b][a][r];
-                    v[2 * r] += __uint_as_float(w << 16); v[2 * r + 1] += __uint_as_float(w & 0xffff0000u);
-                }
-            }
-            if (RELU_OUT) {
-#pragma unroll
-                for (int r = 0; r < NCH; ++r) v[r] = fmaxf(v[r], 0.f);
-            }
-            if (mval[b]) {
-                const long off = (long)mrow[b] * p.ldy + chbase + a * (PAIR ? 32 : 16);
-                if (F32) {
-                    float* yp = reinterpret_cast<float*>(p.y) + off;
-#pragma unroll
-                    for (int r = 0; r < NCH; r += 4) *reinterpret_cast<float4*>(yp + r) = make_float4(v[r], v[r + 1], v[r + 2], v[r + 3]);
-                } else {
-                    bf16_t* yp = reinterpret_cast<bf16_t*>(p.y) + off;
-                    unsigned o[NCH / 2];
-#pragma unroll
-                    for (int r = 0; r < NCH / 2; ++r) o[r] = pack_bf2(v[2 * r], v[2 * r + 1]);
-                    if constexpr (NCH == 8) *reinterpret_cast<uint4*>(yp) = make_uint4(o[0], o[1], o[NCH / 2 - 2], o[NCH / 2 - 1]);
-                    else *reinterpret_cast<uint2*>(yp) = make_uint2(o[0], o[1]);
-                    if (GAPJ) {
-#pragma unroll
-                        for (int r = 0; r < NCH / 2; ++r) { gs[2 * r] += pc_gapfx(__uint_as_float(o[r] << 16)); gs[2 * r + 1] += pc_gapfx(__uint_as_float(o[r] & 0xffff0000u)); }
-                    }
-                }
-            }
-        }
-        if (GAPJ) {
-            int c; bool writer;
-            const long long tot = pc_colsum16<NCH>(gs, l15, c, writer);
-            if (writer) pc_gap_add(p, gap_obj, chbase + a * (PAIR ? 32 : 16) + c, tot);
-        }
-    }
-}
+#include "conv_pc_common.h"
 
 template <int BM, int BN, int WM, int WN, int NPW, int NS, int HT, bool TAPS, bool RELU, bool TWO, int KP = 1>
 __global__ __launch_bounds__((WM * WN + NPW) * 64) void conv_pc_kernel(ConvParams p) {
diff --git a/cutie_amd/csrc/conv_pc_common.h b/cutie_amd/csrc/conv_pc_common.h
--- /dev/null
+++ b/cutie_amd/csrc/conv_pc_common.h
@@ -0,0 +1,245 @@
+#pragma once
+#include "conv_common.h"
+
+typedef __amdgpu_buffer_rsrc_t rsrc_t;
+#define PC_WORD3 0x00020000
+#define PC_RECORDS 0x7fffffff
+#define PC_OOB 0x80000000u
+#define LDS_PTR(p) ((__attribute__((address_space(3))) void*)(p))
+#define PC_WAIT_VM(N) __builtin_amdgcn_s_waitcnt(((N) & 15) | (((N) >> 4) << 14) | (7 << 4) | (15 << 8))
+#define PC_WAIT_LGKM0() __builtin_amdgcn_s_waitcnt(15 | (3 << 14) | (7 << 4) | (0 << 8))
+#define PC_BARRIER() { asm volatile("" ::: "memory"); __builtin_amdgcn_s_barrier(); asm volatile("" ::: "memory"); }
+#ifdef PC_ABL_NO_LOOPBAR
+#define PC_LOOP_BARRIER() { asm volatile("" ::: "memory"); }
+#else
+#define PC_LOOP_BARRIER() PC_BARRIER()
+#endif
+#ifdef PC_ABL_NO_WAIT
+#define PC_LOOP_WAIT_VM(N) ((void)0)
+#else
+#define PC_LOOP_WAIT_VM(N) PC_WAIT_VM(N)
+#endif
+#ifdef PC_ABL_SAME_TILE
+#define PC_SAME_TILE_GUARD(...)
+#else
+#define PC_SAME_TILE_GUARD(...) __VA_ARGS__
+#endif
+#ifdef PC_ABL_NO_DMA
+#define PC_DMA(...) ((void)0)
+#else
+#define PC_DMA(...) __builtin_amdgcn_raw_ptr_buffer_load_lds(__VA_ARGS__)
+#endif
+
+__device__ __forceinline__ rsrc_t pc_rsrc(const void* base) {
+    return __builtin_amdgcn_make_buffer_rsrc(const_cast<void*>(base), 0, PC_RECORDS, PC_WORD3);
+}
+
+typedef short pc_s16x2 __attribute__((ext_vector_type(2)));
+__device__ __forceinline__ unsigned pc_relu2(unsigned w) {
+    return __builtin_bit_cast(unsigned, __builtin_elementwise_max(__builtin_bit_cast(pc_s16x2, w), (pc_s16x2){0, 0}));
+}
+
+__device__ __forceinline__ int pc_wrow(int R, bool pair) {
+    if (!pair) return R;
+    const int ii = R & 15, alo = (R >> 4) & 1;
+    return (R & ~31) | ((ii >> 2) << 3) | (alo << 2) | (ii & 3);
+}
+
+#define PC_HT(TH, TW) ((TH) * 256 + (TW))
+template <int BM, int BN, int NS, int HT>
+constexpr int pc_lds_bytes(int NPW) {
+    if (HT == 0) return NS * (BM + BN) * 128;
+    const int TH = HT >> 8, TW = HT & 255, npiece = ((TH + 2) * (TW + 2) + 7) / 8, nxp = (npiece + NPW - 1) / NPW;
+    return 2 * nxp * NPW * 1024 + NS * BN * 128;
+}
+
+template <int NCH>
+__device__ __forceinline__ void pc_finish(const ConvParams& p, float (&v)[NCH], int m, int ch0, bool vec_ok, bool have_res,
+                                          const unsigned (&rpre)[NCH / 2], float (&stored)[NCH]) {
+#ifdef PC_ABL_FIXED_EPI
+    {
+#pragma unroll
+        for (int r = 0; r < NCH; ++r) v[r] = fmaxf(v[r], 0.f);
+        bf16_t* yp = reinterpret_cast<bf16_t*>(p.y) + (long)m * p.ldy + ch0;
+        unsigned o[NCH / 2];
+#pragma unroll
+        for (int r = 0; r < NCH / 2; ++r) o[r] = pack_bf2(v[2 * r], v[2 * r + 1]);
+        if constexpr (NCH == 8) *reinterpret_cast<uint4*>(yp) = make_uint4(o[0], o[1], o[NCH / 2 - 2], o[NCH / 2 - 1]);
+        else *reinterpret_cast<uint2*>(yp) = make_uint2(o[0], o[1]);
+        return;
+    }
+#endif
+    const int act = (p.flags >> CUTIE_ACT_SHIFT) & 7;
+    const bool out_f32 = p.flags & CUTIE_F_OUT_F32;
+    const bool full = ch0 + NCH <= p.Cout;
+    if (p.res) {
+        if (have_res) {
+#pragma unroll
+            for (int r = 0; r < NCH / 2; ++r) { v[2 * r] += __uint_as_float(rpre[r] << 16); v[2 * r + 1] += __uint_as_float(rpre[r] & 0xffff0000u); }
+        } else {
+            const int mres = conv_res_row(p, m);
+            const bf16_t* rp = p.res + (long)mres * p.ldr + ch0;
+            if (full && vec_ok) {
+                unsigned rr[NCH / 2];
+                if constexpr (NCH == 8) { const uint4 t = *reinterpret_cast<const uint4*>(rp); rr[0] = t.x; rr[1] = t.y; rr[NCH / 2 - 2] = t.z; rr[NCH / 2 - 1] = t.w; }
+                else { const uint2 t = *reinterpret_cast<const uint2*>(rp); rr[0] = t.x; rr[1] = t.y; }
+#pragma unroll
+                for (int r = 0; r < NCH / 2; ++r) { v[2 * r] += __uint_as_float(rr[r] << 16); v[2 * r + 1] += __uint_as_float(rr[r] & 0xffff0000u); }
+            } else {
+#pragma unroll
+                for (int r = 0; r < NCH; ++r) if (ch0 + r < p.Cout) v[r] += bf2f(rp[r]);
+            }
+        }
+    }
+#pragma unroll
+    for (int r = 0; r < NCH; ++r) {
+        if (act == CUTIE_ACT_RELU) v[r] = fmaxf(v[r], 0.f);
+        else if (act == CUTIE_ACT_SIGMOID) v[r] = sigmoidf_(v[r]);
+        else if (act == CUTIE_ACT_SQ1) v[r] = v[r] * v[r] + 1.f;
+    }
+    if (out_f32) {
+        float* yp = reinterpret_cast<float*>(p.y) + (long)m * p.ldy + ch0;
+        if (full && vec_ok) {
+#pragma unroll
+            for (int r = 0; r < NCH; r += 4) *reinterpret_cast<float4*>(yp + r) = make_float4(v[r], v[r + 1], v[r + 2], v[r + 3]);
+        } else {
+#pragma unroll
+            for (int r = 0; r < NCH; ++r) if (ch0 + r < p.Cout) yp[r] = v[r];
+        }
+    } else {
+        bf16_t* yp = reinterpret_cast<bf16_t*>(p.y) + (long)m * p.ldy + ch0;
+        unsigned o[NCH / 2];
+#pragma unroll
+        for (int r = 0; r < NCH / 2; ++r) o[r] = pack_bf2(v[2 * r], v[2 * r + 1]);
+        if (full && vec_ok) {
+            if constexpr (NCH == 8) *reinterpret_cast<uint4*>(yp) = make_uint4(o[0], o[1], o[NCH / 2 - 2], o[NCH / 2 - 1]);
+            else *reinterpret_cast<uint2*>(yp) = make_uint2(o[0], o[1]);
+        } else {
+#pragma unroll
+            for (int r = 0; r < NCH; ++r) if (ch0 + r < p.Cout) yp[r] = (bf16_t)(r & 1 ? o[r >> 1] >> 16 : o[r >> 1] & 0xffffu);
+        }
+        {
+#pragma unroll
+            for (int r = 0; r < NCH / 2; ++r) { stored[2 * r] = __uint_as_float(o[r] << 16); stored[2 * r + 1] = __uint_as_float(o[r] & 0xffff0000u); }
+        }
+    }
+}
+
+__device__ __forceinline__ int pc_div(int m, int d, float rd) {
+    int q = (int)((float)m * rd);
+    int r = m - q * d;
+    q += (r >= d) ? 1 : 0;
+    q -= (r < 0) ? 1 : 0;
+    return q;
+}
+
+__device__ __forceinline__ int pc_res_row(const ConvParams& p, int m) {
+    if (!(p.flags & CUTIE_F_RES_BCAST)) return m;
+    int r = m - pc_div(m, p.OHW, __builtin_amdgcn_rcpf((float)p.OHW)) * p.OHW;
+    if (p.res_grp_rows > 0) r += pc_div(m, p.res_grp_rows, __builtin_amdgcn_rcpf((float)p.res_grp_rows)) * p.res_grp_stride;
+    return r;
+}
+
+template <int NCH>
+__device__ __forceinline__ long long pc_colsum16(const long long (&s)[NCH], int l15, int& c, bool& writer) {
+    const bool h8 = l15 & 8, h4 = l15 & 4, h2 = l15 & 2;
+    long long w;
+    if constexpr (NCH == 8) {
+        long long t[4], u[2];
+#pragma unroll
+        for (int r = 0; r < 4; ++r) t[r] = (h8 ? s[4 + r] : s[r]) + __shfl_xor(h8 ? s[r] : s[4 + r], 8, 64);
+#pragma unroll
+        for (int r = 0; r < 2; ++r) u[r] = (h4 ? t[2 + r] : t[r]) + __shfl_xor(h4 ? t[r] : t[2 + r], 4, 64);
+        w = (h2 ? u[1] : u[0]) + __shfl_xor(h2 ? u[0] : u[1], 2, 64);
+        w += __shfl_xor(w, 1, 64);
+        c = (h8 ? 4 : 0) + (h4 ? 2 : 0) + (h2 ? 1 : 0);
+        writer = (l15 & 1) == 0;
+    } else {
+        long long t[2];
+#pragma unroll
+        for (int r = 0; r < 2; ++r) t[r] = (h8 ? s[2 + r] : s[r]) + __shfl_xor(h8 ? s[r] : s[2 + r], 8, 64);
+        w = (h4 ? t[1] : t[0]) + __shfl_xor(h4 ? t[0] : t[1], 4, 64);
+        w += __shfl_xor(w, 2, 64);
+        w += __shfl_xor(w, 1, 64);
+        c = (h8 ? 2 : 0) + (h4 ? 1 : 0);
+        writer = (l15 & 3) == 0;
+    }
+    return w;
+}
+__device__ __forceinline__ long long pc_gapfx(float v) { return conv_gapfx(v); }
+__device__ __forceinline__ void pc_gap_add(const ConvParams& p, int obj, int ch, long long v) {
+    if (ch < p.Cout) atomicAdd(reinterpret_cast<unsigned long long*>(p.gap + (long)obj * p.Cout + ch), (unsigned long long)(v << GAP_ELEM_SHIFT));
+}
+
+template <int NCH, int TM, int TNP, bool PAIR, bool RELU_OUT, bool F32, bool RES, bool PRE, bool GAPJ = false>
+__device__ __forceinline__ void pc_epilogue_fast(const ConvParams& p, const f32x4 (&acc)[PAIR ? 2 * TNP : TNP][TM], const float (&bias)[TNP][NCH],
+                                                 const int (&mrow)[TM], const bool (&mval)[TM], int chbase,
+                                                 const unsigned (&rpre)[PRE ? TM : 1][PRE ? TNP : 1][NCH / 2], int gap_obj = 0, int l15 = 0) {
+    unsigned rr[TM][TNP][NCH / 2];
+    if (RES && !PRE) {
+#pragma unroll
+        for (int b = 0; b < TM; ++b) {
+            const int mres = pc_res_row(p, mrow[b]);
+#pragma unroll
+            for (int a = 0; a < TNP; ++a) {
+                const bf16_t* rp = p.res + (long)mres * p.ldr + chbase + a * (PAIR ? 32 : 16);
+#pragma unroll
+                for (int r = 0; r < NCH / 2; ++r) rr[b][a][r] = 0u;
+                if (mval[b]) {
+                    if constexpr (NCH == 8) { const uint4 t = *reinterpret_cast<const uint4*>(rp); rr[b][a][0] = t.x; rr[b][a][1] = t.y; rr[b][a][NCH / 2 - 2] = t.z; rr[b][a][NCH / 2 - 1] = t.w; }
+                    else { const uint2 t = *reinterpret_cast<const uint2*>(rp); rr[b][a][0] = t.x; rr[b][a][1] = t.y; }
+                }
+            }
+        }
+    }
+#pragma unroll
+    for (int a = 0; a < TNP; ++a) {
+        long long gs[NCH];
+#pragma unroll
+        for (int r = 0; r < NCH; ++r) gs[r] = 0;
+#pragma unroll
+        for (int b = 0; b < TM; ++b) {
+            float v[NCH];
+#pragma unroll
+            for (int r = 0; r < 4; ++r) {
+                v[r] = acc[PAIR ? 2 * a : a][b][r] + bias[a][r];
+                if (PAIR) v[(NCH - 4) + r] = acc[PAIR ? 2 * a + 1 : a][b][r] + bias[a][(NCH - 4) + r];
+            }
+            if (RES) {
+#pragma unroll
+                for (int r = 0; r < NCH / 2; ++r) {
+                    const unsigned w = PRE ? rpre[PRE ? b : 0][PRE ? a : 0][r] : rr[b][a][r];
+                    v[2 * r] += __uint_as_float(w << 16); v[2 * r + 1] += __uint_as_float(w & 0xffff0000u);
+                }
+            }
+            if (RELU_OUT) {
+#pragma unroll
+                for (int r = 0; r < NCH; ++r) v[r] = fmaxf(v[r], 0.f);
+            }
+            if (mval[b]) {
+                const long off = (long)mrow[b] * p.ldy + chbase + a * (PAIR ? 32 : 16);
+                if (F32) {
+                    float* yp = reinterpret_cast<float*>(p.y) + off;
+#pragma unroll
+                    for (int r = 0; r < NCH; r += 4) *reinterpret_cast<float4*>(yp + r) = make_float4(v[r], v[r + 1], v[r + 2], v[r + 3]);
+                } else {
+                    bf16_t* yp = reinterpret_cast<bf16_t*>(p.y) + off;
+                    unsigned o[NCH / 2];
+#pragma unroll
+                    for (int r = 0; r < NCH / 2; ++r) o[r] = pack_bf2(v[2 * r], v[2 * r + 1]);
+                    if constexpr (NCH == 8) *reinterpret_cast<uint4*>(yp) = make_uint4(o[0], o[1], o[NCH / 2 - 2], o[NCH / 2 - 1]);
+                    else *reinterpret_cast<uint2*>(yp) = make_uint2(o[0], o[1]);
+                    if (GAPJ) {
+#pragma unroll
+                        for (int r = 0; r < NCH / 2; ++r) { gs[2 * r] += pc_gapfx(__uint_as_float(o[r] << 16)); gs[2 * r + 1] += pc_gapfx(__uint_as_float(o[r] & 0xffff0000u)); }
+                    }
+                }
+            }
+        }
+        if (GAPJ) {
+            int c; bool writer;
+            const long long tot = pc_colsum16<NCH>(gs, l15, c, writer);
+            if (writer) pc_gap_add(p, gap_obj, chbase + a * (PAIR ? 32 : 16) + c, tot);
+        }
+    }
+}
diff --git a/cutie_amd/model/plans.py b/cutie_amd/model/plans.py
--- a/cutie_amd/model/plans.py
+++ b/cutie_amd/model/plans.py
@@ -41,6 +41,7 @@
 
 GRAPHS = os.environ.get('CUTIE_AMD_GRAPHS', '0') not in ('', '0')
 GRAPH_MIN_OPS = 8
+B2B = os.environ.get('CUTIE_AMD_B2B', '1') not in ('', '0')
 QINIT_SKIP = os.environ.get('CUTIE_AMD_QINIT_SKIP', '1') not in ('', '0')
 AUTOTUNE = os.environ.get('CUTIE_AMD_AUTOTUNE', '0') not in ('', '0')
 PACKAGED_TILES = os.path.join(os.path.dirname(os.path.abspath(__file__)), '..', 'tiles_gfx950.json')
@@ -202,6 +203,8 @@
     def pack_into(self, arena):
         arr = self.ol.finalize()
         ptrs = arr['p'].astype(np.int64)
+        fused_head = (arr['kind'] == O.CONV) & ((arr['flags'] & O.F_FUSE_NEXT) != 0)
+        fused_head[-1:] = False
         items = []
         for name, t in self.bufs.items():
             if name in self.persistent or t.numel() == 0:
@@ -211,7 +214,8 @@
             if not hit.any():
                 continue
             rows = np.nonzero(hit.any(axis=1))[0]
-            items.append(dict(name=name, base=base, nbytes=nbytes, first=int(rows[0]), last=int(rows[-1]), hit=hit, t=t))
+            last = max(int(r) + (1 if fused_head[r] else 0) for r in rows)
+            items.append(dict(name=name, base=base, nbytes=nbytes, first=int(rows[0]), last=last, hit=hit, t=t))
         items.sort(key=lambda b: (b['first'], -b['nbytes']))
         placed = []
         total = 0
@@ -348,7 +352,8 @@
             save_tile_cache(cache)
 
     def conv(self, wname, x, *, name=None, out=None, stride=1, pad=None, x2=None, res=None, res_bcast=False,
-             relu_in=False, act=O.ACT_NONE, out_f32=False, ldy=None, gap_acc=None, zero=None, persistent=False, res_group=None):
+             relu_in=False, act=O.ACT_NONE, out_f32=False, ldy=None, gap_acc=None, zero=None, persistent=False, res_group=None,
+             fuse_next=False):
         w = self.eng.w[wname]
         if pad is None:
             pad = (w.kh - 1) // 2
@@ -365,7 +370,7 @@
                      pad=pad, x2=None if x2 is None else x2.t, C2=0 if x2 is None else x2.C,
                      ldx2=0 if x2 is None else x2.ld, res=None if res is None else res.t,
                      ldr=0 if res is None else res.ld, res_bcast=res_bcast, relu_in=relu_in, act=act, out_f32=out_f32,
-                     gap_acc=gap_acc, zero=zero, prio=self.prio, res_group=res_group)
+                     gap_acc=gap_acc, zero=zero, prio=self.prio, res_group=res_group, fuse_next=fuse_next)
         return out
 
     def ca_block(self, prefix, x, name, out=None, head=None):
@@ -407,9 +412,13 @@
                 last = bi == nb - 1
                 out = taps.get(lname) if (taps and last) else None
                 if bottleneck:
+                    down = (p + '.downsample.0') in self.eng.w
+                    fuse = B2B and _lib.has_conv_b2b()
                     t1 = self.conv(p + '.conv1', x, act=O.ACT_RELU)
-                    t2 = self.conv(p + '.conv2', t1, stride=s, act=O.ACT_RELU)
-                    r = self.conv(p + '.downsample.0', x, stride=s) if (p + '.downsample.0') in self.eng.w else x
+                    r = self.conv(p + '.downsample.0', x, stride=s) if (down and fuse) else x
+                    t2 = self.conv(p + '.conv2', t1, stride=s, act=O.ACT_RELU, fuse_next=fuse)
+                    if down and not fuse:
+                        r = self.conv(p + '.downsample.0', x, stride=s)
                     x = self.conv(p + '.conv3', t2, res=r, act=O.ACT_RELU, out=out)
                 else:
                     t1 = self.conv(p + '.conv1', x, stride=s, act=O.ACT_RELU)
diff --git a/cutie_amd/ops.py b/cutie_amd/ops.py
--- a/cutie_amd/ops.py
+++ b/cutie_amd/ops.py
@@ -23,6 +23,7 @@
 
 F_RELU_IN, F_OUT_F32, F_RES_BCAST = 1, 2, 4
 F_PRIO, F_AFF_PRIO = 256, 64
+F_FUSE_NEXT, F_FUSE_ANY = 512, 1024
 F_TILE_OFF = 128 if os.environ.get('CUTIE_AMD_COUT1_TILE', '1') in ('', '0') else 0
 ACT_NONE, ACT_RELU, ACT_SIGMOID, ACT_SQ1 = 0, 1, 2, 3
 ACT_SHIFT = 4
@@ -367,9 +368,9 @@
 
     def conv(self, x1, w, y, *, B, H, W, C1, ldx1, OH, OW, ldy, stride=1, pad=0, x2=None, C2=0, ldx2=0,
              res=None, ldr=0, res_bcast=False, relu_in=False, act=ACT_NONE, out_f32=False, tile=None, splitk=1,
-             gap_acc=None, zero=None, prio=False, res_group=None):
+             gap_acc=None, zero=None, prio=False, res_group=None, fuse_next=False):
         flags = (F_RELU_IN if relu_in else 0) | (F_OUT_F32 if out_f32 else 0) | (F_RES_BCAST if res_bcast else 0) | (act << ACT_SHIFT) | F_TILE_OFF | \
-            (F_PRIO if prio else 0)
+            (F_PRIO if prio else 0) | (F_FUSE_NEXT if fuse_next else 0) | (F_FUSE_ANY if fuse_next == 'any' else 0)
         assert C1 + C2 == w.cin_padded, (C1, C2, w.cin_padded)
         M = B * OH * OW
         side = gap_acc is not None or zero is not None
diff --git a/include/cutie_hip.h b/include/cutie_hip.h
--- a/include/cutie_hip.h
+++ b/include/cutie_hip.h
@@ -27,6 +27,8 @@
 #define CUTIE_F_PLAIN     8
 #define CUTIE_F_TILE_OFF  128
 #define CUTIE_F_PRIO      256
+#define CUTIE_F_FUSE_NEXT 512
+#define CUTIE_F_FUSE_ANY  1024
 #define CUTIE_ACT_SHIFT   4
 #define CUTIE_ACT_NONE    0
 #define CUTIE_ACT_RELU    1
```

Result: no change. 1168 (median of 3 runs) (+0.1%).
